# qiangbo1222/HierDiff

Measured on AMD Instinct MI355X. Metric: sampled molecules/sec (1000 diffusion steps, B=256, N=30), higher is better.
Workload: dtype f32

## Files before the change

### hierdiff_amd/csrc/common.hpp

```cpp
#pragma once
#include <hip/hip_runtime.h>
#include <stdint.h>
#include <type_traits>

typedef float f32x4 __attribute__((ext_vector_type(4)));
typedef float f32x16 __attribute__((ext_vector_type(16)));
typedef float f32x2 __attribute__((ext_vector_type(2)));
typedef unsigned u32x4 __attribute__((ext_vector_type(4)));
typedef __bf16 bf16x2_t __attribute__((ext_vector_type(2)));
typedef __bf16 bf16x4_t __attribute__((ext_vector_type(4)));
typedef __bf16 bf16x8_t __attribute__((ext_vector_type(8)));
typedef __bf16 bf16x8 __attribute__((ext_vector_type(8)));

#define HD_DEVINL __device__ __forceinline__

HD_DEVINL void glds16(const void* gsrc, void* lds_dst) {
    __builtin_amdgcn_global_load_lds((const __attribute__((address_space(1))) void*)gsrc,
                                     (__attribute__((address_space(3))) void*)lds_dst, 16, 0, 0);
}
template <int OFF>
HD_DEVINL void glds16o(const void* gsrc, void* lds_dst) {
    static_assert(OFF >= 0 && OFF < 4096, "12-bit immediate");
    __builtin_amdgcn_global_load_lds((const __attribute__((address_space(1))) void*)gsrc,
                                     (__attribute__((address_space(3))) void*)lds_dst, 16, OFF, 0);
}


HD_DEVINL float silu_f(float x) {
    const float L2E_HI = 1.44269502162933349609375f;
    const float L2E_LO = 1.925962991e-8f;
    const float LN2 = 0.693147180559945309f;
    float nx = -x;
    float t = nx * L2E_HI;
    float tlo = __builtin_fmaf(nx, L2E_HI, -t) + nx * L2E_LO;
    float e = __builtin_amdgcn_exp2f(t);
    e = e * __builtin_fmaf(tlo, LN2, 1.0f);
    return x * __builtin_amdgcn_rcpf(1.0f + e);
}

HD_DEVINL float sigmoid_f(float x) {
    const float L2E_HI = 1.44269502162933349609375f, L2E_LO = 1.925962991e-8f, LN2 = 0.693147180559945309f;
    float nx = -x;
    float t = nx * L2E_HI;
    float tlo = __builtin_fmaf(nx, L2E_HI, -t) + nx * L2E_LO;
    float e = __builtin_amdgcn_exp2f(t) * __builtin_fmaf(tlo, LN2, 1.0f);
    return __builtin_amdgcn_rcpf(1.0f + e);
}

HD_DEVINL float silu_fast(float x) {
    float e = __builtin_amdgcn_exp2f(x * -1.44269502162933349609375f);
    return x * __builtin_amdgcn_rcpf(1.0f + e);
}

HD_DEVINL float silu_scaled(float x) { return x * __builtin_amdgcn_rcpf(1.0f + __builtin_amdgcn_exp2f(x)); }
HD_DEVINL void bf16_split2(float y0, float y1, uint32_t& hi, uint32_t& lo) {
    const uint32_t hp = __builtin_bit_cast(uint32_t, __builtin_convertvector((f32x2){y0, y1}, bf16x2_t));
    const float l0 = y0 - __builtin_bit_cast(float, hp << 16);
    const float l1 = y1 - __builtin_bit_cast(float, hp & 0xffff0000u);
    hi = hp;
    lo = __builtin_bit_cast(uint32_t, __builtin_convertvector((f32x2){l0, l1}, bf16x2_t));
}

typedef _Float16 f16x8 __attribute__((ext_vector_type(8)));
typedef _Float16 f16x2_t __attribute__((ext_vector_type(2)));
HD_DEVINL void f16_split2(float y0, float y1, uint32_t& hi, uint32_t& lo) {
    const f16x2_t hp = __builtin_convertvector((f32x2){y0, y1}, f16x2_t);
    const float l0 = y0 - (float)hp[0];
    const float l1 = y1 - (float)hp[1];
    hi = __builtin_bit_cast(uint32_t, hp);
    lo = __builtin_bit_cast(uint32_t, __builtin_convertvector((f32x2){l0, l1}, f16x2_t));
}
template <bool F16>
HD_DEVINL void split2(float y0, float y1, uint32_t& hi, uint32_t& lo) {
    if constexpr (F16) f16_split2(y0, y1, hi, lo);
    else bf16_split2(y0, y1, hi, lo);
}
template <bool F16>
HD_DEVINL f32x16 mma16(bf16x8 a, bf16x8 b, f32x16 c) {
    if constexpr (F16) return __builtin_amdgcn_mfma_f32_32x32x16_f16(__builtin_bit_cast(f16x8, a), __builtin_bit_cast(f16x8, b), c, 0, 0, 0);
    else return __builtin_amdgcn_mfma_f32_32x32x16_bf16(a, b, c, 0, 0, 0);
}
#define HD_F16_FLOOR 9.5367431640625e-07f
#define HD_TWOWAY(p) ((p) == 1 || (p) == 3)

HD_DEVINL void bf16_split3(float y0, float y1, uint32_t& hi, uint32_t& mid, uint32_t& lo) {
    const uint32_t hp = __builtin_bit_cast(uint32_t, __builtin_convertvector((f32x2){y0, y1}, bf16x2_t));
    const float r0 = y0 - __builtin_bit_cast(float, hp << 16);
    const float r1 = y1 - __builtin_bit_cast(float, hp & 0xffff0000u);
    const uint32_t mp = __builtin_bit_cast(uint32_t, __builtin_convertvector((f32x2){r0, r1}, bf16x2_t));
    const float s0 = r0 - __builtin_bit_cast(float, mp << 16);
    const float s1 = r1 - __builtin_bit_cast(float, mp & 0xffff0000u);
    hi = hp;
    mid = mp;
    lo = __builtin_bit_cast(uint32_t, __builtin_convertvector((f32x2){s0, s1}, bf16x2_t));
}

template <int I, int N, typename F>
HD_DEVINL void static_for(F&& f) {
    if constexpr (I < N) {
        f(std::integral_constant<int, I>{});
        static_for<I + 1, N>(f);
    }
}


HD_DEVINL void philox_round(uint32_t& c0, uint32_t& c1, uint32_t& c2, uint32_t& c3, uint32_t k0, uint32_t k1) {
    const uint32_t M0 = 0xD2511F53u, M1 = 0xCD9E8D57u;
    uint32_t hi0 = __umulhi(M0, c0), lo0 = M0 * c0;
    uint32_t hi1 = __umulhi(M1, c2), lo1 = M1 * c2;
    uint32_t n0 = hi1 ^ c1 ^ k0, n1 = lo1, n2 = hi0 ^ c3 ^ k1, n3 = lo0;
    c0 = n0; c1 = n1; c2 = n2; c3 = n3;
}

HD_DEVINL float philox_normal(uint64_t seed, uint64_t sample, uint32_t draw, uint32_t index) {
    uint32_t c0 = index >> 1, c1 = draw, c2 = (uint32_t)sample, c3 = (uint32_t)(sample >> 32);
    uint32_t k0 = (uint32_t)seed, k1 = (uint32_t)(seed >> 32);
#pragma unroll
    for (int r = 0; r < 10; ++r) {
        philox_round(c0, c1, c2, c3, k0, k1);
        k0 += 0x9E3779B9u; k1 += 0xBB67AE85u;
    }
    float u1 = ((float)(c0 >> 8) + 0.5f) * (1.0f / 16777216.0f);
    float u2 = ((float)(c1 >> 8) + 0.5f) * (1.0f / 16777216.0f);
    float rad = sqrtf(-2.0f * logf(u1));
    float ang = 6.283185307179586f * u2;
    return (index & 1) ? rad * sinf(ang) : rad * cosf(ang);
}
```

### hierdiff_amd/csrc/hierdiff_hip.hip

```cpp
#include "../../include/hierdiff_hip.h"
#include "kernels.hpp"

#include <algorithm>
#include <cmath>
#include <cstdio>
#include <cstring>
#include <cstdlib>
#include <string>
#include <mutex>
#include <vector>


static thread_local std::string g_err;

static int fail(int code, const std::string& msg) {
    g_err = msg;
    return code;
}

#define HIP_TRY(expr)                                                                        \
    do {                                                                                     \
        hipError_t _e = (expr);                                                              \
        if (_e != hipSuccess)                                                                \
            return fail(HD_E_HIP, std::string(#expr) + ": " + hipGetErrorString(_e));        \
    } while (0)

#define HD_TRY(expr)                 \
    do {                             \
        int _r = (expr);             \
        if (_r != HD_OK) return _r;  \
    } while (0)


#define HD_FUSE_MIN_ROWS 5400
#define HD_NODE_SPLIT_MAX_ROWS 2048
#define HD_SPLIT_MAX_TILES 512
#define HD_MIX_MAX_TILES 16384

struct LayerW {
    size_t ab_img, ab_bias, wrd, w2_img, b2, wa, w3_img, b3, w4_img, b4;
    size_t ab_gimg, w3_gimg, w4_gimg;
    float ba;
    float w2s, wrmax, wdmax;
    float w3s, w4s, abs_;
    float w3l1, w4l1, b3max, b4max;
};

struct ProfRec { int fam; hipEvent_t a, b; };

struct hd_handle {
    hd_config cfg;
    int device;
    int H, fin, F, D, NS;
    int edge_mode, node_mode;
    bool scaled;
    long long n_weights;
    bool weights_set;
    float* dw;
    size_t dw_floats;
    size_t embT, emb_b, outW, out_b;
    std::vector<LayerW> gcl;
    std::vector<LayerW> coord;
    int* d_nanflag;
    long long* d_nan_events;
    int T;
    std::vector<float> tau_h, coef_h;
    float* d_tau;
    float* d_coef;
    int* d_step;
    uint32_t* d_draw;
    float* d_tcur;
    unsigned long long* d_base;
    hipStream_t own_stream;
    hipEvent_t ev_in, ev_out;
    hipEvent_t ev_last;
    bool ev_last_set;
    unsigned long long weights_gen, sched_gen;
    float* d_coef_ip;
    unsigned long long ip_sched_gen, ip_gen;
    uint32_t* d_ipdraw;
    int ipdraw_cap;
    int split_max_tiles;
    int fuse_min_rows;
    int node_split_max_rows;
    int f32_split;
    int mix_max_tiles;
    int mix_rounds;
    int n_cu;
#ifdef HD_DEBUG_KERNELS
    long long* d_trace;
    int trace_wg;
    int ablate;
#endif
    int prof;
    int prof_stride;
    long long prof_fwd;
    bool prof_now;
    std::vector<ProfRec> recs;
    std::vector<hipEvent_t> pool;
    size_t pool_used;
};

struct GraphKey {
    const float *raw_x, *raw_h;
    int has_ctx, mol_shape, noise_rows, T, s_hi;
    uint64_t seed;
    unsigned long long weights_gen, sched_gen;
    bool operator==(const GraphKey& o) const {
        return raw_x == o.raw_x && raw_h == o.raw_h && has_ctx == o.has_ctx && mol_shape == o.mol_shape &&
               noise_rows == o.noise_rows && T == o.T && s_hi == o.s_hi && seed == o.seed && weights_gen == o.weights_gen &&
               sched_gen == o.sched_gen;
    }
};

struct InpaintKey {
    int has_ctx, T, resamplings;
    uint64_t seed;
    unsigned long long weights_gen, sched_gen, ip_gen;
    bool operator==(const InpaintKey& o) const {
        return has_ctx == o.has_ctx && T == o.T && resamplings == o.resamplings && seed == o.seed && weights_gen == o.weights_gen &&
               sched_gen == o.sched_gen && ip_gen == o.ip_gen;
    }
};

struct hd_topology {
    hd_handle* h;
    int device;
    char* arena;
    int B, N, M, M_pad, E, E_pad, n_tiles, n_wg, n_parts;
    int *node_of, *slot_of, *ei, *ej, *seg_part, *tile_nseg, *pstart, *nvalid;
    int *rptr, *rrows, *sptr, *srows;
    std::vector<int>* node_of_host;
    float *w2img, *w2timg;
    uint8_t *eseg, *nm_bytes;
    float* nmask;
    float *hbuf, *AB, *AB2, *Tb, *agg, *x0, *xcur, *part, *xpart, *eps;
    float *abmax, *abmax2;
    float *rowinfo;
    float *zbuf, *ctxbuf;
    hipGraphExec_t gexec;
    GraphKey gkey;
    hipGraphExec_t gexec_ip;
    InpaintKey ikey;
    uint8_t* ip_fixed;
    float* ip_known;
    size_t arena_bytes;
    char* staging;
    size_t staging_bytes;
    hipStream_t stream0, last_stream;
    hipEvent_t ready;
    bool multi_stream;
};


static inline float agg_norm(const hd_config& c, const hd_topology* t) {
    return c.aggregation_mean ? (float)t->N : c.normalization_factor;
}

extern "C" int hd_version(void) { return HD_ABI_VERSION; }
extern "C" const char* hd_last_error(void) { return g_err.c_str(); }

extern "C" int hd_device_count(void) {
    int n = 0;
    if (hipGetDeviceCount(&n) != hipSuccess) { (void)hipGetLastError(); return 0; }
    return n;
}

static long long weight_count(const hd_config& c) {
    const long long H = c.hidden_nf, fin = c.in_node_nf + c.context_node_nf;
    long long n = H * fin + H + fin * H + fin;
    long long gcl = H * (2 * H + 2) + H + H * H + H + H * 2 * H + H + H * H + H + (c.attention ? H + 1 : 0);
    long long crd = H * (2 * H + 2) + H + H * H + H + H;
    n += (long long)c.n_layers * (c.inv_sublayers * gcl + crd);
    return n;
}

extern "C" long long hd_weight_count(const hd_handle* h) { return h ? h->n_weights : 0; }

template <typename T>
static int dev_alloc(T** p, size_t count) {
    *p = nullptr;
    if (count == 0) count = 1;
    hipError_t e = hipMalloc(reinterpret_cast<void**>(p), count * sizeof(T));
    if (e != hipSuccess) return fail(HD_E_NOMEM, std::string("hipMalloc: ") + hipGetErrorString(e));
    return HD_OK;
}

template <typename T>
static int dev_upload(T** p, const std::vector<T>& v) {
    HD_TRY(dev_alloc(p, v.size()));
    if (!v.empty()) HIP_TRY(hipMemcpy(*p, v.data(), v.size() * sizeof(T), hipMemcpyHostToDevice));
    return HD_OK;
}


static int prepare_kernels(hd_handle* h);
template <int H> static int prepare_edge_bwd_h();

extern "C" int hd_create(const hd_config* cfg, int device, hd_handle** out) {
    if (!cfg || !out) return fail(HD_E_INVALID, "hd_create: null argument");
    *out = nullptr;
    if (cfg->n_dims != 3) return fail(HD_E_INVALID, "hd_create: n_dims must be 3");
    const int H = cfg->hidden_nf;
    if (H != 32 && H != 64 && H != 128 && H != 256)
        return fail(HD_E_INVALID, "hd_create: hidden_nf must be 32, 64, 128 or 256");
    if (cfg->n_layers < 1 || cfg->inv_sublayers < 1) return fail(HD_E_INVALID, "hd_create: n_layers / inv_sublayers must be >= 1");
    const int F = cfg->in_node_nf - (cfg->condition_time ? 1 : 0);
    if (F < 1) return fail(HD_E_INVALID, "hd_create: in_node_nf must leave at least one feature column");
    if (cfg->context_node_nf < 0) return fail(HD_E_INVALID, "hd_create: context_node_nf < 0");
    if (cfg->precision != 0 && cfg->precision != 3)
        return fail(HD_E_INVALID, "hd_create: precision must be 0 (fp32) or 3 (fp16x3); 1 (bf16x3) and 2 (bf16x6) were retired in ABI 12");
    if (!cfg->aggregation_mean && !(cfg->normalization_factor != 0.0f)) return fail(HD_E_INVALID, "hd_create: normalization_factor == 0");
    if (hd_device_count() <= device || device < 0)
        return fail(HD_E_HIP, "hd_create: no such HIP device (is a GPU visible?)");
    HIP_TRY(hipSetDevice(device));
    hd_handle* h = new hd_handle();
    h->cfg = *cfg;
    h->device = device;
    h->H = H;
    h->fin = cfg->in_node_nf + cfg->context_node_nf;
    h->F = F;
    h->D = 3 + F;
    {
        const bool wide = cfg->hidden_nf >= 128;
        switch (cfg->precision) {
            case 3: h->edge_mode = 3; h->node_mode = wide ? 3 : 0; break;
            default: h->edge_mode = 0; h->node_mode = 0; break;
        }
        h->scaled = h->edge_mode == 3;
    }
    h->NS = (cfg->hidden_nf == 32) ? 1 : 2;
    h->n_weights = weight_count(*cfg);
    h->weights_set = false;
    h->dw = nullptr;
    h->dw_floats = 0;
    h->T = 0;
    h->d_tau = h->d_coef = nullptr;
    h->prof = 0;
    h->prof_stride = 1;
    h->prof_fwd = 0;
    h->prof_now = false;
    h->pool_used = 0;
    h->own_stream = nullptr;
    h->ev_in = h->ev_out = nullptr;
    h->ev_last = nullptr; h->ev_last_set = false;
    h->weights_gen = h->sched_gen = 0;
    h->d_coef_ip = nullptr; h->ip_sched_gen = 0; h->ip_gen = 0; h->d_ipdraw = nullptr; h->ipdraw_cap = 0;
    h->d_nanflag = nullptr; h->d_nan_events = nullptr; h->d_step = nullptr; h->d_draw = nullptr; h->d_tcur = nullptr;
    h->d_base = nullptr;
    h->split_max_tiles = HD_SPLIT_MAX_TILES;
    h->mix_max_tiles = HD_MIX_MAX_TILES;
    h->fuse_min_rows = HD_FUSE_MIN_ROWS;
    h->node_split_max_rows = HD_NODE_SPLIT_MAX_ROWS;
    h->f32_split = 1;
    h->mix_rounds = -1;
    {
        hipDeviceProp_t prop;
        h->n_cu = (hipGetDeviceProperties(&prop, device) == hipSuccess && prop.multiProcessorCount > 0) ? prop.multiProcessorCount : 256;
    }
#ifdef HD_DEBUG_KERNELS
    h->d_trace = nullptr; h->trace_wg = 0;
    { const char* e = getenv("HD_ABLATE"); h->ablate = e ? atoi(e) : 0; }
    { const char* e = getenv("HD_SPLIT_MAX_TILES"); if (e) h->split_max_tiles = atoi(e); }
    { const char* e = getenv("HD_MIX_MAX_TILES"); if (e) h->mix_max_tiles = atoi(e); }
    { const char* e = getenv("HD_FUSE_MIN_ROWS"); if (e) h->fuse_min_rows = atoi(e); }
    { const char* e = getenv("HD_NODE_SPLIT_MAX_ROWS"); if (e) h->node_split_max_rows = atoi(e); }
    { const char* e = getenv("HD_F32_SPLIT"); if (e) h->f32_split = atoi(e); }
    { const char* e = getenv("HD_MIX_ROUNDS"); if (e) h->mix_rounds = atoi(e); }
#endif
    auto create_rest = [&]() -> int {
        HD_TRY(dev_alloc(&h->d_nanflag, 1));
        HD_TRY(dev_alloc(&h->d_nan_events, 1));
        HD_TRY(dev_alloc(&h->d_step, 1));
        HD_TRY(dev_alloc(&h->d_draw, 1));
        HD_TRY(dev_alloc(&h->d_tcur, 1));
        HD_TRY(dev_alloc(&h->d_base, 1));
        HIP_TRY(hipMemset(h->d_nanflag, 0, sizeof(int)));
        HIP_TRY(hipMemset(h->d_nan_events, 0, sizeof(long long)));
        HIP_TRY(hipEventCreateWithFlags(&h->ev_in, hipEventDisableTiming));
        HIP_TRY(hipEventCreateWithFlags(&h->ev_out, hipEventDisableTiming));
        HIP_TRY(hipEventCreateWithFlags(&h->ev_last, hipEventDisableTiming));
        return prepare_kernels(h);
    };
    const int r = create_rest();
    if (r != HD_OK) { const std::string keep = g_err; hd_destroy(h); g_err = keep; return r; }
    *out = h;
    return HD_OK;
}

extern "C" int hd_destroy(hd_handle* h) {
    if (!h) return HD_OK;
    (void)hipSetDevice(h->device);
    (void)hipDeviceSynchronize();
    hipFree(h->dw); hipFree(h->d_nanflag); hipFree(h->d_nan_events);
    hipFree(h->d_tau); hipFree(h->d_coef); hipFree(h->d_step); hipFree(h->d_draw); hipFree(h->d_tcur); hipFree(h->d_base);
    hipFree(h->d_coef_ip); hipFree(h->d_ipdraw);
#ifdef HD_DEBUG_KERNELS
    hipFree(h->d_trace);
#endif
    for (auto e : h->pool) hipEventDestroy(e);
    if (h->ev_in) hipEventDestroy(h->ev_in);
    if (h->ev_out) hipEventDestroy(h->ev_out);
    if (h->ev_last) hipEventDestroy(h->ev_last);
    if (h->own_stream) hipStreamDestroy(h->own_stream);
    delete h;
    return HD_OK;
}


template <typename Fn>
static void pack_gemm_b(std::vector<float>& dst, size_t off, int K, int Nc, int WN, Fn W) {
    const int BN = 32 * WN, ntile = Nc / BN, nchunk = K / 32;
    for (int ct = 0; ct < ntile; ++ct)
        for (int c = 0; c < nchunk; ++c)
            for (int wc = 0; wc < WN; ++wc)
                for (int q = 0; q < 4; ++q)
                    for (int lane = 0; lane < 64; ++lane)
                        for (int j = 0; j < 4; ++j) {
                            const int k = 32 * c + 16 * (lane >> 5) + 4 * q + j;
                            const int col = ct * BN + 32 * wc + (lane & 31);
                            dst[off + ((((size_t)(ct * nchunk + c) * WN + wc) * 4 + q) * 64 + lane) * 4 + j] = W(col, k);
                        }
}

template <typename Fn>
static void pack_gemm_b16(std::vector<float>& dst, size_t off, int K, int Nc, Fn W) {
    const int nchunk = K / 32;
    for (int ct = 0; ct < Nc / 16; ++ct)
        for (int c = 0; c < nchunk; ++c)
            for (int lane = 0; lane < 64; ++lane)
                for (int p = 0; p < 8; ++p) {
                    const int m = lane & 15, gs = lane >> 4, odd = gs >> 1, hf = gs & 1;
                    dst[off + (((size_t)ct * nchunk + c) * 64 + lane) * 8 + p] = W(16 * ct + m, 32 * c + 16 * hf + 2 * p + odd);
                }
}

static void pack_edge_w2(std::vector<float>& dst, size_t off, int H, const float* W2) {
    const int NCT = H / 32;
    for (int c = 0; c < H / 32; ++c)
        for (int q = 0; q < 4; ++q)
            for (int ct = 0; ct < NCT; ++ct)
                for (int lane = 0; lane < 64; ++lane)
                    for (int j = 0; j < 4; ++j) {
                        const int k = 32 * c + 16 * (lane >> 5) + 4 * q + j;
                        const int col = 32 * ct + (lane & 31);
                        dst[off + (size_t)c * 32 * H + ((size_t)(q * NCT + ct) * 64 + lane) * 4 + j] = W2[(size_t)col * H + k];
                    }
}

template <typename Fn>
static float pack_node_b_f16(std::vector<float>& dstf, size_t off, int K, int Nc, Fn W, float* l1) {
    float wmax = 0.0f, l1max = 0.0f;
    for (int col = 0; col < Nc; ++col) {
        double sum = 0.0;
        for (int k = 0; k < K; ++k) { const float v = std::fabs(W(col, k)); sum += v; if (v > wmax && std::isfinite(v)) wmax = v; }
        l1max = std::max(l1max, (float)(sum * 1.000001));
    }
    if (l1) *l1 = l1max;
    int ex = 0;
    if (wmax > 0.0f) (void)std::frexp(wmax, &ex);
    const float sw = std::ldexp(1.0f, wmax > 0.0f ? std::max(-100, std::min(100, 15 - ex)) : 0);
    _Float16* dst = reinterpret_cast<_Float16*>(dstf.data() + off);
    const int nct = Nc / 32;
    for (int st = 0; st < K / 16; ++st)
        for (int ct = 0; ct < nct; ++ct)
            for (int lane = 0; lane < 64; ++lane)
                for (int i = 0; i < 8; ++i) {
                    const float v = W(32 * ct + (lane & 31), 16 * st + 8 * (lane >> 5) + i) * sw;
                    const size_t base = ((size_t)(st * nct + ct) * 2) * 512;
                    const _Float16 hi = (_Float16)v;
                    dst[base + (size_t)lane * 8 + i] = hi;
                    dst[base + 512 + (size_t)lane * 8 + i] = (_Float16)(v - (float)hi);
                }
    return sw;
}

template <typename Fn>
static void pack_node_b_f32(std::vector<float>& dst, size_t off, int K, int Nc, Fn W) {
    const int nct = Nc / 32;
    for (int st = 0; st < K / 32; ++st)
        for (int ct = 0; ct < nct; ++ct)
            for (int q = 0; q < 4; ++q)
                for (int lane = 0; lane < 64; ++lane)
                    for (int j = 0; j < 4; ++j)
                        dst[off + (((size_t)(st * nct + ct) * 4 + q) * 64 + lane) * 4 + j] =
                            W(32 * ct + (lane & 31), 32 * st + 16 * (lane >> 5) + 4 * q + j);
}

static float pack_edge_w2_f16(std::vector<float>& dstf, size_t off, int H, const float* W2) {
    float wmax = 0.0f;
    for (size_t i = 0; i < (size_t)H * H; ++i) { const float v = std::fabs(W2[i]); if (v > wmax && std::isfinite(v)) wmax = v; }
    int ex = 0;
    if (wmax > 0.0f) (void)std::frexp(wmax, &ex);
    const int k = std::max(-100, std::min(100, 15 - ex));
    const float sw = std::ldexp(1.0f, wmax > 0.0f ? k : 0);
    _Float16* dst = reinterpret_cast<_Float16*>(dstf.data() + off);
    const int NCT = H / 32;
    for (int c = 0; c < H / 32; ++c)
        for (int st = 0; st < 2; ++st)
            for (int ct = 0; ct < NCT; ++ct)
                for (int lane = 0; lane < 64; ++lane)
                    for (int i = 0; i < 8; ++i) {
                        const int kk = 32 * c + 16 * (lane >> 5) + 8 * st + i;
                        const int col = 32 * ct + (lane & 31);
                        const float v = W2[(size_t)col * H + kk] * sw;
                        const _Float16 hi = (_Float16)v;
                        const _Float16 lo = (_Float16)(v - (float)hi);
                        const size_t blk = (size_t)c * 32 * H * 2;
// ... 274 lines not shown
    std::vector<float>& nmask = L.nmask;
    slot_of.assign(BN, -1); node_of.clear(); nvalid.assign(B, 0); nmask.clear();
    for (size_t f = 0; f < BN; ++f) {
        if (active[f]) { slot_of[f] = (int)node_of.size(); node_of.push_back((int)f); nmask.push_back(node_mask[f] ? 1.0f : 0.0f); }
        if (node_mask[f]) nvalid[f / N]++;
    }
    const int M = (int)node_of.size();
    const int M_pad = std::max(128, (M + 127) / 128 * 128);
    nmask.resize(M_pad, 0.0f);
    std::vector<int> mei, mej;
    std::vector<long long> mstart(B + 1, 0);
    for (int b = 0; b < B; ++b) {
        for (int i = 0; i < N; ++i) {
            const size_t fi = (size_t)b * N + i;
            if (!active[fi]) continue;
            for (int j = 0; j < N; ++j) {
                const size_t fj = (size_t)b * N + j;
                const bool on = edge_mask ? edge_mask[fi * N + j] != 0 : (node_mask[fi] && node_mask[fj] && i != j);
                if (on) { mei.push_back(slot_of[fi]); mej.push_back(slot_of[fj]); }
            }
        }
        mstart[b + 1] = (long long)mei.size();
    }
    const long long E = (long long)mei.size();
    if (E > (1LL << 30)) return fail(HD_E_INVALID, "hd_topology_create: too many edges");
    std::vector<int>& pstart = L.pstart;
    std::vector<int> first_piece(M, 0);
    pstart.assign(M + 1, 0);
    for (int b = 0; b < B; ++b) {
        const long long e0 = mstart[b], e1 = mstart[b + 1];
        for (long long e = e0; e < e1;) {
            const int node = mei[e];
            long long f = e;
            while (f < e1 && mei[f] == node) ++f;
            first_piece[node] = (int)((e - e0) / 32);
            pstart[node + 1] = (int)((f - 1 - e0) / 32) - first_piece[node] + 1;
            e = f;
        }
    }
    for (int i = 0; i < M; ++i) pstart[i + 1] += pstart[i];
    std::vector<int>&ei = L.ei, &ej = L.ej, &seg_part = L.seg_part, &tile_nseg = L.tile_nseg;
    std::vector<uint8_t>& eseg = L.eseg;
    ei.clear(); ej.clear(); seg_part.clear(); tile_nseg.clear(); eseg.clear();
    auto new_tile = [&]() {
        const int t = (int)tile_nseg.size();
        ei.resize(ei.size() + 32, 0); ej.resize(ej.size() + 32, 0); eseg.resize(eseg.size() + 32, 255);
        seg_part.resize(seg_part.size() + 32, 0); tile_nseg.push_back(0);
        return t;
    };
    auto place = [&](int t, int off, int b, int piece, int cnt) {
        const long long e0 = mstart[b] + 32LL * piece;
        int prev = -1;
        for (int r = 0; r < cnt; ++r) {
            const int node = mei[e0 + r];
            if (node != prev) {
                seg_part[(size_t)t * 32 + tile_nseg[t]] = pstart[node] + (piece - first_piece[node]);
                tile_nseg[t]++;
                prev = node;
            }
            ei[(size_t)t * 32 + off + r] = node; ej[(size_t)t * 32 + off + r] = mej[e0 + r];
            eseg[(size_t)t * 32 + off + r] = (uint8_t)(tile_nseg[t] - 1);
        }
    };
    int tail_tile = -1, tail_fill = 0;
    for (int b = 0; b < B; ++b) {
        const int Eb = (int)(mstart[b + 1] - mstart[b]);
        const int nfull = Eb / 32, tail = Eb % 32;
        for (int k = 0; k < nfull; ++k) place(new_tile(), 0, b, k, 32);
        if (tail) {
            if (tail_tile < 0 || tail_fill + tail > 32) { tail_tile = new_tile(); tail_fill = 0; }
            place(tail_tile, tail_fill, b, nfull, tail);
            tail_fill = (tail_fill + tail + 3) & ~3;
        }
    }
    L.n_tiles = (int)tile_nseg.size();
    L.n_wg = (L.n_tiles + 3) / 4;
    while ((int)tile_nseg.size() < std::max(1, L.n_wg * 4)) new_tile();
    L.M = M; L.M_pad = M_pad; L.E = E; L.n_parts = pstart[M];
    L.rptr.assign(M + 1, 0); L.sptr.assign(M + 1, 0);
    const size_t rows = ei.size();
    for (size_t r = 0; r < rows; ++r)
        if (eseg[r] != 255) { L.rptr[ei[r] + 1]++; L.sptr[ej[r] + 1]++; }
    for (int i = 0; i < M; ++i) { L.rptr[i + 1] += L.rptr[i]; L.sptr[i + 1] += L.sptr[i]; }
    L.rrows.assign((size_t)E, 0); L.srows.assign((size_t)E, 0);
    {
        std::vector<int> rp(L.rptr.begin(), L.rptr.end() - 1), sp(L.sptr.begin(), L.sptr.end() - 1);
        for (size_t r = 0; r < rows; ++r)
            if (eseg[r] != 255) { L.rrows[rp[ei[r]]++] = (int)r; L.srows[sp[ej[r]]++] = (int)r; }
    }
    return HD_OK;
}

extern "C" int hd_topology_layout(const uint8_t* node_mask, const uint8_t* edge_mask, int B, int N, long long* counts5,
                                  int* ei, int* ej, uint8_t* eseg, int* seg_part, int* tile_nseg, int* pstart) {
    if (!node_mask || !counts5) return fail(HD_E_INVALID, "hd_topology_layout: null argument");
    TileLayout L;
    HD_TRY(build_layout(node_mask, edge_mask, B, N, L));
    counts5[0] = L.M; counts5[1] = L.E; counts5[2] = (long long)L.tile_nseg.size(); counts5[3] = L.n_parts;
    counts5[4] = (long long)L.ei.size();
    if (ei) std::copy(L.ei.begin(), L.ei.end(), ei);
    if (ej) std::copy(L.ej.begin(), L.ej.end(), ej);
    if (eseg) std::copy(L.eseg.begin(), L.eseg.end(), eseg);
    if (seg_part) std::copy(L.seg_part.begin(), L.seg_part.end(), seg_part);
    if (tile_nseg) std::copy(L.tile_nseg.begin(), L.tile_nseg.end(), tile_nseg);
    if (pstart) std::copy(L.pstart.begin(), L.pstart.end(), pstart);
    return HD_OK;
}

extern "C" int hd_topology_create_s(hd_handle* h, const uint8_t* node_mask, const uint8_t* edge_mask, int B, int N,
                                    void* stream, hd_topology** out) {
    if (!h || !node_mask || !out) return fail(HD_E_INVALID, "hd_topology_create: null argument");
    hipStream_t s0 = (hipStream_t)stream;
    *out = nullptr;
    TileLayout L;
    HD_TRY(build_layout(node_mask, edge_mask, B, N, L));
    HIP_TRY(hipSetDevice(h->device));
    const size_t BN = (size_t)B * N;
    const int M = L.M, M_pad = L.M_pad, n_tiles = L.n_tiles, n_wg = L.n_wg, n_parts = L.n_parts;
    const long long E = L.E;
    const int E_pad = (int)L.ei.size();
    std::vector<int>&slot_of = L.slot_of, &node_of = L.node_of, &nvalid = L.nvalid, &ei = L.ei, &ej = L.ej;
    std::vector<int>&seg_part = L.seg_part, &tile_nseg = L.tile_nseg, &pstart = L.pstart;
    std::vector<uint8_t>& eseg = L.eseg;
    std::vector<float>& nmask = L.nmask;
    std::vector<uint8_t> nm_bytes(BN);
    for (size_t f = 0; f < BN; ++f) nm_bytes[f] = node_mask[f] ? 1 : 0;

    hd_topology* t = new hd_topology();
    std::memset(t, 0, sizeof(*t));
    t->h = h; t->device = h->device; t->B = B; t->N = N; t->M = M; t->M_pad = M_pad; t->E = (int)E; t->E_pad = E_pad;
    t->n_tiles = n_tiles; t->n_wg = n_wg; t->n_parts = n_parts;
    const int H = h->H;
    std::vector<char> blob;
    auto stage = [&](const void* src, size_t bytes) {
        const size_t off = (blob.size() + 255) & ~size_t(255);
        blob.resize(off + std::max<size_t>(bytes, 4), 0);
        if (bytes) std::memcpy(blob.data() + off, src, bytes);
        return off;
    };
    auto stage_v = [&](const auto& v) { return stage(v.data(), v.size() * sizeof(v[0])); };
    const size_t o_node_of = stage_v(node_of), o_slot_of = stage_v(slot_of), o_ei = stage_v(ei), o_ej = stage_v(ej);
    const size_t o_seg_part = stage_v(seg_part), o_tile_nseg = stage_v(tile_nseg), o_pstart = stage_v(pstart), o_nvalid = stage_v(nvalid);
    const size_t o_eseg = stage_v(eseg), o_nm = stage_v(nm_bytes), o_nmask = stage_v(nmask);
    const size_t o_rptr = stage_v(L.rptr), o_rrows = stage_v(L.rrows), o_sptr = stage_v(L.sptr), o_srows = stage_v(L.srows);
    const size_t table_bytes = (blob.size() + 255) & ~size_t(255);
    size_t ws_floats = 0;
    auto carve = [&](size_t count) { const size_t o = ws_floats; ws_floats += (std::max<size_t>(count, 1) + 63) & ~size_t(63); return o; };
    const size_t f_h = carve((size_t)M_pad * H), f_AB = carve((size_t)M_pad * 2 * H), f_AB2 = carve((size_t)M_pad * 2 * H);
    const size_t f_Tb = carve((size_t)M_pad * H), f_agg = carve((size_t)M_pad * H);
    const size_t f_x0 = carve((size_t)M_pad * 4), f_xcur = carve((size_t)M_pad * 4);
    const size_t f_part = carve((size_t)std::max(1, n_parts) * H), f_xpart = carve((size_t)std::max(1, n_parts) * 4);
    const size_t f_abmax = carve((size_t)M_pad * 2), f_abmax2 = carve((size_t)M_pad * 2), f_rowinfo = carve((size_t)M_pad * 2);
    const size_t f_eps = carve(BN * h->D), f_z = carve(BN * h->D), f_ctx = carve(BN * (size_t)std::max(1, h->cfg.context_node_nf));
    const size_t f_w2 = carve((size_t)H * H * 3 / 2), f_w2t = carve((size_t)H * H * 3 / 2);
    auto build = [&]() -> int {
        ArenaSlot sl;
        HD_TRY(arena_acquire(h->device, table_bytes + ws_floats * sizeof(float), table_bytes, sl));
        t->arena = sl.dev; t->arena_bytes = sl.dev_bytes; t->staging = sl.pinned; t->staging_bytes = sl.pinned_bytes;
        t->stream0 = t->last_stream = s0;
        char* base = t->arena;
        std::memcpy(t->staging, blob.data(), blob.size());
        HIP_TRY(hipMemcpyAsync(base, t->staging, blob.size(), hipMemcpyHostToDevice, s0));
        HIP_TRY(hipMemsetAsync(base + table_bytes, 0, ws_floats * sizeof(float), s0));
        HIP_TRY(hipEventCreateWithFlags(&t->ready, hipEventDisableTiming));
        HIP_TRY(hipEventRecord(t->ready, s0));
        auto I = [&](size_t off) { return reinterpret_cast<int*>(base + off); };
        t->node_of = I(o_node_of); t->slot_of = I(o_slot_of); t->ei = I(o_ei); t->ej = I(o_ej); t->seg_part = I(o_seg_part);
        t->tile_nseg = I(o_tile_nseg); t->pstart = I(o_pstart); t->nvalid = I(o_nvalid);
        t->eseg = reinterpret_cast<uint8_t*>(base + o_eseg); t->nm_bytes = reinterpret_cast<uint8_t*>(base + o_nm);
        t->nmask = reinterpret_cast<float*>(base + o_nmask);
        t->rptr = I(o_rptr); t->rrows = I(o_rrows); t->sptr = I(o_sptr); t->srows = I(o_srows);
        float* ws = reinterpret_cast<float*>(base + table_bytes);
        t->hbuf = ws + f_h; t->AB = ws + f_AB; t->AB2 = ws + f_AB2; t->Tb = ws + f_Tb; t->agg = ws + f_agg; t->x0 = ws + f_x0;
        t->xcur = ws + f_xcur; t->part = ws + f_part; t->xpart = ws + f_xpart; t->eps = ws + f_eps; t->zbuf = ws + f_z;
        t->abmax = ws + f_abmax; t->abmax2 = ws + f_abmax2; t->rowinfo = ws + f_rowinfo;
        t->ctxbuf = ws + f_ctx; t->w2img = ws + f_w2; t->w2timg = ws + f_w2t;
        t->node_of_host = new std::vector<int>(node_of);
        return HD_OK;
    };
    const int r = build();
    if (r != HD_OK) { const std::string keep = g_err; hd_topology_destroy(t); g_err = keep; return r; }
    *out = t;
    return HD_OK;
}

extern "C" int hd_topology_create(hd_handle* h, const uint8_t* node_mask, const uint8_t* edge_mask, int B, int N,
                                  hd_topology** out) {
    HD_TRY(hd_topology_create_s(h, node_mask, edge_mask, B, N, nullptr, out));
    HIP_TRY(hipStreamSynchronize(nullptr));
    hipEvent_t ev = (*out)->ready;
    (*out)->ready = nullptr;
    if (ev) (void)hipEventDestroy(ev);
    return HD_OK;
}

__global__ void k_widen_index(const int* src, long long* dst, int n) {
    const int i = blockIdx.x * blockDim.x + threadIdx.x;
    if (i < n) dst[i] = src[i];
}

extern "C" int hd_topology_nodes_device(hd_topology* t, long long* index, void* stream) {
    if (!t || !index) return fail(HD_E_INVALID, "hd_topology_nodes_device: null argument");
    HIP_TRY(hipSetDevice(t->device));
    topo_use(t, (hipStream_t)stream);
    if (t->M > 0) hipLaunchKernelGGL(k_widen_index, dim3((t->M + 255) / 256), dim3(256), 0, (hipStream_t)stream, t->node_of, index, t->M);
    HIP_TRY(hipGetLastError());
    return HD_OK;
}

extern "C" int hd_topology_info(const hd_topology* t, long long* info6) {
    if (!t || !info6) return fail(HD_E_INVALID, "hd_topology_info: null argument");
    info6[0] = t->B; info6[1] = t->N; info6[2] = t->M; info6[3] = t->E; info6[4] = t->n_tiles; info6[5] = t->n_parts;
    return HD_OK;
}


extern "C" int hd_profile_enable(hd_handle* h, int on) {
    if (!h) return fail(HD_E_INVALID, "hd_profile_enable: null handle");
    h->prof = on & 7;
    h->prof_stride = std::max(1, on >> 8);
    h->prof_fwd = 0;
    h->prof_now = false;
    h->recs.clear();
    h->pool_used = 0;
    return HD_OK;
}

static hipEvent_t prof_event(hd_handle* h) {
    if (h->pool_used == h->pool.size()) {
        hipEvent_t e;
        hipEventCreate(&e);
        h->pool.push_back(e);
    }
    return h->pool[h->pool_used++];
}

struct ProfScope {
    hd_handle* h; hipStream_t s; int fam; hipEvent_t a;
    ProfScope(hd_handle* h_, hipStream_t s_, int fam_) : h(h_), s(s_), fam(fam_), a(nullptr) {
        if (h->prof_now && (h->prof & (1 << fam))) { a = prof_event(h); hipEventRecord(a, s); }
    }
    ~ProfScope() {
        if (a) { hipEvent_t b = prof_event(h); hipEventRecord(b, s); h->recs.push_back({fam, a, b}); }
    }
};

extern "C" int hd_profile_read(hd_handle* h, double* ms3, long long* launches3) {
    if (!h || !ms3 || !launches3) return fail(HD_E_INVALID, "hd_profile_read: null argument");
    for (int k = 0; k < 3; ++k) { ms3[k] = 0.0; launches3[k] = 0; }
    for (auto& r : h->recs) {
        HIP_TRY(hipEventSynchronize(r.b));
        float ms = 0.f;
        HIP_TRY(hipEventElapsedTime(&ms, r.a, r.b));
        ms3[r.fam] += ms;
        launches3[r.fam] += 1;
    }
    h->recs.clear();
    h->pool_used = 0;
    return HD_OK;
}


template <int WM, int WN, int CN>
static void launch_gemm(int epi, bool cat, const GemmArgs& g, hipStream_t s) {
    const int nrt = (g.M + 32 * WM - 1) / (32 * WM), nct = g.Nc / (32 * WN * CN);
    dim3 grid(8 * ((nrt + 7) / 8) * nct);
    dim3 block(WM * WN * 64);
    if (cat && epi == EPI_RANK1_SILU) hipLaunchKernelGGL((k_gemm<WM, WN, CN, EPI_RANK1_SILU, true>), grid, block, 0, s, g);
    else if (epi == EPI_BIAS_MASK) hipLaunchKernelGGL((k_gemm<WM, WN, CN, EPI_BIAS_MASK, false>), grid, block, 0, s, g);
    else if (cat && epi == EPI_BIAS) hipLaunchKernelGGL((k_gemm<WM, WN, CN, EPI_BIAS, true>), grid, block, 0, s, g);
    else if (cat) hipLaunchKernelGGL((k_gemm<WM, WN, CN, EPI_BIAS_SILU, true>), grid, block, 0, s, g);
    else if (epi == EPI_BIAS_SILU) hipLaunchKernelGGL((k_gemm<WM, WN, CN, EPI_BIAS_SILU, false>), grid, block, 0, s, g);
    else if (epi == EPI_BIAS) hipLaunchKernelGGL((k_gemm<WM, WN, CN, EPI_BIAS, false>), grid, block, 0, s, g);
    else if (epi == EPI_EGCL_PRE) hipLaunchKernelGGL((k_gemm<WM, WN, CN, EPI_EGCL_PRE, false>), grid, block, 0, s, g);
    else hipLaunchKernelGGL((k_gemm<WM, WN, CN, EPI_RESID_MASK, false>), grid, block, 0, s, g);
}

template <int RT>
static void launch_r16(int epi, bool agg, const R16Args& g, hipStream_t s) {
    const int wpt = g.Nc >= 128 ? 8 : (g.Nc >> 4);
    const dim3 grid(((g.M + 16 * RT - 1) / (16 * RT)) * (g.Nc / (16 * wpt)) * g.n_img), block(512);
    const int lds = 16 * RT * (g.K + 4) * 4;
    if (agg) hipLaunchKernelGGL((k_gemm_r16<EPI_BIAS_SILU, true, RT>), grid, block, lds, s, g);
    else if (epi == EPI_BIAS) hipLaunchKernelGGL((k_gemm_r16<EPI_BIAS, false, RT>), grid, block, lds, s, g);
    else if (epi == EPI_BIAS_SILU) hipLaunchKernelGGL((k_gemm_r16<EPI_BIAS_SILU, false, RT>), grid, block, lds, s, g);
    else hipLaunchKernelGGL((k_gemm_r16<EPI_RESID_MASK, false, RT>), grid, block, lds, s, g);
}

static void gemm_r16(hd_handle* h, int epi, bool agg, const R16Args& g, hipStream_t s) {
    ProfScope ps(h, s, 1);
    launch_r16<1>(epi, agg, g, s);
}

template <int H>
static int node_lds_bytes(bool upd, int np = 2) {
    const int r1 = std::max(32 * (H + 8) * 2 * np, 32 * (H + 4) * 4);
    return 32 * ((upd ? 2 * H : H) + 8) * 2 * np + r1;
}

template <int H>
static int node_f32_lds_bytes(bool upd) { return 32 * ((upd ? 2 * H : H) + 4) * 4 + 32 * (H + 4) * 4; }

template <int H, int NW>
static void launch_node_hw(bool upd, int nab, int mode, const NodeArgs& a, hipStream_t s) {
    const int nrt = (a.M + 31) / 32;
    const dim3 grid(8 * ((nrt + 7) / 8)), block(64 * NW);
    if (mode == 0) {
        const int ldsf = node_f32_lds_bytes<H>(upd);
        if (!upd) hipLaunchKernelGGL((k_node_f32<H, NW, false, 1>), grid, block, ldsf, s, a);
        else if (nab == 1) hipLaunchKernelGGL((k_node_f32<H, NW, true, 1>), grid, block, ldsf, s, a);
        else hipLaunchKernelGGL((k_node_f32<H, NW, true, 2>), grid, block, ldsf, s, a);
        return;
    }
    if constexpr (H >= 128) {
        const int lds = node_lds_bytes<H>(upd);
        if (!upd) hipLaunchKernelGGL((k_node<H, NW, false, 1, 2, true>), grid, block, lds, s, a);
        else if (nab == 1) hipLaunchKernelGGL((k_node<H, NW, true, 1, 2, true>), grid, block, lds, s, a);
        else hipLaunchKernelGGL((k_node<H, NW, true, 2, 2, true>), grid, block, lds, s, a);
    }
}

template <int H, int NW>
static int prepare_node_hw() {
    HIP_TRY(hipFuncSetAttribute((const void*)k_node_f32<H, NW, false, 1>, hipFuncAttributeMaxDynamicSharedMemorySize, node_f32_lds_bytes<H>(false)));
    HIP_TRY(hipFuncSetAttribute((const void*)k_node_f32<H, NW, true, 1>, hipFuncAttributeMaxDynamicSharedMemorySize, node_f32_lds_bytes<H>(true)));
    HIP_TRY(hipFuncSetAttribute((const void*)k_node_f32<H, NW, true, 2>, hipFuncAttributeMaxDynamicSharedMemorySize, node_f32_lds_bytes<H>(true)));
    if constexpr (H >= 128) {
        HIP_TRY(hipFuncSetAttribute((const void*)k_node<H, NW, false, 1, 2, true>, hipFuncAttributeMaxDynamicSharedMemorySize, node_lds_bytes<H>(false)));
        HIP_TRY(hipFuncSetAttribute((const void*)k_node<H, NW, true, 1, 2, true>, hipFuncAttributeMaxDynamicSharedMemorySize, node_lds_bytes<H>(true)));
        HIP_TRY(hipFuncSetAttribute((const void*)k_node<H, NW, true, 2, 2, true>, hipFuncAttributeMaxDynamicSharedMemorySize, node_lds_bytes<H>(true)));
    }
    return HD_OK;
}

template <int H>
static void launch_node_h(bool upd, int nab, int mode, const NodeArgs& a, hipStream_t s) {
    launch_node_hw<H, (H / 32 < 8 ? H / 32 : 8)>(upd, nab, mode, a, s);
}

template <int H>
static int prepare_node_h() { return prepare_node_hw<H, (H / 32 < 8 ? H / 32 : 8)>(); }

static void node_update(hd_handle* h, bool upd, int nab, const NodeArgs& a, hipStream_t s) {
    ProfScope ps(h, s, 1);
    const int mode = h->node_mode;
    switch (h->H) {
        case 32: launch_node_h<32>(upd, nab, mode, a, s); break;
        case 64: launch_node_h<64>(upd, nab, mode, a, s); break;
        case 128: launch_node_h<128>(upd, nab, mode, a, s); break;
        default: launch_node_h<256>(upd, nab, mode, a, s); break;
    }
}

template <int H, int PH, int CTW>
static void launch_node_split_hc(const NodeSplitArgs& a, hipStream_t s) {
    const int nrt = (a.M + 31) / 32;
    const int per = (PH == 3 ? 2 * H / 32 * a.n_img : H / 32) / CTW;
    const int lds = node_split_lds_bytes<H, PH, CTW>();
    hipLaunchKernelGGL((k_node_split<H, PH, CTW>), dim3(8 * ((nrt + 7) / 8) * per), dim3(256), lds, s, a);
}
template <int H, int PH>
static void launch_node_split_h(const NodeSplitArgs& a, hipStream_t s) { launch_node_split_hc<H, PH, 1>(a, s); }
template <int PH>
static void launch_node_split(hd_handle* h, const NodeSplitArgs& a, hipStream_t s) {
    ProfScope ps(h, s, 1);
    if (h->H == 128) launch_node_split_h<128, PH>(a, s); else launch_node_split_h<256, PH>(a, s);
}
template <int H, int PH, int CTW>
static int prepare_node_split_one() {
    const int lds = node_split_lds_bytes<H, PH, CTW>();
    HIP_TRY(hipFuncSetAttribute((const void*)k_node_split<H, PH, CTW>, hipFuncAttributeMaxDynamicSharedMemorySize, lds));
    return HD_OK;
// ... 60 lines not shown
        }
        hipLaunchKernelGGL((k_edge<256, false, PREC, ABL>), grid, block, lds, s, b);
    };
    switch (h->ablate) {
        case 1: run(std::integral_constant<int, 1>{}); return true;
        case 2: run(std::integral_constant<int, 2>{}); return true;
        case 4: run(std::integral_constant<int, 4>{}); return true;
        case 5: run(std::integral_constant<int, 5>{}); return true;
        case 8: run(std::integral_constant<int, 8>{}); return true;
        case 12: run(std::integral_constant<int, 12>{}); return true;
        case 13: run(std::integral_constant<int, 13>{}); return true;
        case 15: run(std::integral_constant<int, 15>{}); return true;
        case 16: run(std::integral_constant<int, 16>{}); return true;
        case 18: run(std::integral_constant<int, 18>{}); return true;
        case 20: run(std::integral_constant<int, 20>{}); return true;
        case 24: run(std::integral_constant<int, 24>{}); return true;
        case 30: run(std::integral_constant<int, 30>{}); return true;
        case 32: run(std::integral_constant<int, 32>{}); return true;
        case 64: run(std::integral_constant<int, 64>{}); return true;
        case 128: run(std::integral_constant<int, 128>{}); return true;
        case 1024: run(std::integral_constant<int, 1024>{}); return true;
        case 1025: run(std::integral_constant<int, 1025>{}); return true;
        default: return false;
    }
}
#else
extern "C" int hd_debug_edge_trace(hd_handle*, long long*, int) { return 0; }
#endif

static bool edge_runs_split(const hd_handle* h, int n_tiles, int mode) {
    return n_tiles > 0 && n_tiles <= (mode == 0 ? h->split_max_tiles + h->split_max_tiles / 3 : h->split_max_tiles);
}
static bool edge_runs_mixed(const hd_handle* h, int n_tiles, int mode) {
    const int per_round = 4 * h->n_cu;
    const int left = n_tiles - (n_tiles / per_round) * per_round;
    const bool pays = left > 0 && left * 10 <= (mode == 0 ? 29 : 10) * h->n_cu;
    return n_tiles > per_round && n_tiles < h->mix_max_tiles && (pays || h->mix_rounds >= 0);
}

template <int H>
static int launch_edge_h(hd_handle* h, bool coord, const EdgeArgs& a, hipStream_t s, int mode_override = -1) {
    const int lds = edge_lds_bytes<H>();
    const int prec = mode_override >= 0 ? mode_override : h->edge_mode;
    const dim3 grid(a.n_wg), block(256);
    if constexpr (H >= 128) {
        if (a.dscal) {
            if (a.pre2) {
                if (coord) hipLaunchKernelGGL((k_edge<H, true, 3, HD_EDGE_SAVE | HD_EDGE_UNSCALED>), grid, block, lds, s, a);
                else hipLaunchKernelGGL((k_edge<H, false, 3, HD_EDGE_SAVE | HD_EDGE_UNSCALED>), grid, block, lds, s, a);
            } else {
                if (coord) hipLaunchKernelGGL((k_edge<H, true, 3, HD_EDGE_UNSCALED>), grid, block, lds, s, a);
                else hipLaunchKernelGGL((k_edge<H, false, 3, HD_EDGE_UNSCALED>), grid, block, lds, s, a);
            }
            return HD_OK;
        }
    }
    if (a.pre2) {
        if (coord) hipLaunchKernelGGL((k_edge<H, true, 0, HD_EDGE_SAVE>), grid, block, lds, s, a);
        else hipLaunchKernelGGL((k_edge<H, false, 0, HD_EDGE_SAVE>), grid, block, lds, s, a);
        return HD_OK;
    }
#ifdef HD_DEBUG_KERNELS
    if constexpr (H == 256) {
        if (h->ablate && !coord && (prec == 3 ? launch_edge_ablated<3>(h, a, s) : launch_edge_ablated<0>(h, a, s))) return HD_OK;
    }
#endif
    if constexpr (H >= 128) {
        const int mode = prec;
        if (edge_runs_split(h, a.n_tiles, mode)) {
            const dim3 sgrid(a.n_tiles);
            if (mode == 0) {
                if (coord) hipLaunchKernelGGL((k_edge_split<H, true, 0>), sgrid, block, 0, s, a);
                else hipLaunchKernelGGL((k_edge_split<H, false, 0>), sgrid, block, 0, s, a);
            } else {
                if (coord) hipLaunchKernelGGL((k_edge_split<H, true, 3>), sgrid, block, 0, s, a);
                else hipLaunchKernelGGL((k_edge_split<H, false, 3>), sgrid, block, 0, s, a);
            }
            return HD_OK;
        }
    }
    if constexpr (H >= 128) {
        const int mode = prec;
        const int per_round = 4 * h->n_cu;
        int R = a.n_tiles / per_round;
        if (edge_runs_mixed(h, a.n_tiles, mode)) {
            if (h->mix_rounds >= 0) R = std::min(R, h->mix_rounds);
            EdgeArgs m = a;
            m.n_wg = R * h->n_cu;
            const dim3 mgrid(m.n_wg + (a.n_tiles - 4 * m.n_wg));
            const int ldsm = std::max(edge_lds_bytes<H>(), edge_split_lds_bytes<H, 0>());
            if (mode == 0) {
                if (coord) hipLaunchKernelGGL((k_edge_mixed<H, true, 0>), mgrid, block, ldsm, s, m);
                else hipLaunchKernelGGL((k_edge_mixed<H, false, 0>), mgrid, block, ldsm, s, m);
            } else {
                if (coord) hipLaunchKernelGGL((k_edge_mixed<H, true, 3>), mgrid, block, ldsm, s, m);
                else hipLaunchKernelGGL((k_edge_mixed<H, false, 3>), mgrid, block, ldsm, s, m);
            }
            return HD_OK;
        }
    }
    if (prec == 3) {
        if (coord) hipLaunchKernelGGL((k_edge<H, true, 3>), grid, block, lds, s, a);
        else hipLaunchKernelGGL((k_edge<H, false, 3>), grid, block, lds, s, a);
    } else {
        if (coord) hipLaunchKernelGGL((k_edge<H, true, 0>), grid, block, lds, s, a);
        else hipLaunchKernelGGL((k_edge<H, false, 0>), grid, block, lds, s, a);
    }
    return HD_OK;
}

template <int H>
static int prepare_edge_h() {
    const int lds = edge_lds_bytes<H>();
    HIP_TRY(hipFuncSetAttribute((const void*)k_edge<H, true, 0>, hipFuncAttributeMaxDynamicSharedMemorySize, lds));
    HIP_TRY(hipFuncSetAttribute((const void*)k_edge<H, false, 0>, hipFuncAttributeMaxDynamicSharedMemorySize, lds));
    HIP_TRY(hipFuncSetAttribute((const void*)k_edge<H, true, 3>, hipFuncAttributeMaxDynamicSharedMemorySize, lds));
    HIP_TRY(hipFuncSetAttribute((const void*)k_edge<H, false, 3>, hipFuncAttributeMaxDynamicSharedMemorySize, lds));
    HIP_TRY(hipFuncSetAttribute((const void*)k_edge<H, true, 0, HD_EDGE_SAVE>, hipFuncAttributeMaxDynamicSharedMemorySize, lds));
    HIP_TRY(hipFuncSetAttribute((const void*)k_edge<H, false, 0, HD_EDGE_SAVE>, hipFuncAttributeMaxDynamicSharedMemorySize, lds));
    if constexpr (H >= 128) {
        HIP_TRY(hipFuncSetAttribute((const void*)k_edge<H, true, 3, HD_EDGE_SAVE | HD_EDGE_UNSCALED>, hipFuncAttributeMaxDynamicSharedMemorySize, lds));
        HIP_TRY(hipFuncSetAttribute((const void*)k_edge<H, false, 3, HD_EDGE_SAVE | HD_EDGE_UNSCALED>, hipFuncAttributeMaxDynamicSharedMemorySize, lds));
        HIP_TRY(hipFuncSetAttribute((const void*)k_edge<H, true, 3, HD_EDGE_UNSCALED>, hipFuncAttributeMaxDynamicSharedMemorySize, lds));
        HIP_TRY(hipFuncSetAttribute((const void*)k_edge<H, false, 3, HD_EDGE_UNSCALED>, hipFuncAttributeMaxDynamicSharedMemorySize, lds));
        const int m0 = std::max(edge_lds_bytes<H>(), edge_split_lds_bytes<H, 0>());
        HIP_TRY(hipFuncSetAttribute((const void*)k_edge_mixed<H, true, 0>, hipFuncAttributeMaxDynamicSharedMemorySize, m0));
        HIP_TRY(hipFuncSetAttribute((const void*)k_edge_mixed<H, false, 0>, hipFuncAttributeMaxDynamicSharedMemorySize, m0));
        HIP_TRY(hipFuncSetAttribute((const void*)k_edge_mixed<H, true, 3>, hipFuncAttributeMaxDynamicSharedMemorySize, m0));
        HIP_TRY(hipFuncSetAttribute((const void*)k_edge_mixed<H, false, 3>, hipFuncAttributeMaxDynamicSharedMemorySize, m0));
    }
    return HD_OK;
}

static int prepare_kernels(hd_handle* h) {
    switch (h->H) {
        case 32: HD_TRY(prepare_node_h<32>()); HD_TRY(prepare_edge_bwd_h<32>()); return prepare_edge_h<32>();
        case 64: HD_TRY(prepare_node_h<64>()); HD_TRY(prepare_edge_bwd_h<64>()); return prepare_edge_h<64>();
        case 128: HD_TRY(prepare_node_h<128>()); HD_TRY(prepare_node_split_h<128>()); HD_TRY(prepare_edge_bwd_h<128>()); return prepare_edge_h<128>();
        default: HD_TRY(prepare_node_h<256>()); HD_TRY(prepare_node_split_h<256>()); HD_TRY(prepare_edge_bwd_h<256>()); return prepare_edge_h<256>();
    }
}

static int edge(hd_handle* h, bool coord, const EdgeArgs& a, hipStream_t s, int mode_override = -1) {
    if (a.n_wg == 0) return HD_OK;
    ProfScope ps(h, s, 0);
    switch (h->H) {
        case 32: return launch_edge_h<32>(h, coord, a, s, mode_override);
        case 64: return launch_edge_h<64>(h, coord, a, s, mode_override);
        case 128: return launch_edge_h<128>(h, coord, a, s, mode_override);
        default: return launch_edge_h<256>(h, coord, a, s, mode_override);
    }
}

static int forward_impl(hd_handle* h, hd_topology* t, const float* xh, const float* tt, int t_numel,
                        const float* context, int mol_shape, float* out, hipStream_t s) {
    const hd_config& c = h->cfg;
    const int H = h->H, M = t->M;
    const float* W = h->dw;
    h->prof_now = h->prof != 0 && (h->prof_fwd++ % h->prof_stride) == 0;
    if (M == 0) HIP_TRY(hipMemsetAsync(h->d_nanflag, 0, sizeof(int), s));
    if (M > 0) {
        {
            ProfScope ps(h, s, 2);
            InitArgs a;
            a.xh = xh; a.t = tt; a.ctx = context; a.node_of = t->node_of; a.nmask = t->nmask;
            a.embT = W + h->embT; a.emb_b = W + h->emb_b; a.h = t->hbuf; a.x0 = t->x0; a.xcur = t->xcur;
            a.nanflag = h->d_nanflag;
            a.zero_max = (h->node_mode == 3 && M < h->node_split_max_rows && h->edge_mode == 3) ? t->abmax : nullptr;
            a.M = M; a.N = t->N; a.D = h->D; a.F = h->F; a.C = c.context_node_nf; a.H = H;
            a.t_stride = (t_numel == 1) ? 0 : 1; a.cond_time = c.condition_time;
            const long long total = (long long)M * (H / 4);
            hipLaunchKernelGGL(k_node_init, dim3((unsigned)((total + 255) / 256)), dim3(256), 0, s, a);
        }
        const float range = c.coords_range / (float)c.n_layers;
        const int S = c.inv_sublayers;
        const float* ab_cur = t->AB;
        auto node_args = [&]() {
            NodeArgs a;
            std::memset(&a, 0, sizeof(a));
            a.h_in = t->hbuf; a.h_out = t->hbuf; a.part = t->part; a.pstart = t->pstart; a.nmask = t->nmask;
            a.norm = agg_norm(c, t); a.M = M;
            return a;
        };
        auto set_ab = [&](NodeArgs& a, int q, const LayerW& nw, float* dst) {
            a.ABimg[q] = W + nw.ab_img; a.ABbias[q] = W + nw.ab_bias; a.ABout[q] = dst;
            a.abinv[q] = h->node_mode == 3 ? 1.0f / nw.abs_ : 1.0f;
            a.ABmax[q] = (h->edge_mode == 3 && h->node_mode != 0) ? (dst == t->AB ? t->abmax : t->abmax2) : nullptr;
        };
        const bool fused = h->node_mode != 0 || M >= h->fuse_min_rows;
        auto r16_args = [&]() {
            R16Args g;
            std::memset(&g, 0, sizeof(g));
            g.A = t->hbuf; g.lda = H; g.K1 = H; g.K = H; g.M = M; g.n_img = 1; g.nmask = t->nmask; g.norm = agg_norm(c, t);
            return g;
        };
        auto ab_r16 = [&](int nab, const LayerW* const* nxt, float* const* dst) {
            R16Args g = r16_args();
            g.Nc = 2 * H; g.ldc = 2 * H; g.n_img = nab;
            for (int q = 0; q < nab; ++q) { g.Bimg[q] = W + nxt[q]->ab_gimg; g.bias[q] = W + nxt[q]->ab_bias; g.C[q] = dst[q]; }
            gemm_r16(h, EPI_BIAS, false, g, s);
        };
        const bool nsplit = h->node_mode == 3 && M < h->node_split_max_rows;
        const bool fsplit = h->node_mode == 0 && M < h->fuse_min_rows && H >= 128 && h->f32_split;
        auto split_args = [&]() {
            NodeSplitArgs a;
            std::memset(&a, 0, sizeof(a));
            a.h_in = t->hbuf; a.h_out = t->hbuf; a.part = t->part; a.pstart = t->pstart; a.nmask = t->nmask; a.norm = agg_norm(c, t);
            a.T = t->Tb; a.rowinfo = t->rowinfo; a.M = M; a.n_img = 1;
            return a;
        };
        auto split_ab = [&](NodeSplitArgs& a, int q, const LayerW& nw, float* dst) {
            a.Wimg[q] = W + nw.ab_img; a.bias[q] = W + nw.ab_bias; a.winv[q] = 1.0f / nw.abs_; a.ABout[q] = dst;
            a.ABmax[q] = h->edge_mode == 3 ? (dst == t->AB ? t->abmax : t->abmax2) : nullptr;
        };
        {
            const LayerW* first[2] = {&h->gcl[0], nullptr};
            float* dst[2] = {t->AB, nullptr};
            if (nsplit) {
                NodeSplitArgs a = split_args();
                split_ab(a, 0, h->gcl[0], t->AB);
                a.upd = 0;
                launch_node_split<3>(h, a, s);
            } else if (fsplit) {
                NodeSplitArgs a = split_args();
                a.Wimg[0] = W + h->gcl[0].ab_img; a.bias[0] = W + h->gcl[0].ab_bias; a.ABout[0] = t->AB; a.upd = 0;
                launch_node_split_f32<3>(h, a, s);
            } else if (fused) {
                NodeArgs a = node_args();
                set_ab(a, 0, h->gcl[0], t->AB);
                node_update(h, false, 1, a, s);
            } else {
                ab_r16(1, first, dst);
            }
        }
        for (int i = 0; i < c.n_layers; ++i) {
            for (int j = 0; j <= c.inv_sublayers; ++j) {
                const bool coord = (j == c.inv_sublayers);
                const LayerW& w = coord ? h->coord[i] : h->gcl[(size_t)i * c.inv_sublayers + j];
                EdgeArgs e;
                std::memset(&e, 0, sizeof(e));
                e.AB = ab_cur; e.wrd = W + w.wrd; e.W2img = W + w.w2_img; e.b2 = W + w.b2; e.wa = W + w.wa;
                e.w2s_inv = 1.0f / w.w2s; e.wrmax = w.wrmax; e.wdmax = w.wdmax;
                const bool fused_max = h->edge_mode == 3 && h->node_mode != 0;
                e.abmax = (fused_max && ab_cur == t->AB2) ? t->abmax2 : t->abmax;
                if (h->edge_mode == 3 && !fused_max) {
                    ProfScope ps(h, s, 2);
                    AbMaxArgs am{ab_cur, t->abmax, M, H};
                    hipLaunchKernelGGL(k_ab_rowmax, dim3((M + 3) / 4), dim3(256), 0, s, am);
                }
                e.ei = t->ei; e.ej = t->ej; e.eseg = t->eseg; e.seg_part = t->seg_part; e.tile_nseg = t->tile_nseg;
                e.xcur = t->xcur; e.x0 = t->x0; e.part = coord ? t->xpart : t->part; e.ba = w.ba;
                e.norm_constant = c.norm_constant; e.coords_range = range; e.attention = c.attention;
                e.use_tanh = c.tanh; e.n_tiles = t->n_tiles; e.n_wg = t->n_wg;
                HD_TRY(edge(h, coord, e, s));
                if (!coord) {
                    const LayerW* nxt[2] = {nullptr, nullptr};
                    float* dst[2] = {t->AB, t->AB2};
                    int nab = 1;
                    if (j + 1 < S) {
                        nxt[0] = &h->gcl[(size_t)i * S + j + 1];
                    } else {
                        nxt[0] = &h->coord[i];
                        if (i + 1 < c.n_layers) { nxt[1] = &h->gcl[(size_t)(i + 1) * S]; nab = 2; }
                    }
                    if (nsplit) {
                        NodeSplitArgs a = split_args();
                        a.w3l1 = w.w3l1; a.w4l1 = w.w4l1; a.b3max = w.b3max; a.b4max = w.b4max;
                        NodeSplitArgs p1 = a, p2 = a, p3 = a;
                        p1.Wimg[0] = W + w.w3_img; p1.bias[0] = W + w.b3; p1.winv[0] = 1.0f / w.w3s;
                        launch_node_split<1>(h, p1, s);
                        p2.Wimg[0] = W + w.w4_img; p2.bias[0] = W + w.b4; p2.winv[0] = 1.0f / w.w4s;
                        p3.n_img = nab; p3.upd = 1;
                        for (int q = 0; q < nab; ++q) { split_ab(p3, q, *nxt[q], dst[q]); p2.zero_max[q] = p3.ABmax[q]; }
                        launch_node_split<2>(h, p2, s);
                        launch_node_split<3>(h, p3, s);
                    } else if (fsplit) {
                        NodeSplitArgs p1 = split_args(), p2 = split_args(), p3 = split_args();
                        p1.Wimg[0] = W + w.w3_img; p1.bias[0] = W + w.b3;
                        launch_node_split_f32<1>(h, p1, s);
                        p2.Wimg[0] = W + w.w4_img; p2.bias[0] = W + w.b4;
                        launch_node_split_f32<2>(h, p2, s);
                        p3.n_img = nab; p3.upd = 1;
                        for (int q = 0; q < nab; ++q) { p3.Wimg[q] = W + nxt[q]->ab_img; p3.bias[q] = W + nxt[q]->ab_bias; p3.ABout[q] = dst[q]; }
                        launch_node_split_f32<3>(h, p3, s);
                    } else if (fused) {
                        NodeArgs a = node_args();
                        a.W3img = W + w.w3_img; a.b3 = W + w.b3; a.W4img = W + w.w4_img; a.b4 = W + w.b4;
                        if (h->node_mode == 3) {
                            a.w3inv = 1.0f / w.w3s; a.w4inv = 1.0f / w.w4s; a.w3l1 = w.w3l1; a.w4l1 = w.w4l1; a.b3max = w.b3max; a.b4max = w.b4max;
                        }
                        for (int q = 0; q < nab; ++q) set_ab(a, q, *nxt[q], dst[q]);
                        node_update(h, true, nab, a, s);
                    } else {
                        R16Args g = r16_args();
                        g.part = t->part; g.pstart = t->pstart; g.K1 = H; g.K = 2 * H; g.Nc = H;
                        g.Bimg[0] = W + w.w3_gimg; g.bias[0] = W + w.b3; g.C[0] = t->Tb; g.ldc = H;
                        gemm_r16(h, EPI_BIAS_SILU, true, g, s);
                        g = r16_args();
                        g.A = t->Tb; g.Bimg[0] = W + w.w4_gimg; g.bias[0] = W + w.b4; g.C[0] = t->hbuf; g.ldc = H; g.Nc = H;
                        gemm_r16(h, EPI_RESID_MASK, false, g, s);
                        ab_r16(nab, nxt, dst);
                    }
                    ab_cur = t->AB;
                } else {
                    ProfScope ps(h, s, 2);
                    XupdArgs x;
                    x.part = t->xpart; x.pstart = t->pstart; x.nmask = t->nmask; x.xcur = t->xcur;
                    x.norm = agg_norm(c, t); x.M = M;
                    hipLaunchKernelGGL(k_xupd, dim3((M + 255) / 256), dim3(256), 0, s, x);
                    ab_cur = t->AB2;
                }
            }
        }
        {
            ProfScope ps(h, s, 2);
            Post1Args p;
            p.h = t->hbuf; p.outW = W + h->outW; p.out_b = W + h->out_b; p.x0 = t->x0; p.xcur = t->xcur;
            p.node_of = t->node_of; p.nmask = t->nmask; p.out = out; p.nanflag = h->d_nanflag;
            p.M = M; p.N = t->N; p.D = h->D; p.F = h->F; p.H = H; p.mol_shape = mol_shape;
            hipLaunchKernelGGL(k_post1, dim3((M + 3) / 4), dim3(256), 0, s, p);
        }
    }
    {
        ProfScope ps(h, s, 2);
        Post2Args p;
        p.slot_of = t->slot_of; p.nmask = t->nmask; p.nvalid = t->nvalid; p.out = out; p.nanflag = h->d_nanflag;
        p.nan_events = h->d_nan_events; p.B = t->B; p.N = t->N; p.D = h->D;
        hipLaunchKernelGGL(k_post2, dim3((t->B + 3) / 4), dim3(256), 0, s, p);
    }
    HIP_TRY(hipGetLastError());
    return HD_OK;
}

static int check_ready(hd_handle* h, hd_topology* t, const char* who) {
    if (!h || !t) return fail(HD_E_INVALID, std::string(who) + ": null handle/topology");
    if (t->h != h) return fail(HD_E_INVALID, std::string(who) + ": topology belongs to another handle");
    if (!h->weights_set) return fail(HD_E_STATE, std::string(who) + ": weights not set (hd_set_weights)");
    return HD_OK;
}

extern "C" int hd_egnn_forward(hd_handle* h, hd_topology* topo, const float* xh, const float* t, int t_numel,
                               const float* context, int mol_shape, float* out, void* stream) {
    HD_TRY(check_ready(h, topo, "hd_egnn_forward"));
    if (!xh || !out) return fail(HD_E_INVALID, "hd_egnn_forward: null tensor");
    if (h->cfg.condition_time && (!t || (t_numel != 1 && t_numel != topo->B)))
        return fail(HD_E_INVALID, "hd_egnn_forward: t must have 1 or B elements");
    if (h->cfg.context_node_nf > 0 && !context) return fail(HD_E_INVALID, "hd_egnn_forward: context required");
    if (mol_shape > topo->N) mol_shape = topo->N;
    HIP_TRY(hipSetDevice(h->device));
    topo_use(topo, (hipStream_t)stream);
    return forward_impl(h, topo, xh, t, t_numel, context, mol_shape, out, (hipStream_t)stream);
}

extern "C" int hd_nan_events(hd_handle* h, void* stream, long long* count) {
    if (!h || !count) return fail(HD_E_INVALID, "hd_nan_events: null argument");
    HIP_TRY(hipStreamSynchronize((hipStream_t)stream));
    HIP_TRY(hipMemcpy(count, h->d_nan_events, sizeof(long long), hipMemcpyDeviceToHost));
    return HD_OK;
}


extern "C" int hd_topology_nodes(const hd_topology* t, int* node_of) {
    if (!t || !node_of) return fail(HD_E_INVALID, "hd_topology_nodes: null argument");
    std::copy(t->node_of_host->begin(), t->node_of_host->end(), node_of);
    return HD_OK;
}

template <int H>
static int edge_bwd_lds_bytes() { return (2 * 32 * H + 4 * 288) * 4; }

template <int H>
static int prepare_edge_bwd_h() {
    const int lds = edge_bwd_lds_bytes<H>();
    HIP_TRY(hipFuncSetAttribute((const void*)k_edge_bwd<H, false, 0>, hipFuncAttributeMaxDynamicSharedMemorySize, lds));
    HIP_TRY(hipFuncSetAttribute((const void*)k_edge_bwd<H, false, 1>, hipFuncAttributeMaxDynamicSharedMemorySize, lds));
    HIP_TRY(hipFuncSetAttribute((const void*)k_edge_bwd<H, true, 0>, hipFuncAttributeMaxDynamicSharedMemorySize, lds));
    HIP_TRY(hipFuncSetAttribute((const void*)k_edge_bwd<H, true, 1>, hipFuncAttributeMaxDynamicSharedMemorySize, lds));
    if constexpr (H >= 128) {
        HIP_TRY(hipFuncSetAttribute((const void*)k_edge_bwd<H, false, 1, 3>, hipFuncAttributeMaxDynamicSharedMemorySize, lds));
        HIP_TRY(hipFuncSetAttribute((const void*)k_edge_bwd<H, true, 1, 3>, hipFuncAttributeMaxDynamicSharedMemorySize, lds));
    }
    return HD_OK;
}

template <int H>
static void launch_edge_bwd_h(bool coord, int stage, int prec, const EdgeBwdArgs& a, int n_wg, hipStream_t s) {
    const dim3 grid(n_wg), block(256);
    if (stage == 0 && a.pre2) {
        const int ldss = 4 * 288 * 4;
        if (coord) hipLaunchKernelGGL((k_edge_bwd<H, true, 0, 0, true>), grid, block, ldss, s, a);
        else hipLaunchKernelGGL((k_edge_bwd<H, false, 0, 0, true>), grid, block, ldss, s, a);
        return;
    }
    if constexpr (H >= 128) {
        if (prec == 3 && stage == 1) {
            const int lds = (2 * 16 * H + 4 * 288) * 4;
            if (coord) hipLaunchKernelGGL((k_edge_bwd<H, true, 1, 3>), grid, block, lds, s, a);
            else hipLaunchKernelGGL((k_edge_bwd<H, false, 1, 3>), grid, block, lds, s, a);
            return;
        }
    }
    const int lds = edge_bwd_lds_bytes<H>();
    if (!coord && stage == 0) hipLaunchKernelGGL((k_edge_bwd<H, false, 0>), grid, block, lds, s, a);
    else if (!coord) hipLaunchKernelGGL((k_edge_bwd<H, false, 1>), grid, block, lds, s, a);
    else if (stage == 0) hipLaunchKernelGGL((k_edge_bwd<H, true, 0>), grid, block, lds, s, a);
    else hipLaunchKernelGGL((k_edge_bwd<H, true, 1>), grid, block, lds, s, a);
}

static void launch_edge_bwd(hd_handle* h, bool coord, int stage, int prec, const EdgeBwdArgs& a, int n_wg, hipStream_t s) {
    switch (h->H) {
        case 32: launch_edge_bwd_h<32>(coord, stage, 0, a, n_wg, s); break;
        case 64: launch_edge_bwd_h<64>(coord, stage, 0, a, n_wg, s); break;
        case 128: launch_edge_bwd_h<128>(coord, stage, prec, a, n_wg, s); break;
        default: launch_edge_bwd_h<256>(coord, stage, prec, a, n_wg, s); break;
    }
}

static int check_train(hd_handle* h, hd_topology* t, const char* who) {
    if (!h || !t) return fail(HD_E_INVALID, std::string(who) + ": null handle/topology");
    if (t->h != h) return fail(HD_E_INVALID, std::string(who) + ": topology belongs to another handle");
    if (h->cfg.precision != 0) return fail(HD_E_STATE, std::string(who) + ": training primitives need precision 0 (exact fp32)");
    return HD_OK;
}

extern "C" long long hd_edge_layer_f16ws_floats(hd_handle* h, hd_topology* t, int* n_wg) {
    if (!h || !t || t->h != h) return 0;
    if (n_wg) *n_wg = t->n_wg;
    return 4 + 2 * (long long)t->n_wg + (long long)t->n_wg * 4 * 32;
}

extern "C" long long hd_edge_layer_save_rows(hd_handle* h, hd_topology* t, int precision) {
    if (!h || !t || t->h != h || t->n_wg == 0 || t->M == 0) return 0;
    if (precision != 0 && precision != 3) return 0;
    const int mode = h->H >= 128 ? precision : 0;
    if (h->H >= 128 && edge_runs_split(h, t->n_tiles, mode)) return 0;
    return (long long)t->n_wg * 4 * 32 + 32;
}

extern "C" int hd_edge_layer_forward_s(hd_handle* h, hd_topology* t, int coord, int precision, const float* AB, const float* x,
                                       const float* x0, const float* wrd, const float* W2, const float* b2,
                                       const float* wa, const float* ba, float* out, float* pre2, void* stream) {
    HD_TRY(check_train(h, t, "hd_edge_layer_forward"));
    if (precision != 0 && precision != 3)
        return fail(HD_E_INVALID, "hd_edge_layer_forward_s: precision must be 0 (fp32) or 3 (fp16x3); 2 (bf16x6) was retired in ABI 12");
    const bool f16 = precision == 3 && h->H >= 128;
    topo_use(t, (hipStream_t)stream);
    if (!AB || !x || !x0 || !wrd || !W2 || !b2 || !wa || !out) return fail(HD_E_INVALID, "hd_edge_layer_forward: null tensor");
    HIP_TRY(hipSetDevice(h->device));
    hipStream_t s = (hipStream_t)stream;
    const hd_config& c = h->cfg;
    const int H = h->H, M = t->M;
    const int ow = coord ? 4 : H;
    if (t->n_wg == 0 || M == 0) {
        HIP_TRY(hipMemsetAsync(out, 0, (size_t)std::max(1, M) * ow * sizeof(float), s));
        return HD_OK;
    }
    EdgeArgs e;
    std::memset(&e, 0, sizeof(e));
    if (f16) {
        float* scal = pre2 ? pre2 + (size_t)t->n_wg * 128 * H : t->w2img + (size_t)H * H;
        hipLaunchKernelGGL(k_f16_prep, dim3(1), dim3(1024), 0, s, W2, wrd, scal, H);
        hipLaunchKernelGGL((k_pack_w2_f16<false>), dim3((H * H / 8 + 255) / 256), dim3(256), 0, s, W2, (const float*)scal,
                           reinterpret_cast<f16x8*>(t->w2img), H);
        AbMaxArgs am{AB, t->abmax, M, H};
        hipLaunchKernelGGL(k_ab_rowmax, dim3((M + 3) / 4), dim3(256), 0, s, am);
        e.dscal = scal; e.abmax = t->abmax;
    } else hipLaunchKernelGGL((k_pack_w2<false>), dim3((H * H + 255) / 256), dim3(256), 0, s, W2, t->w2img, H);
    e.AB = AB; e.wrd = wrd; e.W2img = t->w2img; e.b2 = b2; e.wa = wa;
    e.w2s_inv = 1.0f; e.wrmax = e.wdmax = 0.0f;
    e.ei = t->ei; e.ej = t->ej; e.eseg = t->eseg; e.seg_part = t->seg_part; e.tile_nseg = t->tile_nseg;
    e.xcur = x; e.x0 = x0; e.part = coord ? t->xpart : t->part; e.ba = 0.0f; e.ba_ptr = ba;
    e.norm_constant = c.norm_constant; e.coords_range = c.coords_range / (float)c.n_layers; e.attention = c.attention;
    e.use_tanh = c.tanh; e.n_tiles = t->n_tiles; e.n_wg = t->n_wg;
    e.pre2 = pre2;
    HD_TRY(edge(h, coord != 0, e, s, f16 ? 3 : 0));
    AggArgs ag;
    ag.part = coord ? t->xpart : t->part; ag.pstart = t->pstart; ag.agg = out; ag.norm = agg_norm(c, t);
    ag.M = M; ag.H = ow;
    const long long total = (long long)M * (ow / 4);
    hipLaunchKernelGGL(k_agg, dim3((unsigned)((total + 255) / 256)), dim3(256), 0, s, ag);
// ... 572 lines not shown
}

extern "C" int hd_dw2_f16(int device, int rows, int H, const float* G2, const float* P, const float* gmax, const float* pmax, int n,
                          float* dW2, int ldc, float* ws, long long ws_floats, void* stream) {
    const char* who = "hd_dw2_f16";
    if (!G2 || !P || !dW2 || !ws || !gmax || !pmax || n < 1) return fail(HD_E_INVALID, std::string(who) + ": null tensor / no maxima");
    if (H != 128 && H != 256) return fail(HD_E_INVALID, std::string(who) + ": H must be 128 or 256 (narrower layers use hd_gemm_f32)");
    if (rows <= 0 || rows % 32 != 0 || ldc < H) return fail(HD_E_INVALID, std::string(who) + ": rows must be a positive multiple of 32 (whole edge tiles), ldc >= H");
    if (hd_device_count() <= device || device < 0) return fail(HD_E_HIP, std::string(who) + ": no such HIP device (is a GPU visible?)");
    HIP_TRY(hipSetDevice(device));
    hipStream_t s = (hipStream_t)stream;
    int slabs = (int)std::min<long long>(256, ws_floats / ((long long)H * H));
    slabs = std::max(1, std::min(slabs, rows / 128));
    if ((long long)slabs * H * H > ws_floats) return fail(HD_E_INVALID, std::string(who) + ": workspace smaller than one H x H slab");
    const int kslab = ((rows / 32 + slabs - 1) / slabs) * 32;
    slabs = (rows + kslab - 1) / kslab;
    Dw2F16Args a;
    a.G = G2; a.P = P; a.ws = ws; a.gmax = gmax; a.pmax = pmax; a.rows = rows; a.kslab = kslab; a.nmax = n;
    {
        static std::mutex mu;
        static unsigned long long prepared_mask = 0;
        std::lock_guard<std::mutex> lk(mu);
        const unsigned long long bit = 1ull << (device & 63);
        if (!(prepared_mask & bit)) {
            HIP_TRY(hipFuncSetAttribute((const void*)k_dw2_f16<256>, hipFuncAttributeMaxDynamicSharedMemorySize, dw2_f16_lds_bytes<256>()));
            HIP_TRY(hipFuncSetAttribute((const void*)k_dw2_f16<128>, hipFuncAttributeMaxDynamicSharedMemorySize, dw2_f16_lds_bytes<128>()));
            prepared_mask |= bit;
        }
    }
    if (H == 256) hipLaunchKernelGGL((k_dw2_f16<256>), dim3(slabs), dim3(512), dw2_f16_lds_bytes<256>(), s, a);
    else hipLaunchKernelGGL((k_dw2_f16<128>), dim3(slabs), dim3(512), dw2_f16_lds_bytes<128>(), s, a);
    hipLaunchKernelGGL(k_dw2_reduce, dim3((H * H + 255) / 256), dim3(256), 0, s, ws, dW2, H * H, H, ldc, slabs);
    HIP_TRY(hipGetLastError());
    return HD_OK;
}

static int vlb_check(const char* who, int device, int B, int N, int D, int int_nf, int cont_nf) {
    if (B < 1 || N < 1 || D < 4 || int_nf < 0 || cont_nf < 0 || 3 + int_nf + cont_nf > D)
        return fail(HD_E_INVALID, std::string(who) + ": bad shape (B, N >= 1, D >= 4, 3 + int_nf + cont_nf <= D)");
    if (hd_device_count() <= device || device < 0) return fail(HD_E_HIP, std::string(who) + ": no such HIP device (is a GPU visible?)");
    HIP_TRY(hipSetDevice(device));
    return HD_OK;
}

extern "C" int hd_vlb_loss_forward(int device, int B, int N, int D, int int_nf, int cont_nf, int l2_train, float T, float nv2, float nb2,
                                   float log_nv0, const float* net, const float* zt, const float* xh, const float* eps, const float* nm,
                                   const float* gam, const float* t_int, float* loss, float* err, void* stream) {
    HD_TRY(vlb_check("hd_vlb_loss_forward", device, B, N, D, int_nf, cont_nf));
    if (!net || !zt || !xh || !eps || !nm || !gam || !t_int || !loss || !err) return fail(HD_E_INVALID, "hd_vlb_loss_forward: null tensor");
    VlbArgs a;
    std::memset(&a, 0, sizeof(a));
    a.net = net; a.zt = zt; a.xh = xh; a.eps = eps; a.nm = nm; a.gam = gam; a.t_int = t_int; a.loss = loss; a.err = err;
    a.B = B; a.N = N; a.D = D; a.int_nf = int_nf; a.cont_nf = cont_nf; a.l2_train = l2_train; a.T = T; a.nv2 = nv2; a.nb2 = nb2; a.log_nv0 = log_nv0;
    hipLaunchKernelGGL((k_vlb<false>), dim3(B), dim3(256), 0, (hipStream_t)stream, a);
    HIP_TRY(hipGetLastError());
    return HD_OK;
}

extern "C" int hd_vlb_loss_backward(int device, int B, int N, int D, int int_nf, int cont_nf, int l2_train, float T, float nv2, float nb2,
                                    float log_nv0, const float* net, const float* zt, const float* xh, const float* eps, const float* nm,
                                    const float* gam, const float* t_int, const float* gout, float* dnet, float* dzt, float* dgam,
                                    void* stream) {
    HD_TRY(vlb_check("hd_vlb_loss_backward", device, B, N, D, int_nf, cont_nf));
    if (!net || !zt || !xh || !eps || !nm || !gam || !t_int || !gout || !dnet || !dzt || !dgam)
        return fail(HD_E_INVALID, "hd_vlb_loss_backward: null tensor");
    VlbArgs a;
    std::memset(&a, 0, sizeof(a));
    a.net = net; a.zt = zt; a.xh = xh; a.eps = eps; a.nm = nm; a.gam = gam; a.t_int = t_int; a.gout = gout; a.dnet = dnet; a.dzt = dzt; a.dgam = dgam;
    a.B = B; a.N = N; a.D = D; a.int_nf = int_nf; a.cont_nf = cont_nf; a.l2_train = l2_train; a.T = T; a.nv2 = nv2; a.nb2 = nb2; a.log_nv0 = log_nv0;
    hipLaunchKernelGGL((k_vlb<true>), dim3(B), dim3(256), 0, (hipStream_t)stream, a);
    HIP_TRY(hipGetLastError());
    return HD_OK;
}

extern "C" int hd_vlb_zt(int device, int B, int ND, const float* xh, const float* eps, const float* gt, float* zt, const float* dzt,
                         float* dgt, void* stream) {
    if (B < 1 || ND < 1 || !xh || !eps || !gt || (!dzt && !zt) || (dzt && !dgt)) return fail(HD_E_INVALID, "hd_vlb_zt: bad argument");
    if (hd_device_count() <= device || device < 0) return fail(HD_E_HIP, "hd_vlb_zt: no such HIP device (is a GPU visible?)");
    HIP_TRY(hipSetDevice(device));
    VlbZtArgs a{xh, eps, gt, zt, dzt, dgt, B, ND};
    if (dzt) hipLaunchKernelGGL((k_vlb_zt<true>), dim3(B), dim3(256), 0, (hipStream_t)stream, a);
    else hipLaunchKernelGGL((k_vlb_zt<false>), dim3(B), dim3(256), 0, (hipStream_t)stream, a);
    HIP_TRY(hipGetLastError());
    return HD_OK;
}

extern "C" int hd_edge_prep(int device, int H, int dir, float* W1, const float* b1, float* Wst, float* bst, float* wrd, void* stream) {
    if (H < 1 || !W1 || !Wst || !wrd || (dir == 0 && (!b1 || !bst))) return fail(HD_E_INVALID, "hd_edge_prep: bad argument");
    if (hd_device_count() <= device || device < 0) return fail(HD_E_HIP, "hd_edge_prep: no such HIP device (is a GPU visible?)");
    HIP_TRY(hipSetDevice(device));
    EdgePrepArgs a{W1, b1, Wst, bst, wrd, H};
    const dim3 grid((H * (2 * H + 2) + 255) / 256);
    if (dir == 0) hipLaunchKernelGGL((k_edge_prep<0>), grid, dim3(256), 0, (hipStream_t)stream, a);
    else hipLaunchKernelGGL((k_edge_prep<1>), grid, dim3(256), 0, (hipStream_t)stream, a);
    HIP_TRY(hipGetLastError());
    return HD_OK;
}

extern "C" int hd_colsum_f32(int device, int rows, int n, const float* const* src, const int* width, float* const* dst,
                             float* ws, void* stream) {
    if (n < 1 || n > 4 || !src || !width || !dst || !ws) return fail(HD_E_INVALID, "hd_colsum_f32: 1..4 arrays, a workspace");
    if (rows < 0) return fail(HD_E_INVALID, "hd_colsum_f32: rows < 0");
    if (hd_device_count() <= device || device < 0) return fail(HD_E_HIP, "hd_colsum_f32: no such HIP device (is a GPU visible?)");
    HIP_TRY(hipSetDevice(device));
    ColSumArgs a;
    std::memset(&a, 0, sizeof(a));
    a.rows = rows; a.n = n; a.ws = ws;
    for (int i = 0; i < n; ++i) {
        if (!src[i] || !dst[i] || width[i] < 1) return fail(HD_E_INVALID, "hd_colsum_f32: null array / width < 1");
        a.src[i] = src[i]; a.dst[i] = dst[i]; a.width[i] = width[i]; a.off[i + 1] = a.off[i] + width[i];
    }
    const int total = a.off[n];
    hipStream_t s = (hipStream_t)stream;
    hipLaunchKernelGGL(k_colsum_stage1, dim3((total + 63) / 64, CS_CHUNKS), dim3(256), 0, s, a);
    hipLaunchKernelGGL(k_colsum_stage2, dim3((total + 255) / 256), dim3(256), 0, s, a);
    HIP_TRY(hipGetLastError());
    return HD_OK;
}

static std::mutex g_digest_mu;
static unsigned long long* g_digest_host[64] = {nullptr};

extern "C" int hd_params_digest(int device, const void* const* ptrs_dev, const long long* prefix_dev, int n, long long total,
                                unsigned long long* state_dev, unsigned long long* digest_host, void* stream) {
    if (!ptrs_dev || !prefix_dev || !state_dev || !digest_host) return fail(HD_E_INVALID, "hd_params_digest: null argument");
    if (n < 1 || total < 0) return fail(HD_E_INVALID, "hd_params_digest: n < 1 or total < 0");
    if (hd_device_count() <= device || device < 0 || device >= 64) return fail(HD_E_HIP, "hd_params_digest: no such HIP device (is a GPU visible?)");
    HIP_TRY(hipSetDevice(device));
    hipStream_t s = (hipStream_t)stream;
    if (total == 0) { *digest_host = 0; return HD_OK; }
    std::lock_guard<std::mutex> lk(g_digest_mu);
    if (!g_digest_host[device]) HIP_TRY(hipHostMalloc(reinterpret_cast<void**>(&g_digest_host[device]), 64, hipHostMallocDefault));
    DigestArgs a;
    a.ptrs = reinterpret_cast<const uint32_t* const*>(ptrs_dev); a.prefix = prefix_dev; a.n = n; a.total = total;
    a.state = state_dev; a.host_out = g_digest_host[device];
    const long long groups = (total + DIGEST_CHUNK - 1) / DIGEST_CHUNK;
    hipLaunchKernelGGL(k_params_digest, dim3((unsigned)groups), dim3(256), 0, s, a);
    HIP_TRY(hipGetLastError());
    HIP_TRY(hipStreamSynchronize(s));
    *digest_host = *reinterpret_cast<volatile unsigned long long*>(g_digest_host[device]);
    return HD_OK;
}


static NoiseSrc make_noise(const float* raw_x, const float* raw_h, int rows, uint64_t seed, uint64_t base,
                           uint32_t draw, int share) {
    NoiseSrc n;
    n.raw_x = raw_x; n.raw_h = raw_h; n.rows = rows; n.seed = seed; n.sample_base = base; n.draw = draw; n.share = share;
    return n;
}

static int step_impl(hd_handle* h, hd_topology* t, const float* zt, const float* eps, const float* coef, int coef_rows,
                     const NoiseSrc& ns, int mol, float* zs, int out_stride, const int* step_ptr,
                     const uint32_t* draw_ptr, uint32_t draw0, hipStream_t s, const unsigned long long* base_ptr = nullptr) {
    ProfScope ps(h, s, 2);
    StepArgs a;
    a.zt = zt; a.eps = eps; a.coef = coef; a.nm = t->nm_bytes; a.zs = zs; a.noise = ns; a.draw_ptr = draw_ptr;
    a.step_ptr = step_ptr; a.base_ptr = base_ptr; a.draw0 = draw0; a.coef_rows = coef_rows; a.B = t->B; a.N = t->N; a.D = h->D; a.F = h->F;
    a.mol = mol; a.out_stride = out_stride;
    hipLaunchKernelGGL(k_post_step, dim3(t->B), dim3(256), (size_t)a.mol * a.D * sizeof(float), s, a);
    HIP_TRY(hipGetLastError());
    return HD_OK;
}

extern "C" int hd_posterior_step(hd_handle* h, hd_topology* topo, const float* zt, const float* eps, const float* coef,
                                 int coef_rows, const float* raw_x, const float* raw_h, int noise_rows, int mol_shape,
                                 float* zs, void* stream) {
    if (!h || !topo) return fail(HD_E_INVALID, "hd_posterior_step: null handle/topology");
    if (!zt || !eps || !coef || !raw_x || !raw_h || !zs) return fail(HD_E_INVALID, "hd_posterior_step: null tensor");
    if (coef_rows != 1 && coef_rows != topo->B) return fail(HD_E_INVALID, "hd_posterior_step: coef_rows must be 1 or B");
    if (noise_rows != 1 && noise_rows != topo->B) return fail(HD_E_INVALID, "hd_posterior_step: noise_rows must be 1 or B");
    const int mol = (mol_shape < 0 || mol_shape > topo->N) ? topo->N : mol_shape;
    if (zs == zt && mol != topo->N) return fail(HD_E_INVALID, "hd_posterior_step: in-place needs mol_shape == N");
    HIP_TRY(hipSetDevice(h->device));
    topo_use(topo, (hipStream_t)stream);
    return step_impl(h, topo, zt, eps, coef, coef_rows, make_noise(raw_x, raw_h, noise_rows, 0, 0, 0, 0), mol, zs, mol,
                     nullptr, nullptr, 0, (hipStream_t)stream);
}

extern "C" int hd_final_decode(hd_handle* h, hd_topology* topo, const float* z0, const float* eps, const float* coef3,
                               const float* raw_x, const float* raw_h, int noise_rows, uint64_t seed,
                               uint64_t sample_id_base, uint32_t draw, int share_rows, float* x, float* hfeat,
                               void* stream) {
    if (!h || !topo) return fail(HD_E_INVALID, "hd_final_decode: null handle/topology");
    if (!z0 || !eps || !coef3 || !x || !hfeat) return fail(HD_E_INVALID, "hd_final_decode: null tensor");
    if ((raw_x == nullptr) != (raw_h == nullptr)) return fail(HD_E_INVALID, "hd_final_decode: raw_x and raw_h go together");
    if (raw_x && noise_rows != 1 && noise_rows != topo->B) return fail(HD_E_INVALID, "hd_final_decode: noise_rows must be 1 or B");
    HIP_TRY(hipSetDevice(h->device));
    hipStream_t s = (hipStream_t)stream;
    topo_use(topo, s);
    ProfScope ps(h, s, 2);
    DecodeArgs a;
    a.z0 = z0; a.eps = eps; a.nm = topo->nm_bytes; a.x = x; a.hfeat = hfeat;
    a.noise = make_noise(raw_x, raw_h, noise_rows, seed, sample_id_base, draw, share_rows);
    a.sigma_0 = coef3[0]; a.alpha_0 = coef3[1]; a.sigma_x = coef3[2];
    a.B = topo->B; a.N = topo->N; a.D = h->D; a.F = h->F;
    hipLaunchKernelGGL(k_final_decode, dim3((topo->B + 3) / 4), dim3(256), 0, s, a);
    HIP_TRY(hipGetLastError());
    return HD_OK;
}

extern "C" int hd_noise(hd_handle* h, hd_topology* topo, const float* raw_x, const float* raw_h, int noise_rows,
                        uint64_t seed, uint64_t sample_id_base, uint32_t draw, int share_rows, float* z, void* stream) {
    if (!h || !topo || !z) return fail(HD_E_INVALID, "hd_noise: null argument");
    if ((raw_x == nullptr) != (raw_h == nullptr)) return fail(HD_E_INVALID, "hd_noise: raw_x and raw_h go together");
    if (raw_x && noise_rows != 1 && noise_rows != topo->B) return fail(HD_E_INVALID, "hd_noise: noise_rows must be 1 or B");
    HIP_TRY(hipSetDevice(h->device));
    hipStream_t s = (hipStream_t)stream;
    topo_use(topo, s);
    ProfScope ps(h, s, 2);
    NoiseArgs a;
    a.nm = topo->nm_bytes; a.z = z; a.noise = make_noise(raw_x, raw_h, noise_rows, seed, sample_id_base, draw, share_rows);
    a.B = topo->B; a.N = topo->N; a.D = h->D; a.F = h->F;
    hipLaunchKernelGGL(k_noise, dim3((topo->B + 3) / 4), dim3(256), 0, s, a);
    HIP_TRY(hipGetLastError());
    return HD_OK;
}

extern "C" int hd_set_schedule(hd_handle* h, int T, const float* tau, const float* coef4) {
    if (!h || !tau || !coef4 || T < 1) return fail(HD_E_INVALID, "hd_set_schedule: bad argument");
    HIP_TRY(hipSetDevice(h->device));
    HIP_TRY(hipDeviceSynchronize());
    hipFree(h->d_tau); hipFree(h->d_coef);
    h->d_tau = h->d_coef = nullptr;
    h->tau_h.assign(tau, tau + T + 1);
    h->coef_h.assign(coef4, coef4 + (size_t)4 * T);
    HD_TRY(dev_upload(&h->d_tau, h->tau_h));
    HD_TRY(dev_upload(&h->d_coef, h->coef_h));
    h->T = T;
    h->sched_gen++;
    return HD_OK;
}

extern "C" int hd_sample_loop(hd_handle* h, hd_topology* topo, float* z, const float* context, int mol_shape,
                              int s_hi, int s_lo, const float* raw_x, const float* raw_h, int noise_rows,
                              uint64_t seed, uint64_t sample_id_base, int use_graph, void* stream) {
    HD_TRY(check_ready(h, topo, "hd_sample_loop"));
    if (h->T < 1) return fail(HD_E_STATE, "hd_sample_loop: schedule not set (hd_set_schedule)");
    if (!z) return fail(HD_E_INVALID, "hd_sample_loop: null z");
    if (s_hi > h->T || s_lo < 0 || s_lo > s_hi) return fail(HD_E_INVALID, "hd_sample_loop: need 0 <= s_lo <= s_hi <= T");
    if ((raw_x == nullptr) != (raw_h == nullptr)) return fail(HD_E_INVALID, "hd_sample_loop: raw_x and raw_h go together");
    if (noise_rows != 1 && noise_rows != topo->B) return fail(HD_E_INVALID, "hd_sample_loop: noise_rows must be 1 or B");
    if (h->cfg.context_node_nf > 0 && !context) return fail(HD_E_INVALID, "hd_sample_loop: context required");
    if (!h->cfg.condition_time) return fail(HD_E_INVALID, "hd_sample_loop: needs a time-conditioned model");
    const int mol = (mol_shape < 0 || mol_shape > topo->N) ? topo->N : mol_shape;
    HIP_TRY(hipSetDevice(h->device));
    hipStream_t s = (hipStream_t)stream;
    const int nsteps = s_hi - s_lo;
    topo_use(topo, s);
    if (nsteps == 0) return HD_OK;
    const int T = h->T;
    const uint32_t draw0 = (uint32_t)(T - (s_hi - 1));
    const int share = (noise_rows == 1) ? 1 : 0;
    if (!use_graph) {
        for (int k = 0; k < nsteps; ++k) {
            const int sidx = s_hi - 1 - k;
            HD_TRY(forward_impl(h, topo, z, h->d_tau + sidx + 1, 1, context, mol_shape < 0 ? -1 : mol, topo->eps, s));
            NoiseSrc ns = make_noise(raw_x ? raw_x + (size_t)k * noise_rows * mol * 3 : nullptr,
                                     raw_h ? raw_h + (size_t)k * noise_rows * mol * h->F : nullptr, noise_rows, seed,
                                     sample_id_base, draw0 + (uint32_t)k, share);
            HD_TRY(step_impl(h, topo, z, topo->eps, h->d_coef + (size_t)sidx * 4, 1, ns, mol, z, topo->N, nullptr, nullptr, 0, s));
        }
        return HD_OK;
    }
    const size_t zbytes = (size_t)topo->B * topo->N * h->D * sizeof(float);
    const size_t cbytes = (size_t)topo->B * topo->N * h->cfg.context_node_nf * sizeof(float);
    hipStream_t rs = s;
    if (s == nullptr) {
        if (!h->own_stream) HIP_TRY(hipStreamCreateWithFlags(&h->own_stream, hipStreamNonBlocking));
        rs = h->own_stream;
        HIP_TRY(hipEventRecord(h->ev_in, s));
        HIP_TRY(hipStreamWaitEvent(rs, h->ev_in, 0));
    }
    GraphKey key;
    key.raw_x = raw_x; key.raw_h = raw_h; key.has_ctx = context ? 1 : 0; key.mol_shape = mol_shape < 0 ? -1 : mol;
    key.noise_rows = noise_rows; key.T = T; key.s_hi = raw_x ? s_hi : 0; key.seed = seed; key.weights_gen = h->weights_gen; key.sched_gen = h->sched_gen;
    if (h->ev_last_set) HIP_TRY(hipStreamWaitEvent(rs, h->ev_last, 0));
    if (topo->gexec && !(topo->gkey == key)) {
        if (h->ev_last_set) HIP_TRY(hipEventSynchronize(h->ev_last));
        HIP_TRY(hipStreamSynchronize(rs));
        hipGraphExecDestroy(topo->gexec);
        topo->gexec = nullptr;
    }
    if (!topo->gexec) {
        const int was_prof = h->prof;
        h->prof = 0;
        hipGraph_t graph = nullptr;
        HIP_TRY(hipStreamBeginCapture(rs, hipStreamCaptureModeThreadLocal));
        int rc = forward_impl(h, topo, topo->zbuf, h->d_tcur, 1, context ? topo->ctxbuf : nullptr, mol_shape < 0 ? -1 : mol,
                              topo->eps, rs);
        if (rc == HD_OK) {
            NoiseSrc ns = make_noise(raw_x, raw_h, noise_rows, seed, 0, draw0, share);
            rc = step_impl(h, topo, topo->zbuf, topo->eps, h->d_coef, 1, ns, mol, topo->zbuf, topo->N, h->d_step, h->d_draw,
                           draw0, rs, h->d_base);
        }
        if (rc == HD_OK) hipLaunchKernelGGL(k_advance, dim3(1), dim3(1), 0, rs, h->d_step, h->d_draw, h->d_tcur, h->d_tau);
        const hipError_t ce = hipStreamEndCapture(rs, &graph);
        h->prof = was_prof;
        if (rc != HD_OK) { if (graph) hipGraphDestroy(graph); return rc; }
        if (ce != hipSuccess) return fail(HD_E_HIP, std::string("hipStreamEndCapture: ") + hipGetErrorString(ce));
        const hipError_t ie = hipGraphInstantiate(&topo->gexec, graph, nullptr, nullptr, 0);
        hipGraphDestroy(graph);
        if (ie != hipSuccess) { topo->gexec = nullptr; return fail(HD_E_HIP, std::string("hipGraphInstantiate: ") + hipGetErrorString(ie)); }
        topo->gkey = key;
    }
    HIP_TRY(hipMemcpyAsync(topo->zbuf, z, zbytes, hipMemcpyDeviceToDevice, rs));
    if (context) HIP_TRY(hipMemcpyAsync(topo->ctxbuf, context, cbytes, hipMemcpyDeviceToDevice, rs));
    hipLaunchKernelGGL(k_loop_state, dim3(1), dim3(1), 0, rs, h->d_step, h->d_draw, h->d_tcur, h->d_base, h->d_tau,
                       s_hi - 1, draw0, (unsigned long long)sample_id_base);
    for (int k = 0; k < nsteps; ++k) {
        const hipError_t le = hipGraphLaunch(topo->gexec, rs);
        if (le != hipSuccess) return fail(HD_E_HIP, std::string("hipGraphLaunch: ") + hipGetErrorString(le));
    }
    HIP_TRY(hipMemcpyAsync(z, topo->zbuf, zbytes, hipMemcpyDeviceToDevice, rs));
    HIP_TRY(hipEventRecord(h->ev_last, rs));
    h->ev_last_set = true;
    if (rs != s) {
        HIP_TRY(hipEventRecord(h->ev_out, rs));
        HIP_TRY(hipStreamWaitEvent(s, h->ev_out, 0));
    }
    return HD_OK;
}


extern "C" int hd_set_inpaint_schedule(hd_handle* h, int T, const float* coef4) {
    if (!h || !coef4 || T < 1) return fail(HD_E_INVALID, "hd_set_inpaint_schedule: bad argument");
    if (h->T < 1) return fail(HD_E_STATE, "hd_set_inpaint_schedule: schedule not set (hd_set_schedule)");
    if (T != h->T) return fail(HD_E_INVALID, "hd_set_inpaint_schedule: T differs from the schedule's (hd_set_schedule)");
    HIP_TRY(hipSetDevice(h->device));
    HIP_TRY(hipDeviceSynchronize());
    hipFree(h->d_coef_ip);
    h->d_coef_ip = nullptr;
    h->ip_sched_gen = 0;
    const std::vector<float> rows(coef4, coef4 + (size_t)4 * T);
    HD_TRY(dev_upload(&h->d_coef_ip, rows));
    h->ip_sched_gen = h->sched_gen;
    h->ip_gen++;
    return HD_OK;
}

static int inpaint_launch(hd_handle* h, hd_topology* t, bool jump, float* z, const uint8_t* fixed, const float* known, uint64_t seed,
                          uint64_t base, uint32_t draw, int step, const uint32_t* draw_ptr, const int* step_ptr,
                          const unsigned long long* base_ptr, hipStream_t s) {
    ProfScope ps(h, s, 2);
    InpaintArgs a;
    a.z = z; a.nm = t->nm_bytes; a.fixed = fixed; a.known = known; a.coef = h->d_coef_ip; a.seed = seed; a.sample_base = base;
    a.draw = draw; a.step = step; a.draw_ptr = draw_ptr; a.step_ptr = step_ptr; a.base_ptr = base_ptr;
    a.B = t->B; a.N = t->N; a.D = h->D;
    const size_t lds = (size_t)t->N * h->D * sizeof(float);
    if (jump) hipLaunchKernelGGL(k_inpaint_jump, dim3(t->B), dim3(256), lds, s, a);
    else hipLaunchKernelGGL(k_inpaint_replace, dim3(t->B), dim3(256), lds, s, a);
    HIP_TRY(hipGetLastError());
    return HD_OK;
}

extern "C" int hd_sample_loop_inpaint(hd_handle* h, hd_topology* topo, float* z, const float* context, int mol_shape,
                                      int s_hi, int s_lo, const float* raw_x, const float* raw_h, int noise_rows,
                                      uint64_t seed, uint64_t sample_id_base, int use_graph, const uint8_t* fixed_mask,
                                      const float* xh_known, int resamplings, void* stream) {
    HD_TRY(check_ready(h, topo, "hd_sample_loop_inpaint"));
    if (h->T < 1) return fail(HD_E_STATE, "hd_sample_loop_inpaint: schedule not set (hd_set_schedule)");
    if (!h->d_coef_ip || h->ip_sched_gen != h->sched_gen)
        return fail(HD_E_STATE, "hd_sample_loop_inpaint: inpainting schedule not set for the current schedule (hd_set_inpaint_schedule)");
    if (!z || !fixed_mask || !xh_known) return fail(HD_E_INVALID, "hd_sample_loop_inpaint: null z / fixed_mask / xh_known");
    if (s_hi > h->T || s_lo < 0 || s_lo > s_hi) return fail(HD_E_INVALID, "hd_sample_loop_inpaint: need 0 <= s_lo <= s_hi <= T");
    if (raw_x || raw_h) return fail(HD_E_INVALID, "hd_sample_loop_inpaint: injected noise is not supported (counter-based generator only)");
    if (noise_rows != topo->B) return fail(HD_E_INVALID, "hd_sample_loop_inpaint: noise_rows must be B");
    if (mol_shape >= 0 && mol_shape < topo->N) return fail(HD_E_INVALID, "hd_sample_loop_inpaint: fixed tail rows (mol_shape < N) are not supported");
    if (resamplings < 1) return fail(HD_E_INVALID, "hd_sample_loop_inpaint: resamplings must be >= 1");
    if (h->cfg.context_node_nf > 0 && !context) return fail(HD_E_INVALID, "hd_sample_loop_inpaint: context required");
    if (!h->cfg.condition_time) return fail(HD_E_INVALID, "hd_sample_loop_inpaint: needs a time-conditioned model");
    const int T = h->T, R = resamplings, nd = 3 * R;
    const uint32_t stride = (uint32_t)T + 2u;
    if ((unsigned long long)stride * (unsigned long long)nd > 0xffffffffULL)
        return fail(HD_E_INVALID, "hd_sample_loop_inpaint: (T + 2) * 3 * resamplings exceeds the 32-bit draw index");
    if ((size_t)topo->N * h->D * sizeof(float) > 64 * 1024) return fail(HD_E_INVALID, "hd_sample_loop_inpaint: N * D floats exceed one workgroup's LDS");
    HIP_TRY(hipSetDevice(h->device));
    hipStream_t s = (hipStream_t)stream;
    const int nsteps = s_hi - s_lo;
    topo_use(topo, s);
    if (nsteps == 0) return HD_OK;
    const int N = topo->N;
    const uint32_t draw0 = (uint32_t)(T - (s_hi - 1));
    if (!use_graph) {
        for (int k = 0; k < nsteps; ++k) {
            const int sidx = s_hi - 1 - k;
            const uint32_t d = draw0 + (uint32_t)k;
            for (int j = 0; j < R; ++j) {
                HD_TRY(forward_impl(h, topo, z, h->d_tau + sidx + 1, 1, context, -1, topo->eps, s));
                NoiseSrc ns = make_noise(nullptr, nullptr, noise_rows, seed, sample_id_base, stride * (uint32_t)(3 * j) + d, 0);
                HD_TRY(step_impl(h, topo, z, topo->eps, h->d_coef + (size_t)sidx * 4, 1, ns, N, z, N, nullptr, nullptr, 0, s));
                HD_TRY(inpaint_launch(h, topo, false, z, fixed_mask, xh_known, seed, sample_id_base, stride * (uint32_t)(3 * j + 1) + d,
                                      sidx, nullptr, nullptr, nullptr, s));
                if (j < R - 1)
                    HD_TRY(inpaint_launch(h, topo, true, z, nullptr, nullptr, seed, sample_id_base, stride * (uint32_t)(3 * j + 2) + d,
                                          sidx, nullptr, nullptr, nullptr, s));
            }
        }
        return HD_OK;
    }
    const size_t BN = (size_t)topo->B * N;
    const size_t zbytes = BN * h->D * sizeof(float);
    const size_t cbytes = BN * h->cfg.context_node_nf * sizeof(float);
    hipStream_t rs = s;
    if (s == nullptr) {
        if (!h->own_stream) HIP_TRY(hipStreamCreateWithFlags(&h->own_stream, hipStreamNonBlocking));
        rs = h->own_stream;
        HIP_TRY(hipEventRecord(h->ev_in, s));
        HIP_TRY(hipStreamWaitEvent(rs, h->ev_in, 0));
    }
    if (h->ev_last_set) HIP_TRY(hipStreamWaitEvent(rs, h->ev_last, 0));
    if (nd > h->ipdraw_cap) {
        if (h->ev_last_set) HIP_TRY(hipEventSynchronize(h->ev_last));
        HIP_TRY(hipStreamSynchronize(rs));
        hipFree(h->d_ipdraw);
        h->d_ipdraw = nullptr; h->ipdraw_cap = 0;
        HD_TRY(dev_alloc(&h->d_ipdraw, (size_t)nd));
        h->ipdraw_cap = nd;
        h->ip_gen++;
    }
    if (!topo->ip_fixed) HIP_TRY(hipMalloc(reinterpret_cast<void**>(&topo->ip_fixed), BN));
    if (!topo->ip_known) HIP_TRY(hipMalloc(reinterpret_cast<void**>(&topo->ip_known), zbytes));
    InpaintKey key;
    key.has_ctx = context ? 1 : 0; key.T = T; key.resamplings = R; key.seed = seed; key.weights_gen = h->weights_gen;
    key.sched_gen = h->sched_gen; key.ip_gen = h->ip_gen;
    if (topo->gexec_ip && !(topo->ikey == key)) {
        if (h->ev_last_set) HIP_TRY(hipEventSynchronize(h->ev_last));
        HIP_TRY(hipStreamSynchronize(rs));
        hipGraphExecDestroy(topo->gexec_ip);
        topo->gexec_ip = nullptr;
    }
    if (!topo->gexec_ip) {
        const int was_prof = h->prof;
        h->prof = 0;
        hipGraph_t graph = nullptr;
        HIP_TRY(hipStreamBeginCapture(rs, hipStreamCaptureModeThreadLocal));
        int rc = HD_OK;
        for (int j = 0; j < R && rc == HD_OK; ++j) {
            rc = forward_impl(h, topo, topo->zbuf, h->d_tcur, 1, context ? topo->ctxbuf : nullptr, -1, topo->eps, rs);
            if (rc == HD_OK) {
                NoiseSrc ns = make_noise(nullptr, nullptr, noise_rows, seed, 0, 0, 0);
                rc = step_impl(h, topo, topo->zbuf, topo->eps, h->d_coef, 1, ns, N, topo->zbuf, N, h->d_step, h->d_ipdraw + 3 * j,
                               0, rs, h->d_base);
            }
            if (rc == HD_OK)
                rc = inpaint_launch(h, topo, false, topo->zbuf, topo->ip_fixed, topo->ip_known, seed, 0, 0, 0, h->d_ipdraw + 3 * j + 1,
                                    h->d_step, h->d_base, rs);
            if (rc == HD_OK && j < R - 1)
                rc = inpaint_launch(h, topo, true, topo->zbuf, nullptr, nullptr, seed, 0, 0, 0, h->d_ipdraw + 3 * j + 2, h->d_step,
                                    h->d_base, rs);
        }
        if (rc == HD_OK) {
            hipLaunchKernelGGL(k_advance, dim3(1), dim3(1), 0, rs, h->d_step, h->d_draw, h->d_tcur, h->d_tau);
            hipLaunchKernelGGL(k_inpaint_advance, dim3((nd + 255) / 256), dim3(256), 0, rs, h->d_ipdraw, nd);
        }
        const hipError_t ce = hipStreamEndCapture(rs, &graph);
        h->prof = was_prof;
        if (rc != HD_OK) { if (graph) hipGraphDestroy(graph); return rc; }
        if (ce != hipSuccess) return fail(HD_E_HIP, std::string("hipStreamEndCapture: ") + hipGetErrorString(ce));
        const hipError_t ie = hipGraphInstantiate(&topo->gexec_ip, graph, nullptr, nullptr, 0);
        hipGraphDestroy(graph);
        if (ie != hipSuccess) { topo->gexec_ip = nullptr; return fail(HD_E_HIP, std::string("hipGraphInstantiate: ") + hipGetErrorString(ie)); }
        topo->ikey = key;
    }
    HIP_TRY(hipMemcpyAsync(topo->zbuf, z, zbytes, hipMemcpyDeviceToDevice, rs));
    if (context) HIP_TRY(hipMemcpyAsync(topo->ctxbuf, context, cbytes, hipMemcpyDeviceToDevice, rs));
    HIP_TRY(hipMemcpyAsync(topo->ip_fixed, fixed_mask, BN, hipMemcpyDeviceToDevice, rs));
    HIP_TRY(hipMemcpyAsync(topo->ip_known, xh_known, zbytes, hipMemcpyDeviceToDevice, rs));
    hipLaunchKernelGGL(k_loop_state, dim3(1), dim3(1), 0, rs, h->d_step, h->d_draw, h->d_tcur, h->d_base, h->d_tau,
                       s_hi - 1, draw0, (unsigned long long)sample_id_base);
    hipLaunchKernelGGL(k_inpaint_state, dim3((nd + 255) / 256), dim3(256), 0, rs, h->d_ipdraw, nd, stride, draw0);
    for (int k = 0; k < nsteps; ++k) {
        const hipError_t le = hipGraphLaunch(topo->gexec_ip, rs);
        if (le != hipSuccess) return fail(HD_E_HIP, std::string("hipGraphLaunch: ") + hipGetErrorString(le));
    }
    HIP_TRY(hipMemcpyAsync(z, topo->zbuf, zbytes, hipMemcpyDeviceToDevice, rs));
    HIP_TRY(hipEventRecord(h->ev_last, rs));
    h->ev_last_set = true;
    if (rs != s) {
        HIP_TRY(hipEventRecord(h->ev_out, rs));
        HIP_TRY(hipStreamWaitEvent(s, h->ev_out, 0));
    }
    return HD_OK;
}

extern "C" int hd_inpaint_decode_fix(hd_handle* h, hd_topology* topo, const uint8_t* fixed_mask, const float* x_known,
                                     const float* h_known, float* x, float* hfeat, void* stream) {
    if (!h || !topo) return fail(HD_E_INVALID, "hd_inpaint_decode_fix: null handle/topology");
    if (topo->h != h) return fail(HD_E_INVALID, "hd_inpaint_decode_fix: topology belongs to another handle");
    if (!fixed_mask || !x_known || !h_known || !x || !hfeat) return fail(HD_E_INVALID, "hd_inpaint_decode_fix: null tensor");
    HIP_TRY(hipSetDevice(h->device));
    hipStream_t s = (hipStream_t)stream;
    topo_use(topo, s);
    ProfScope ps(h, s, 2);
    InpaintFixArgs a;
    a.nm = topo->nm_bytes; a.fixed = fixed_mask; a.x_known = x_known; a.h_known = h_known; a.x = x; a.hfeat = hfeat;
    a.B = topo->B; a.N = topo->N; a.F = h->F;
    hipLaunchKernelGGL(k_inpaint_decode_fix, dim3((topo->B + 3) / 4), dim3(256), 0, s, a);
    HIP_TRY(hipGetLastError());
    return HD_OK;
}

extern "C" int hd_mfma_probe(int device, int kind, const float* in1024, float* scratch, int iters, double* ns_per_mfma_per_simd,
                             void* stream) {
    if (!in1024 || !scratch || !ns_per_mfma_per_simd) return fail(HD_E_INVALID, "hd_mfma_probe: null argument");
    if (kind < 0 || kind > 1 || iters < 1) return fail(HD_E_INVALID, "hd_mfma_probe: kind must be 0 (fp32) or 1 (fp16), iters >= 1");
    if (hd_device_count() <= device || device < 0) return fail(HD_E_HIP, "hd_mfma_probe: no such HIP device (is a GPU visible?)");
    HIP_TRY(hipSetDevice(device));
    hipStream_t s = (hipStream_t)stream;
    hipDeviceProp_t prop;
    HIP_TRY(hipGetDeviceProperties(&prop, device));
    const int n_cu = prop.multiProcessorCount > 0 ? prop.multiProcessorCount : 256;
    const dim3 grid(2 * n_cu), block(256);
    auto launch = [&](int n) {
        if (kind == 0) hipLaunchKernelGGL((k_mfma_probe<0>), grid, block, 0, s, in1024, scratch, n);
        else hipLaunchKernelGGL((k_mfma_probe<1>), grid, block, 0, s, in1024, scratch, n);
    };
    hipEvent_t e0, e1;
    HIP_TRY(hipEventCreate(&e0));
    {
        const hipError_t ce = hipEventCreate(&e1);
        if (ce != hipSuccess) { (void)hipEventDestroy(e0); return fail(HD_E_HIP, std::string("hd_mfma_probe: ") + hipGetErrorString(ce)); }
    }
    launch(iters);
    (void)hipEventRecord(e0, s);
    launch(iters);
    (void)hipEventRecord(e1, s);
    const hipError_t se = hipEventSynchronize(e1);
    float ms = 0.f;
    if (se == hipSuccess) (void)hipEventElapsedTime(&ms, e0, e1);
    (void)hipEventDestroy(e0); (void)hipEventDestroy(e1);
    if (se != hipSuccess) return fail(HD_E_HIP, std::string("hd_mfma_probe: ") + hipGetErrorString(se));
    HIP_TRY(hipGetLastError());
    *ns_per_mfma_per_simd = (double)ms * 1e6 / ((double)iters * 8 * 2);
    return HD_OK;
}


struct EgclRaw {
    size_t W1, b1, W2, b2, We1, be1, We2, be2, Wn1, bn1, Wn2, bn2, Wc1, bc1, wc2, wa, ba;
};

static EgclRaw egcl_raw_offsets(const hd_egcl_config& c) {
    const size_t H = c.hidden_nf, De = c.edges_in_d, ctx = c.context_nf;
    EgclRaw R;
    std::memset(&R, 0, sizeof(R));
    size_t o = 0;
    auto take = [&](size_t n) { size_t r = o; o += n; return r; };
    R.W1 = take(H * (2 * H + 1 + De + ctx)); R.b1 = take(H); R.W2 = take(H * H); R.b2 = take(H);
    if (c.edge_update) { R.We1 = take(H * (H + 1 + De)); R.be1 = take(H); R.We2 = take(H * H); R.be2 = take(H); }
    R.Wn1 = take(2 * H * H); R.bn1 = take(H); R.Wn2 = take(H * H); R.bn2 = take(H);
    if (c.coord_update) { R.Wc1 = take(H * H); R.bc1 = take(H); R.wc2 = take(H); }
    if (c.attention) { R.wa = take(H); R.ba = take(1); }
    return R;
}

constexpr int EGCL_MAX_SPLIT = 32;

extern "C" int hd_egcl_backward(hd_egcl* g, hd_egcl_graph* t, const float* h, const float* x, const float* edge_attr,
                                const float* node_mask, const float* edge_mask, const float* saved, const float* dh_out,
                                const float* dx_out, const float* dedge_attr_out, float* dh, float* dx, float* dedge_attr,
                                float* dweights, void* stream) {
    if (!g || !t) return fail(HD_E_INVALID, "hd_egcl_backward: null handle/graph");
    if (t->g != g) return fail(HD_E_INVALID, "hd_egcl_backward: graph belongs to another handle");
    if (!g->weights_set) return fail(HD_E_STATE, "hd_egcl_backward: weights not set (hd_egcl_set_weights)");
    if (!h || !x || !saved || !dh || !dx || !dweights) return fail(HD_E_INVALID, "hd_egcl_backward: null tensor");
    const hd_egcl_config& c = g->cfg;
    if (g->De > 0 && !edge_attr) return fail(HD_E_INVALID, "hd_egcl_backward: edge_attr required");
    HIP_TRY(hipSetDevice(g->device));
    hipStream_t s = (hipStream_t)stream;
    const int H = g->H, De = g->De, ctx = g->ctx, M = t->M, E = t->E, W = H + ctx;
    const int ld1 = 2 * H + 1 + De + ctx, lde = H + 1 + De;
    const float* Wt = g->dw + g->raw;
    const EgclRaw R = egcl_raw_offsets(c);
    const EgclSaved SL = egcl_saved_layout(g, M, E);
    auto S = [&](size_t off) { return saved + off; };
    const size_t Ep = t->Ep, Mp = t->Mp, EH = Ep * H, MH = Mp * H;
    const size_t wsf = (size_t)EGCL_MAX_SPLIT * (2 * (size_t)H * H + 2 * H);
    const size_t need = 7 * EH + 8 * Ep + 9 * MH + 4 * MH + 4 * Mp + wsf;
    if (t->bw_floats < need) {
        hipFree(t->bw); t->bw = nullptr; t->bw_floats = 0;
        HD_TRY(dev_alloc(&t->bw, need));
        t->bw_floats = need;
    }
    float* p = t->bw;
    auto take = [&](size_t n) { float* r = p; p += n; return r; };
    float* B[7];
    for (int i = 0; i < 7; ++i) B[i] = take(EH);
    float *escal = take(4 * Ep), *sc4 = take(4 * Ep);
    float *X = take(2 * MH), *pn = take(MH), *Tn = take(MH), *dout = take(MH), *dpn = take(MH), *dX = take(2 * MH), *dAB = take(2 * MH);
    float *T2 = take(MH), *Tc = take(MH), *dxs = take(4 * Mp), *ws = take(wsf);
    auto blocks = [](long long total) { return dim3((unsigned)((total + 255) / 256)); };
    const dim3 wave_grid((unsigned)((E + 3) / 4)), wave_block(256);
    auto mm = [&](int rows, int N, int K, const float* A, long long sam, long long sak, const float* Bm, long long sbk, long long sbn,
                  float* C, int ldc, const float* bias, int epi, const float* aux, float* C2) {
        return hd_gemm_f32(g->device, rows, N, K, A, sam, sak, Bm, sbk, sbn, C, ldc, bias, epi, aux, nullptr, C2, 1, nullptr, nullptr, s);
// ... 214 lines not shown
```

### hierdiff_amd/csrc/k_edge.hpp

```cpp
#pragma once
#include "common.hpp"


#ifndef HD_X6_SILU
#define HD_X6_SILU silu_fast
#endif
#ifndef HD_F32_SILU
#define HD_F32_SILU silu_fast
#endif

struct EdgeArgs {
    const float* AB;
    const float* wrd;
    const float* W2img;
    const float* b2;
    const float* wa;
    const int* ei;
    const int* ej;
    const uint8_t* eseg;
    const int* seg_part;
    const int* tile_nseg;
    const float* xcur;
    const float* x0;
    float* part;
    float ba;
    const float* ba_ptr;
    float norm_constant;
    float coords_range;
    int attention, use_tanh;
    int n_tiles, n_wg;
    long long* trace;
    float w2s_inv;
    float wrmax, wdmax;
    const float* abmax;
    const float* dscal;
    float* pre2;
};

constexpr int HD_EDGE_SAVE = 256;
constexpr int HD_EDGE_UNSCALED = 512;
constexpr float HD_NEG_LOG2E = -1.4426950408889634f;


struct AbMaxArgs { const float* AB; float* out; int M, H; };
__global__ void __launch_bounds__(256) k_ab_rowmax(AbMaxArgs a) {
    const int row = blockIdx.x * 4 + (threadIdx.x >> 6), lane = threadIdx.x & 63;
    if (row >= a.M) return;
    const float* r = a.AB + (size_t)row * 2 * a.H;
    float ma = 0.f, mb = 0.f;
    for (int k = 4 * lane; k < a.H; k += 256) {
        const f32x4 va = *reinterpret_cast<const f32x4*>(r + k), vb = *reinterpret_cast<const f32x4*>(r + a.H + k);
#pragma unroll
        for (int j = 0; j < 4; ++j) { ma = fmaxf(ma, fabsf(va[j])); mb = fmaxf(mb, fabsf(vb[j])); }
    }
#pragma unroll
    for (int o = 32; o > 0; o >>= 1) { ma = fmaxf(ma, __shfl_xor(ma, o)); mb = fmaxf(mb, __shfl_xor(mb, o)); }
    if (lane == 0) { a.out[2 * (size_t)row] = ma; a.out[2 * (size_t)row + 1] = mb; }
}


template <typename V, unsigned O0, unsigned O1, unsigned O2, unsigned O3>
HD_DEVINL void lds_read4(V (&f)[4], unsigned addr) {
    asm volatile("ds_read_b128 %0, %4 offset:%5\n\t"
                 "ds_read_b128 %1, %4 offset:%6\n\t"
                 "ds_read_b128 %2, %4 offset:%7\n\t"
                 "ds_read_b128 %3, %4 offset:%8"
                 : "=&v"(f[0]), "=&v"(f[1]), "=&v"(f[2]), "=&v"(f[3])
                 : "v"(addr), "i"(O0), "i"(O1), "i"(O2), "i"(O3));
}
template <int N, typename V>
HD_DEVINL void lds_wait4(V (&f)[4]) {
    asm volatile("s_waitcnt lgkmcnt(%4)" : "+v"(f[0]), "+v"(f[1]), "+v"(f[2]), "+v"(f[3]) : "i"(N));
}

template <typename V, unsigned O0, unsigned O1>
HD_DEVINL void lds_read2f(V (&f)[2], unsigned addr) {
    asm volatile("ds_read_b128 %0, %2 offset:%3\n\tds_read_b128 %1, %2 offset:%4" : "=&v"(f[0]), "=&v"(f[1]) : "v"(addr), "i"(O0), "i"(O1));
}
template <int N, typename V>
HD_DEVINL void lds_wait2f(V (&f)[2]) { asm volatile("s_waitcnt lgkmcnt(%2)" : "+v"(f[0]), "+v"(f[1]) : "i"(N)); }

HD_DEVINL float xhalf_sum(float x) {
    float lo = x, hi = x;
    asm("s_nop 1\n\tv_permlane32_swap_b32 %0, %1\n\ts_nop 1" : "+v"(lo), "+v"(hi));
    return lo + hi;
}
HD_DEVINL void xhalf_sum4(float (&x)[4]) {
    float lo[4], hi[4];
#pragma unroll
    for (int k = 0; k < 4; ++k) { lo[k] = x[k]; hi[k] = x[k]; }
    asm("s_nop 1\n\t"
        "v_permlane32_swap_b32 %0, %4\n\tv_permlane32_swap_b32 %1, %5\n\t"
        "v_permlane32_swap_b32 %2, %6\n\tv_permlane32_swap_b32 %3, %7\n\t"
        "s_nop 1"
        : "+v"(lo[0]), "+v"(lo[1]), "+v"(lo[2]), "+v"(lo[3]), "+v"(hi[0]), "+v"(hi[1]), "+v"(hi[2]), "+v"(hi[3]));
#pragma unroll
    for (int k = 0; k < 4; ++k) x[k] = lo[k] + hi[k];
}

HD_DEVINL void vm_load2(f32x4& va, f32x4& vb, const float* pa, const float* pb) {
    asm volatile("global_load_dwordx4 %0, %2, off\n\t"
                 "global_load_dwordx4 %1, %3, off"
                 : "=&v"(va), "=&v"(vb) : "v"(pa), "v"(pb));
}
template <int OFF>
HD_DEVINL void vm_load2o(f32x4& va, f32x4& vb, const float* pa, const float* pb) {
    static_assert(OFF >= 0 && OFF < 4096, "immediate offset out of range");
    asm volatile("global_load_dwordx4 %0, %2, off offset:%4\n\t"
                 "global_load_dwordx4 %1, %3, off offset:%4"
                 : "=&v"(va), "=&v"(vb) : "v"(pa), "v"(pb), "i"(OFF));
}
HD_DEVINL void vm_glds2(const float* ga, const float* gb, unsigned lds_a, unsigned lds_b) {
    unsigned keep;
    asm volatile("s_mov_b32 %0, m0\n\t"
                 "s_mov_b32 m0, %3\n\ts_nop 0\n\tglobal_load_lds_dwordx4 %1, off\n\t"
                 "s_mov_b32 m0, %4\n\ts_nop 0\n\tglobal_load_lds_dwordx4 %2, off\n\t"
                 "s_mov_b32 m0, %0"
                 : "=&s"(keep) : "v"(ga), "v"(gb), "s"(lds_a), "s"(lds_b));
}
template <int N, unsigned OA, unsigned OB>
HD_DEVINL void lds_read2_after_vm(f32x4& qa, f32x4& qb, unsigned addr) {
    asm volatile("s_waitcnt vmcnt(%3)\n\t"
                 "ds_read_b128 %0, %2 offset:%4\n\t"
                 "ds_read_b128 %1, %2 offset:%5"
                 : "=&v"(qa), "=&v"(qb) : "v"(addr), "i"(N), "i"(OA), "i"(OB));
}
HD_DEVINL void lds_ready2(f32x4& qa, f32x4& qb) { asm volatile("s_waitcnt lgkmcnt(0)" : "+v"(qa), "+v"(qb)); }

template <int N>
HD_DEVINL void vm_wait2(f32x4& va, f32x4& vb) {
    asm volatile("s_waitcnt vmcnt(%2)" : "+v"(va), "+v"(vb) : "i"(N));
}

template <int NCT>
constexpr unsigned frag_off_bf(int u, int hl) { return (unsigned)((((hl * 2 + u / NCT) * NCT + u % NCT) * 64) * 16); }
constexpr unsigned frag_off_f32(int u) { return (unsigned)(u * 64 * 16); }
template <int NCT>
constexpr unsigned frag_off_x6(int p, int ct) { return (unsigned)((p * NCT + ct) * 64 * 16); }

template <int H, bool COORD, int PREC, int ABL>
HD_DEVINL void edge_tile_body(const EdgeArgs& a, float* smem, float* wrd_s, const int bid, const int nwt) {
    constexpr int NCT = H / 32;
    constexpr int KC = PREC == 2 ? 16 : 32;
    constexpr int NCH = H / KC;
    constexpr int CHF = PREC == 2 ? 24 * H : 32 * H;
    static_assert(CHF % 1024 == 0, "a chunk image is streamed in 1 KiB pieces, four waves");
    constexpr int GL_PER_WAVE = (ABL & 128) ? CHF / (4 * 256) / 4 : CHF / (4 * 256);
    float* wbuf = smem;
    float* scratch = smem + 2 * CHF + 2 * H;

    const int tid = threadIdx.x, lane = tid & 63;
    const int wave = __builtin_amdgcn_readfirstlane(tid >> 6);
    const int hh = lane >> 5, n = lane & 31;
    float* my_scr = scratch + wave * 136;
    uint32_t* seg_s = reinterpret_cast<uint32_t*>(my_scr + 128);

    int wt;
    {
        const int xcd = bid & 7, slot = bid >> 3;
        const int q = nwt >> 3, r = nwt & 7;
        const int start = xcd < r ? xcd * (q + 1) : r * (q + 1) + (xcd - r) * q;
        const int len = q + (xcd < r ? 1 : 0);
        if (slot >= len) return;
        wt = start + slot;
    }
    long long ts0 = 0, ts1 = 0, ts2 = 0, ts3 = 0, ts4 = 0, ts5 = 0;
    if constexpr (ABL & 16) ts0 = __builtin_readcyclecounter();

    for (int k = tid; k < 2 * H; k += 256) wrd_s[k] = a.wrd[k];
    for (int k = tid; k < H; k += 256) { wrd_s[2 * H + k] = a.b2[k]; wrd_s[3 * H + k] = a.wa[k]; }
    auto issue_chunk = [&](int c, int buf) {
        const float* src = a.W2img + (size_t)c * CHF + wave * (GL_PER_WAVE * 256) + lane * 4;
        float* dst = wbuf + buf * CHF + wave * (GL_PER_WAVE * 256);
        static_for<0, GL_PER_WAVE>([&](auto U) {
            constexpr int u = decltype(U)::value;
            glds16o<(u & 3) * 1024>(src + (u >> 2) * 1024, dst + (u >> 2) * 1024);
        });
    };
    issue_chunk(0, 0);

    const int tile = wt * 4 + wave;
    const bool tile_ok = tile < a.n_tiles;
    int ni = 0, nj = 0;
    uint32_t segb = 255;
    if (tile_ok) {
        const int e = tile * 32 + n;
        ni = a.ei[e]; nj = a.ej[e]; segb = a.eseg[e];
    }

    int gc = 0;
    f32x4 xi = *reinterpret_cast<const f32x4*>(a.xcur + (size_t)ni * 4);
    f32x4 xj = *reinterpret_cast<const f32x4*>(a.xcur + (size_t)nj * 4);
    f32x4 yi = *reinterpret_cast<const f32x4*>(a.x0 + (size_t)ni * 4);
    f32x4 yj = *reinterpret_cast<const f32x4*>(a.x0 + (size_t)nj * 4);
    const float dx = xi[0] - xj[0], dy = xi[1] - xj[1], dz = xi[2] - xj[2];
    const float radial = dx * dx + dy * dy + dz * dz;
    if constexpr (COORD) {
        if (hh == 0) {
            const float inv = ((segb != 255) ? 1.0f : 0.0f) / (sqrtf(radial + 1e-8f) + a.norm_constant);
            float* tr = my_scr + 32;
            tr[n * 3 + 0] = dx * inv; tr[n * 3 + 1] = dy * inv; tr[n * 3 + 2] = dz * inv;
        }
    }
    const float ex = yi[0] - yj[0], ey = yi[1] - yj[1], ez = yi[2] - yj[2];
    const float d0 = ex * ex + ey * ey + ez * ez;
    const uint32_t segb_t = segb;
    float f16_inv = 1.0f;
    if constexpr (PREC == 3) {
        const float nodes = a.abmax[2 * (size_t)ni] + a.abmax[2 * (size_t)nj + 1] + HD_F16_FLOOR;
        const float wrmax = (ABL & HD_EDGE_UNSCALED) ? a.dscal[2] : a.wrmax, wdmax = (ABL & HD_EDGE_UNSCALED) ? a.dscal[3] : a.wdmax;
        const float bound = __builtin_fmaf(radial, wrmax, __builtin_fmaf(d0, wdmax, nodes));
        const uint32_t eb = (__builtin_bit_cast(uint32_t, bound) >> 23) & 0xffu;
        f16_inv = __builtin_bit_cast(float, (eb - 13u) << 23);
        if (hh == 0) my_scr[n] = f16_inv * ((ABL & HD_EDGE_UNSCALED) ? a.dscal[1] : a.w2s_inv);
    }
    const int pid_l = tile_ok ? a.seg_part[tile * 32 + n] : 0;
    const int nseg = tile_ok ? a.tile_nseg[tile] : 0;
    if (hh == 0) reinterpret_cast<uint8_t*>(seg_s)[n] = (uint8_t)segb_t;

    const float* Arow = a.AB + (size_t)ni * (2 * H) + (KC / 2) * hh;
    const float* Brow = a.AB + (size_t)nj * (2 * H) + H + (KC / 2) * hh;
    f32x4 pa[4], pb[4];
    auto rows_issue = [&](int u, int c) {
        if constexpr (ABL & 8) { pa[u] = f32x4{radial, d0, radial, d0}; pb[u] = pa[u]; }
        else vm_load2(pa[u], pb[u], Arow + KC * c + 4 * u, Brow + KC * c + 4 * u);
    };
    auto make_P = [&](int c, float (&P)[16]) {
#pragma unroll
        for (int u = 0; u < 4; ++u) {
            f32x4 wr4 = *reinterpret_cast<const f32x4*>(wrd_s + 32 * c + 16 * hh + 4 * u);
            f32x4 wd4 = *reinterpret_cast<const f32x4*>(wrd_s + H + 32 * c + 16 * hh + 4 * u);
#pragma unroll
            for (int j = 0; j < 4; ++j) {
                float pre = pa[u][j] + pb[u][j];
                pre = __builtin_fmaf(radial, wr4[j], pre);
                pre = __builtin_fmaf(d0, wd4[j], pre);
                P[4 * u + j] = HD_F32_SILU(pre);
            }
        }
    };
    auto make_quad = [&](f32x4 av, f32x4 bv, f32x4 wr4, f32x4 wd4, uint32_t (&hi)[2], uint32_t (&lo)[2]) {
        float pre[4], e[4];
#pragma unroll
        for (int j = 0; j < 4; ++j) pre[j] = av[j] + bv[j];
#pragma unroll
        for (int j = 0; j < 4; ++j) pre[j] = __builtin_fmaf(radial, wr4[j], pre[j]);
#pragma unroll
        for (int j = 0; j < 4; ++j) pre[j] = __builtin_fmaf(d0, wd4[j], pre[j]);
        if constexpr (ABL & 2) {
            bf16_split2(av[0], av[1], hi[0], lo[0]);
            bf16_split2(av[2], av[3], hi[1], lo[1]);
            return;
        }
#pragma unroll
        for (int j = 0; j < 4; ++j) e[j] = __builtin_amdgcn_exp2f((ABL & HD_EDGE_UNSCALED) ? pre[j] * HD_NEG_LOG2E : pre[j]);
#pragma unroll
        for (int j = 0; j < 4; ++j) e[j] = PREC == 3 ? __builtin_fmaf(e[j], f16_inv, f16_inv) : 1.0f + e[j];
#pragma unroll
        for (int j = 0; j < 4; ++j) e[j] = __builtin_amdgcn_rcpf(e[j]);
#pragma unroll
        for (int j = 0; j < 4; ++j) pre[j] *= e[j];
        split2<PREC == 3>(pre[0], pre[1], hi[0], lo[0]);
        split2<PREC == 3>(pre[2], pre[3], hi[1], lo[1]);
    };
    auto make_P_bf = [&](int c, u32x4 (&ph)[2], u32x4 (&pl)[2]) {
#pragma unroll
        for (int u = 0; u < 4; ++u) {
            const f32x4 wr4 = *reinterpret_cast<const f32x4*>(wrd_s + 32 * c + 16 * hh + 4 * u);
            const f32x4 wd4 = *reinterpret_cast<const f32x4*>(wrd_s + H + 32 * c + 16 * hh + 4 * u);
            uint32_t hi[2], lo[2];
            make_quad(pa[u], pb[u], wr4, wd4, hi, lo);
            ph[u >> 1][2 * (u & 1)] = hi[0]; ph[u >> 1][2 * (u & 1) + 1] = hi[1];
            pl[u >> 1][2 * (u & 1)] = lo[0]; pl[u >> 1][2 * (u & 1) + 1] = lo[1];
        }
    };

    auto make_quad_x6 = [&](f32x4 av, f32x4 bv, f32x4 wr4, f32x4 wd4, uint32_t (&hi)[2], uint32_t (&mi)[2], uint32_t (&lo)[2]) {
        float y[4];
#pragma unroll
        for (int j = 0; j < 4; ++j) {
            float pre = av[j] + bv[j];
            pre = __builtin_fmaf(radial, wr4[j], pre);
            pre = __builtin_fmaf(d0, wd4[j], pre);
            y[j] = (ABL & 2) ? pre : HD_X6_SILU(pre);
        }
        if constexpr (ABL & 2) {
            hi[0] = mi[0] = lo[0] = __builtin_bit_cast(uint32_t, y[0] + y[1]); hi[1] = mi[1] = lo[1] = __builtin_bit_cast(uint32_t, y[2] + y[3]);
            return;
        }
        bf16_split3(y[0], y[1], hi[0], mi[0], lo[0]);
        bf16_split3(y[2], y[3], hi[1], mi[1], lo[1]);
    };
    float Pc[16];
    u32x4 phc[2], plc[2];
    constexpr int NQ = KC / 8;
    u32x4 xh, xm, xl;
#pragma unroll
    for (int u = 0; u < NQ; ++u) rows_issue(u, 0);
    if constexpr (NQ == 4) asm volatile("s_waitcnt vmcnt(0)" : "+v"(pa[0]), "+v"(pa[1]), "+v"(pa[2]), "+v"(pa[3]),
                                                              "+v"(pb[0]), "+v"(pb[1]), "+v"(pb[2]), "+v"(pb[3]));
    else asm volatile("s_waitcnt vmcnt(0)" : "+v"(pa[0]), "+v"(pa[1]), "+v"(pb[0]), "+v"(pb[1]));
    __syncthreads();
    if constexpr (PREC == 0) make_P(0, Pc);
    else if constexpr (HD_TWOWAY(PREC)) make_P_bf(0, phc, plc);
    else {
#pragma unroll
        for (int u = 0; u < 2; ++u) {
            const f32x4 wr4 = *reinterpret_cast<const f32x4*>(wrd_s + 8 * hh + 4 * u);
            const f32x4 wd4 = *reinterpret_cast<const f32x4*>(wrd_s + H + 8 * hh + 4 * u);
            uint32_t hi[2], mi[2], lo[2];
            make_quad_x6(pa[u], pb[u], wr4, wd4, hi, mi, lo);
            xh[2 * u] = hi[0]; xh[2 * u + 1] = hi[1]; xm[2 * u] = mi[0]; xm[2 * u + 1] = mi[1]; xl[2 * u] = lo[0]; xl[2 * u + 1] = lo[1];
        }
    }
#pragma unroll
    for (int u = 0; u < NQ; ++u) rows_issue(u, NCH > 1 ? 1 : 0);

    #ifdef HD_NO_PEEL
    constexpr bool PEEL = false;
#else
    constexpr bool PEEL = PREC == 3 && !(ABL & 2) && !(ABL & 1024);
#endif
    f32x16 acc[NCT];
    if constexpr (!PEEL) {
#pragma unroll
        for (int ct = 0; ct < NCT; ++ct) {
            const float b2v = PREC == 3 ? 0.0f : wrd_s[2 * H + 32 * ct + n];
#pragma unroll
            for (int r = 0; r < 16; ++r) acc[ct][r] = b2v;
        }
    }
    if constexpr (ABL & 16) ts1 = __builtin_readcyclecounter();
    auto chunk = [&](auto First, const int c) {
        constexpr bool FIRST = decltype(First)::value;
        const int buf = (ABL & 4) ? 0 : (gc & 1);
        if constexpr (!(ABL & 4) && !(ABL & 64)) {
            if constexpr (PREC == 2) { if (c > 0) asm volatile("s_waitcnt vmcnt(4)\n\ts_barrier" ::: "memory"); }
            else if (c > 0) asm volatile("s_waitcnt vmcnt(8)\n\ts_barrier" ::: "memory");
        }
        u32x4 phn[2], pln[2];
        const int cn1 = c + 1 < NCH ? c + 1 : NCH - 1, cn2 = c + 2 < NCH ? c + 2 : NCH - 1;
        const float* Arow_n2 = Arow + KC * cn2;
        const float* Brow_n2 = Brow + KC * cn2;
        const float* wb = wbuf + buf * CHF;
        const unsigned wb_lds = (unsigned)(size_t)(__attribute__((address_space(3))) const void*)wb + lane * 16;
// ... 236 lines not shown
#pragma unroll
            for (int r = 0; r < 16; ++r) e[r] = __builtin_amdgcn_exp2f((ABL & HD_EDGE_UNSCALED) ? acc[ct][r] * HD_NEG_LOG2E : acc[ct][r]);
            __builtin_amdgcn_sched_barrier(0);
#pragma unroll
            for (int r = 0; r < 16; ++r) e[r] = 1.0f + e[r];
            __builtin_amdgcn_sched_barrier(0);
#pragma unroll
            for (int r = 0; r < 16; ++r) e[r] = __builtin_amdgcn_rcpf(e[r]);
            __builtin_amdgcn_sched_barrier(0);
#pragma unroll
            for (int r = 0; r < 16; ++r) acc[ct][r] *= e[r];
            __builtin_amdgcn_sched_barrier(0);
#pragma unroll
            for (int r = 0; r < 16; ++r) dot[r] = __builtin_fmaf(acc[ct][r], wav, dot[r]);
            __builtin_amdgcn_sched_barrier(0);
        }
    }
    if constexpr (ABL & 16) ts3 = __builtin_readcyclecounter();
    float rowdot;
    {
        float v8[8], v4[4], v2[2];
        const bool b4 = n & 16, b3 = n & 8, b2_ = n & 4, b1 = n & 2;
#pragma unroll
        for (int k = 0; k < 8; ++k) {
            const float send = b4 ? dot[k] : dot[k + 8];
            const float keep = b4 ? dot[k + 8] : dot[k];
            v8[k] = keep + __shfl_xor(send, 16);
        }
#pragma unroll
        for (int k = 0; k < 4; ++k) {
            const float send = b3 ? v8[k] : v8[k + 4];
            const float keep = b3 ? v8[k + 4] : v8[k];
            v4[k] = keep + __shfl_xor(send, 8);
        }
#pragma unroll
        for (int k = 0; k < 2; ++k) {
            const float send = b2_ ? v4[k] : v4[k + 2];
            const float keep = b2_ ? v4[k + 2] : v4[k];
            v2[k] = keep + __shfl_xor(send, 4);
        }
        {
            const float send = b1 ? v2[0] : v2[1];
            const float keep = b1 ? v2[1] : v2[0];
            rowdot = keep + __shfl_xor(send, 2);
        }
        rowdot += __shfl_xor(rowdot, 1);
    }
    if constexpr (ABL & 16) ts4 = __builtin_readcyclecounter();
    const int my_slot = (n >> 1) & 15;

    if (!COORD) {
        uint32_t sw[4];
#pragma unroll
        for (int q = 0; q < 4; ++q) sw[q] = seg_s[2 * q + hh];
        float att_mine = 1.0f;
        if (a.attention) {
            const float ba = a.ba_ptr ? *a.ba_ptr : a.ba;
            if constexpr (!HD_TWOWAY(PREC)) att_mine = sigmoid_f(rowdot + ba);
            else att_mine = __builtin_amdgcn_rcpf(1.0f + __builtin_amdgcn_exp2f((ABL & HD_EDGE_UNSCALED) ? (rowdot + ba) * HD_NEG_LOG2E : rowdot + ba));
        }
        float w[16];
        int sg[16];
#pragma unroll
        for (int r = 0; r < 16; ++r) {
            sg[r] = (sw[r >> 2] >> (8 * (r & 3))) & 255;
            const float att = __shfl(att_mine, (lane & 32) | (2 * r));
            w[r] = (sg[r] != 255) ? att : 0.0f;
        }
        if constexpr (ABL & 16) ts5 = __builtin_readcyclecounter();
        const bool tile_has_nan = __builtin_amdgcn_ballot_w64(rowdot != rowdot) != 0;
        for (int s = 0; s < nseg; ++s) {
            float ws[16];
#pragma unroll
            for (int r = 0; r < 16; ++r) ws[r] = (sg[r] == s) ? w[r] : 0.0f;
            float* dst = a.part + (size_t)__builtin_amdgcn_readlane(pid_l, s) * H + n;
            float sums[NCT];
            if (__builtin_expect(tile_has_nan, 0)) {
#pragma unroll
                for (int ct = 0; ct < NCT; ++ct) {
                    float sum = 0.f;
#pragma unroll
                    for (int r = 0; r < 16; ++r) sum = (sg[r] == s) ? __builtin_fmaf(ws[r], acc[ct][r], sum) : sum;
                    sums[ct] = sum;
                }
            } else {
#pragma unroll
                for (int ct = 0; ct < NCT; ++ct) {
                    float sum = 0.f;
#pragma unroll
                    for (int r = 0; r < 16; ++r) sum = __builtin_fmaf(ws[r], acc[ct][r], sum);
                    sums[ct] = sum;
                }
            }
            if constexpr (NCT % 4 == 0) {
#pragma unroll
                for (int c4 = 0; c4 < NCT; c4 += 4) {
                    float q4[4] = {sums[c4], sums[c4 + 1], sums[c4 + 2], sums[c4 + 3]};
                    xhalf_sum4(q4);
#pragma unroll
                    for (int k = 0; k < 4; ++k) sums[c4 + k] = q4[k];
                }
            } else {
#pragma unroll
                for (int ct = 0; ct < NCT; ++ct) sums[ct] = xhalf_sum(sums[ct]);
            }
            if (hh == 0) {
#pragma unroll
                for (int ct = 0; ct < NCT; ++ct) dst[32 * ct] = sums[ct];
            }
        }
    } else {
        if ((n & 1) == 0) my_scr[(my_slot & 3) + 8 * (my_slot >> 2) + 4 * hh] = rowdot;
        __builtin_amdgcn_wave_barrier();
        __builtin_amdgcn_fence(__ATOMIC_ACQ_REL, "wavefront");
        if (hh == 0) {
            float phi = my_scr[n];
            float sc = a.use_tanh ? tanhf(phi) * a.coords_range : phi;
            float* tr = my_scr + 32;
            tr[n * 3 + 0] *= sc;
            tr[n * 3 + 1] *= sc;
            tr[n * 3 + 2] *= sc;
        }
        __builtin_amdgcn_wave_barrier();
        __builtin_amdgcn_fence(__ATOMIC_ACQ_REL, "wavefront");
        if (lane < nseg) {
            const uint8_t* sb = reinterpret_cast<const uint8_t*>(seg_s);
            const float* tr = my_scr + 32;
            float sx = 0.f, sy = 0.f, sz = 0.f;
            for (int rr = 0; rr < 32; ++rr) {
                if (sb[rr] == lane) { sx += tr[rr * 3]; sy += tr[rr * 3 + 1]; sz += tr[rr * 3 + 2]; }
            }
            f32x4 o = {sx, sy, sz, 0.f};
            *reinterpret_cast<f32x4*>(a.part + (size_t)pid_l * 4) = o;
        }
        __builtin_amdgcn_wave_barrier();
        __builtin_amdgcn_fence(__ATOMIC_ACQ_REL, "wavefront");
    }
    if constexpr (ABL & 16) {
        if (lane == 0) {
            long long* t = a.trace + ((size_t)blockIdx.x * 4 + wave) * 8;
            const long long hw = __builtin_amdgcn_s_getreg((16 - 1) << 11 | 4) & 0xffff;
            const long long xcc = __builtin_amdgcn_s_getreg((4 - 1) << 11 | 20) & 0xf;
            t[0] = (ts0 & 0xffffffffffffll) | (hw << 48); t[1] = (ts1 & 0xffffffffffffll) | (xcc << 48);
            const long long m48 = 0xffffffffffffll;
            t[2] = ts2 & m48; t[3] = __builtin_readcyclecounter() & m48; t[4] = ts3 & m48; t[5] = ts4 & m48; t[6] = ts5 & m48; t[7] = nseg;
        }
    }
}

template <int H, bool COORD, int PREC, int ABL = 0>
__global__ __launch_bounds__(256, 2) void k_edge(EdgeArgs a) {
    extern __shared__ __attribute__((aligned(16))) float smem[];
    __shared__ __attribute__((aligned(16))) float wrd_s[4 * H];
    edge_tile_body<H, COORD, PREC, ABL>(a, smem, wrd_s, blockIdx.x, a.n_wg);
}
```

### hierdiff_amd/csrc/k_edge_split.hpp

```cpp
#pragma once
#include "k_edge.hpp"

template <int H, int PREC>
constexpr int edge_split_lds_bytes() {
    return (H / (PREC == 2 ? 16 : 32)) * (PREC == 2 ? 3 : 4) * 64 * 16 + (16 * 64 + 64 + 8 + 32 + 96 + 4 + 32) * 4;
}

template <int H, bool COORD, int PREC, bool DEEP>
HD_DEVINL void edge_split_body(const EdgeArgs& a, char* lds, float* wrd_s, const int tile) {
    constexpr int KC = PREC == 2 ? 16 : 32;
    constexpr int NCT = H / 32, NCW = NCT / 4, NCH = H / KC, CHF = PREC == 2 ? 24 * H : 32 * H, NQ = KC / 8;
    static_assert(NCT % 4 == 0, "column tiles are dealt to four wavefronts");
    constexpr int SL = PREC == 2 ? 3 : 4;
    u32x4* opnd_s = reinterpret_cast<u32x4*>(lds);
    float* dot_x = reinterpret_cast<float*>(lds + NCH * SL * 64 * 16);
    float* att_s = dot_x + 16 * 64;
    uint32_t* seg_s = reinterpret_cast<uint32_t*>(att_s + 64);
    float* cs_phi = reinterpret_cast<float*>(seg_s + 8);
    float* cs_tr = cs_phi + 32;
    int* nan_p = reinterpret_cast<int*>(cs_tr + 96);
    float* rs_s = reinterpret_cast<float*>(nan_p + 4);

    const int tid = threadIdx.x, lane = tid & 63;
    const int wave = __builtin_amdgcn_readfirstlane(tid >> 6);
    const int hh = lane >> 5, n = lane & 31;

    for (int k = tid; k < 2 * H; k += 256) wrd_s[k] = a.wrd[k];
    for (int k = tid; k < H; k += 256) { wrd_s[2 * H + k] = a.b2[k]; wrd_s[3 * H + k] = a.wa[k]; }

    const int e = tile * 32 + n;
    const int ni = a.ei[e], nj = a.ej[e];
    const uint32_t segb = a.eseg[e];
    const f32x4 xi = *reinterpret_cast<const f32x4*>(a.xcur + (size_t)ni * 4);
    const f32x4 xj = *reinterpret_cast<const f32x4*>(a.xcur + (size_t)nj * 4);
    const f32x4 yi = *reinterpret_cast<const f32x4*>(a.x0 + (size_t)ni * 4);
    const f32x4 yj = *reinterpret_cast<const f32x4*>(a.x0 + (size_t)nj * 4);
    const float dx = xi[0] - xj[0], dy = xi[1] - xj[1], dz = xi[2] - xj[2];
    const float radial = dx * dx + dy * dy + dz * dz;
    const float ex = yi[0] - yj[0], ey = yi[1] - yj[1], ez = yi[2] - yj[2];
    const float d0 = ex * ex + ey * ey + ez * ez;
    const int pid_l = a.seg_part[tile * 32 + n];
    const int nseg = a.tile_nseg[tile];
    float f16_inv = 1.0f;
    if constexpr (PREC == 3) {
        const float nodes = a.abmax[2 * (size_t)ni] + a.abmax[2 * (size_t)nj + 1] + HD_F16_FLOOR;
        const float bound = __builtin_fmaf(radial, a.wrmax, __builtin_fmaf(d0, a.wdmax, nodes));
        const uint32_t eb = (__builtin_bit_cast(uint32_t, bound) >> 23) & 0xffu;
        f16_inv = __builtin_bit_cast(float, (eb - 13u) << 23);
        if (wave == 3 && hh == 0) rs_s[n] = f16_inv * a.w2s_inv;
    }
    if (wave == 3 && hh == 0) {
        reinterpret_cast<uint8_t*>(seg_s)[n] = (uint8_t)segb;
        if constexpr (COORD) {
            const float inv = ((segb != 255) ? 1.0f : 0.0f) / (sqrtf(radial + 1e-8f) + a.norm_constant);
            cs_tr[n * 3 + 0] = dx * inv; cs_tr[n * 3 + 1] = dy * inv; cs_tr[n * 3 + 2] = dz * inv;
        }
    }

    const float* Arow = a.AB + (size_t)ni * (2 * H) + (KC / 2) * hh;
    const float* Brow = a.AB + (size_t)nj * (2 * H) + H + (KC / 2) * hh;
    struct Raw { f32x4 a[NQ], b[NQ]; };
    auto load_raw = [&](int c, Raw& w) {
#pragma unroll
        for (int u = 0; u < NQ; ++u) {
            w.a[u] = *reinterpret_cast<const f32x4*>(Arow + KC * c + 4 * u);
            w.b[u] = *reinterpret_cast<const f32x4*>(Brow + KC * c + 4 * u);
        }
    };
    struct Opnd { float P[PREC == 0 ? 16 : 1]; u32x4 ph[2], pl[2], xh, xm, xl; };
    auto finish_P = [&](int c, const Raw& w, Opnd& o) {
#pragma unroll
        for (int u = 0; u < NQ; ++u) {
            const f32x4 wr4 = *reinterpret_cast<const f32x4*>(wrd_s + KC * c + (KC / 2) * hh + 4 * u);
            const f32x4 wd4 = *reinterpret_cast<const f32x4*>(wrd_s + H + KC * c + (KC / 2) * hh + 4 * u);
            if constexpr (PREC == 0) {
#pragma unroll
                for (int j = 0; j < 4; ++j) {
                    float pre = w.a[u][j] + w.b[u][j];
                    pre = __builtin_fmaf(radial, wr4[j], pre);
                    pre = __builtin_fmaf(d0, wd4[j], pre);
                    o.P[4 * u + j] = HD_F32_SILU(pre);
                }
            } else if constexpr (HD_TWOWAY(PREC)) {
                float pre[4], ev[4];
#pragma unroll
                for (int j = 0; j < 4; ++j) pre[j] = w.a[u][j] + w.b[u][j];
#pragma unroll
                for (int j = 0; j < 4; ++j) pre[j] = __builtin_fmaf(radial, wr4[j], pre[j]);
#pragma unroll
                for (int j = 0; j < 4; ++j) pre[j] = __builtin_fmaf(d0, wd4[j], pre[j]);
#pragma unroll
                for (int j = 0; j < 4; ++j) ev[j] = __builtin_amdgcn_exp2f(pre[j]);
#pragma unroll
                for (int j = 0; j < 4; ++j) ev[j] = PREC == 3 ? __builtin_fmaf(ev[j], f16_inv, f16_inv) : 1.0f + ev[j];
#pragma unroll
                for (int j = 0; j < 4; ++j) ev[j] = __builtin_amdgcn_rcpf(ev[j]);
#pragma unroll
                for (int j = 0; j < 4; ++j) pre[j] *= ev[j];
                uint32_t hi[2], lo[2];
                split2<PREC == 3>(pre[0], pre[1], hi[0], lo[0]);
                split2<PREC == 3>(pre[2], pre[3], hi[1], lo[1]);
                o.ph[u >> 1][2 * (u & 1)] = hi[0]; o.ph[u >> 1][2 * (u & 1) + 1] = hi[1];
                o.pl[u >> 1][2 * (u & 1)] = lo[0]; o.pl[u >> 1][2 * (u & 1) + 1] = lo[1];
            } else {
                float y[4];
#pragma unroll
                for (int j = 0; j < 4; ++j) {
                    float pre = w.a[u][j] + w.b[u][j];
                    pre = __builtin_fmaf(radial, wr4[j], pre);
                    pre = __builtin_fmaf(d0, wd4[j], pre);
                    y[j] = HD_X6_SILU(pre);
                }
                uint32_t hi[2], mi[2], lo[2];
                bf16_split3(y[0], y[1], hi[0], mi[0], lo[0]);
                bf16_split3(y[2], y[3], hi[1], mi[1], lo[1]);
                o.xh[2 * u] = hi[0]; o.xh[2 * u + 1] = hi[1]; o.xm[2 * u] = mi[0]; o.xm[2 * u + 1] = mi[1];
                o.xl[2 * u] = lo[0]; o.xl[2 * u + 1] = lo[1];
            }
        }
    };
    const int ct0 = wave * NCW;
    constexpr int NF = (PREC == 2 ? 3 : 4) * NCW;
    const char* wimg = reinterpret_cast<const char*>(a.W2img) + lane * 16;
    auto load_frags = [&](int c, u32x4 (&f)[NF]) {
        const char* base = wimg + (size_t)c * CHF * 4;
#pragma unroll
        for (int i = 0; i < NF; ++i) {
            const int x = i / NCW, k = i % NCW;
            unsigned off;
            if constexpr (PREC == 0) off = frag_off_f32(x * NCT + ct0 + k);
            else if constexpr (HD_TWOWAY(PREC)) off = (unsigned)(((((x >> 1) * 2 + (x & 1)) * NCT + ct0 + k) * 64) * 16);
            else off = (unsigned)((x * NCT + ct0 + k) * 64 * 16);
            f[i] = *reinterpret_cast<const u32x4*>(base + off);
        }
    };
    constexpr int RING0 = PREC == 0 ? 3 : (HD_TWOWAY(PREC) ? 4 : 6);
    constexpr int RING = DEEP ? (PREC == 0 ? 6 : (HD_TWOWAY(PREC) ? 6 : 8)) : RING0;
    u32x4 fr[RING][NF];
    static_for<0, (RING - 1 < NCH ? RING - 1 : NCH)>([&](auto Cc) { load_frags(decltype(Cc)::value, fr[decltype(Cc)::value]); });
    constexpr int CPW = NCH / 4;
    {
        Raw raw[CPW];
#pragma unroll
        for (int i = 0; i < CPW; ++i) load_raw(4 * i + wave, raw[i]);
        __syncthreads();
#pragma unroll
        for (int i = 0; i < CPW; ++i) {
            const int c = 4 * i + wave;
            Opnd o;
            finish_P(c, raw[i], o);
            u32x4* dst = opnd_s + (size_t)c * SL * 64 + lane;
            if constexpr (PREC == 0) {
#pragma unroll
                for (int q = 0; q < 4; ++q) dst[q * 64] = __builtin_bit_cast(u32x4, f32x4{o.P[4 * q], o.P[4 * q + 1], o.P[4 * q + 2], o.P[4 * q + 3]});
            } else if constexpr (HD_TWOWAY(PREC)) {
                dst[0] = o.ph[0]; dst[64] = o.ph[1]; dst[128] = o.pl[0]; dst[192] = o.pl[1];
            } else {
                dst[0] = o.xh; dst[64] = o.xm; dst[128] = o.xl;
            }
        }
    }
    __syncthreads();
    auto read_op = [&](int c, u32x4 (&v)[SL]) {
#pragma unroll
        for (int q = 0; q < SL; ++q) v[q] = opnd_s[((size_t)c * SL + q) * 64 + lane];
    };
    u32x4 opv[2][SL];
    read_op(0, opv[0]);
    f32x16 acc[NCW];
#pragma unroll
    for (int k = 0; k < NCW; ++k) {
        const float b2v = PREC == 3 ? 0.0f : wrd_s[2 * H + 32 * (ct0 + k) + n];
#pragma unroll
        for (int r = 0; r < 16; ++r) acc[k][r] = b2v;
    }
    static_for<0, NCH>([&](auto Cc) {
        constexpr int c = decltype(Cc)::value;
        if constexpr (c + RING - 1 < NCH) load_frags(c + RING - 1, fr[(c + RING - 1) % RING]);
        if constexpr (c + 1 < NCH) read_op(c + 1, opv[(c + 1) & 1]);
        u32x4(&f)[NF] = fr[c % RING];
        u32x4(&ov)[SL] = opv[c & 1];
        if constexpr (PREC == 0) {
#pragma unroll
            for (int q = 0; q < 4; ++q)
#pragma unroll
                for (int j = 0; j < 4; ++j)
#pragma unroll
// ... 35 lines not shown
        for (int k = 0; k < NCW; ++k) {
            const float b2v = wrd_s[2 * H + 32 * (ct0 + k) + n];
#pragma unroll
            for (int r = 0; r < 16; ++r) acc[k][r] = __builtin_fmaf(acc[k][r], rsc[r >> 2][r & 3], b2v);
        }
    }
#pragma unroll
    for (int k = 0; k < NCW; ++k)
#pragma unroll
        for (int r = 0; r < 16; ++r) {
            if constexpr (PREC == 0) acc[k][r] = HD_F32_SILU(acc[k][r]);
            else if constexpr (PREC == 2) acc[k][r] = HD_X6_SILU(acc[k][r]);
            else acc[k][r] = acc[k][r] * __builtin_amdgcn_rcpf(1.0f + __builtin_amdgcn_exp2f(acc[k][r]));
        }
    float dot[16];
#pragma unroll
    for (int r = 0; r < 16; ++r) dot[r] = 0.f;
    for (int w = 0; w < 4; ++w) {
        if (wave == w) {
            if (w > 0) {
#pragma unroll
                for (int r = 0; r < 16; ++r) dot[r] = dot_x[r * 64 + lane];
            }
#pragma unroll
            for (int k = 0; k < NCW; ++k) {
                const float wav = wrd_s[3 * H + 32 * (ct0 + k) + n];
#pragma unroll
                for (int r = 0; r < 16; ++r) dot[r] = __builtin_fmaf(acc[k][r], wav, dot[r]);
            }
            if (w < 3) {
#pragma unroll
                for (int r = 0; r < 16; ++r) dot_x[r * 64 + lane] = dot[r];
            }
        }
        __syncthreads();
    }
    if (wave == 3) {
        float rowdot;
        {
            float v8[8], v4[4], v2[2];
            const bool b4 = n & 16, b3 = n & 8, b2_ = n & 4, b1 = n & 2;
#pragma unroll
            for (int k = 0; k < 8; ++k) {
                const float send = b4 ? dot[k] : dot[k + 8];
                const float keep = b4 ? dot[k + 8] : dot[k];
                v8[k] = keep + __shfl_xor(send, 16);
            }
#pragma unroll
            for (int k = 0; k < 4; ++k) {
                const float send = b3 ? v8[k] : v8[k + 4];
                const float keep = b3 ? v8[k + 4] : v8[k];
                v4[k] = keep + __shfl_xor(send, 8);
            }
#pragma unroll
            for (int k = 0; k < 2; ++k) {
                const float send = b2_ ? v4[k] : v4[k + 2];
                const float keep = b2_ ? v4[k + 2] : v4[k];
                v2[k] = keep + __shfl_xor(send, 4);
            }
            {
                const float send = b1 ? v2[0] : v2[1];
                const float keep = b1 ? v2[1] : v2[0];
                rowdot = keep + __shfl_xor(send, 2);
            }
            rowdot += __shfl_xor(rowdot, 1);
        }
        const int my_slot = (n >> 1) & 15;
        if constexpr (!COORD) {
            float att_mine = 1.0f;
            if (a.attention) {
                const float ba = a.ba_ptr ? *a.ba_ptr : a.ba;
                if constexpr (!HD_TWOWAY(PREC)) att_mine = sigmoid_f(rowdot + ba);
                else att_mine = __builtin_amdgcn_rcpf(1.0f + __builtin_amdgcn_exp2f(rowdot + ba));
            }
            att_s[lane] = att_mine;
            const bool tile_has_nan = __builtin_amdgcn_ballot_w64(rowdot != rowdot) != 0;
            if (lane == 0) *nan_p = tile_has_nan ? 1 : 0;
        } else {
            if ((n & 1) == 0) cs_phi[(my_slot & 3) + 8 * (my_slot >> 2) + 4 * hh] = rowdot;
            __builtin_amdgcn_wave_barrier();
            __builtin_amdgcn_fence(__ATOMIC_ACQ_REL, "wavefront");
            if (hh == 0) {
                const float phi = cs_phi[n];
                const float sc = a.use_tanh ? tanhf(phi) * a.coords_range : phi;
                cs_tr[n * 3 + 0] *= sc;
                cs_tr[n * 3 + 1] *= sc;
                cs_tr[n * 3 + 2] *= sc;
            }
            __builtin_amdgcn_wave_barrier();
            __builtin_amdgcn_fence(__ATOMIC_ACQ_REL, "wavefront");
            if (lane < nseg) {
                const uint8_t* sb = reinterpret_cast<const uint8_t*>(seg_s);
                float sx = 0.f, sy = 0.f, sz = 0.f;
                for (int rr = 0; rr < 32; ++rr) {
                    if (sb[rr] == lane) { sx += cs_tr[rr * 3]; sy += cs_tr[rr * 3 + 1]; sz += cs_tr[rr * 3 + 2]; }
                }
                const f32x4 o = {sx, sy, sz, 0.f};
                *reinterpret_cast<f32x4*>(a.part + (size_t)pid_l * 4) = o;
            }
        }
    }
    if constexpr (COORD) return;
    __syncthreads();
    {
        uint32_t sw[4];
#pragma unroll
        for (int q = 0; q < 4; ++q) sw[q] = seg_s[2 * q + hh];
        float w[16];
        int sg[16];
#pragma unroll
        for (int r = 0; r < 16; ++r) {
            sg[r] = (sw[r >> 2] >> (8 * (r & 3))) & 255;
            const float att = att_s[(lane & 32) | (2 * r)];
            w[r] = (sg[r] != 255) ? att : 0.0f;
        }
        const bool tile_has_nan = *nan_p != 0;
        for (int s = 0; s < nseg; ++s) {
            float ws[16];
#pragma unroll
            for (int r = 0; r < 16; ++r) ws[r] = (sg[r] == s) ? w[r] : 0.0f;
            float* dst = a.part + (size_t)__builtin_amdgcn_readlane(pid_l, s) * H + 32 * ct0 + n;
            float sums[NCW];
            if (__builtin_expect(tile_has_nan, 0)) {
#pragma unroll
                for (int k = 0; k < NCW; ++k) {
                    float sum = 0.f;
#pragma unroll
                    for (int r = 0; r < 16; ++r) sum = (sg[r] == s) ? __builtin_fmaf(ws[r], acc[k][r], sum) : sum;
                    sums[k] = sum;
                }
            } else {
#pragma unroll
                for (int k = 0; k < NCW; ++k) {
                    float sum = 0.f;
#pragma unroll
                    for (int r = 0; r < 16; ++r) sum = __builtin_fmaf(ws[r], acc[k][r], sum);
                    sums[k] = sum;
                }
            }
#pragma unroll
            for (int k = 0; k < NCW; ++k) sums[k] = xhalf_sum(sums[k]);
            if (hh == 0) {
#pragma unroll
                for (int k = 0; k < NCW; ++k) dst[32 * k] = sums[k];
            }
        }
    }
}

template <int H, bool COORD, int PREC>
__global__ __launch_bounds__(256) void k_edge_split(EdgeArgs a) {
    __shared__ __attribute__((aligned(16))) float wrd_s[4 * H];
    __shared__ __attribute__((aligned(16))) char lds[edge_split_lds_bytes<H, PREC>()];
    edge_split_body<H, COORD, PREC, true>(a, lds, wrd_s, blockIdx.x);
}

template <int H, bool COORD, int PREC>
__global__ __launch_bounds__(256, 2) void k_edge_mixed(EdgeArgs a) {
    extern __shared__ __attribute__((aligned(16))) float smem[];
    __shared__ __attribute__((aligned(16))) float wrd_s[4 * H];
    const int bid = blockIdx.x;
    if (bid < a.n_wg) edge_tile_body<H, COORD, PREC, 0>(a, smem, wrd_s, bid, a.n_wg);
    else edge_split_body<H, COORD, PREC, false>(a, reinterpret_cast<char*>(smem), wrd_s, 4 * a.n_wg + (bid - a.n_wg));
}
```

### hierdiff_amd/csrc/k_sampling.hpp

```cpp
#pragma once
#include "common.hpp"


struct XupdArgs {
    const float* part;
    const int* pstart;
    const float* nmask;
    float* xcur;
    float norm;
    int M;
};

__global__ void k_xupd(XupdArgs a) {
    int i = blockIdx.x * blockDim.x + threadIdx.x;
    if (i >= a.M) return;
    float sx = 0.f, sy = 0.f, sz = 0.f;
    for (int p = a.pstart[i]; p < a.pstart[i + 1]; ++p) {
        f32x4 v = *reinterpret_cast<const f32x4*>(a.part + (size_t)p * 4);
        sx += v[0]; sy += v[1]; sz += v[2];
    }
    float m = a.nmask[i];
    f32x4 x = *reinterpret_cast<const f32x4*>(a.xcur + (size_t)i * 4);
    x[0] = (x[0] + sx / a.norm) * m;
    x[1] = (x[1] + sy / a.norm) * m;
    x[2] = (x[2] + sz / a.norm) * m;
    *reinterpret_cast<f32x4*>(a.xcur + (size_t)i * 4) = x;
}

struct AggArgs {
    const float* part;
    const int* pstart;
    float* agg;
    float norm;
    int M, H;
};

__global__ void k_agg(AggArgs a) {
    const int q = a.H >> 2;
    const int idx = blockIdx.x * blockDim.x + threadIdx.x;
    const int i = idx / q, c4 = idx - i * q;
    if (i >= a.M) return;
    f32x4 v = {0.f, 0.f, 0.f, 0.f};
    for (int p = a.pstart[i]; p < a.pstart[i + 1]; ++p) v += *reinterpret_cast<const f32x4*>(a.part + (size_t)p * a.H + 4 * c4);
    *reinterpret_cast<f32x4*>(a.agg + (size_t)i * a.H + 4 * c4) = v / a.norm;
}


struct Post1Args {
    const float* h;
    const float* outW;
    const float* out_b;
    const float* x0;
    const float* xcur;
    const int* node_of;
    const float* nmask;
    float* out;
    int* nanflag;
    int M, N, D, F, H, mol_shape;
};

__global__ void k_post1(Post1Args a) {
    const int lane = threadIdx.x & 63;
    const int i = blockIdx.x * (blockDim.x >> 6) + (threadIdx.x >> 6);
    if (i >= a.M) return;
    const int flat = a.node_of[i];
    const float m = a.nmask[i];
    float* orow = a.out + (size_t)flat * a.D;
    const int q = a.H >> 2;
    for (int f0 = 0; f0 < a.F; f0 += 8) {
        float p[8];
#pragma unroll
        for (int k = 0; k < 8; ++k) p[k] = 0.f;
        for (int c4 = lane; c4 < q; c4 += 64) {
            const f32x4 hv = *reinterpret_cast<const f32x4*>(a.h + (size_t)i * a.H + 4 * c4);
#pragma unroll
            for (int k = 0; k < 8; ++k) {
                if (f0 + k < a.F) {
                    const f32x4 w = *reinterpret_cast<const f32x4*>(a.outW + (size_t)(f0 + k) * a.H + 4 * c4);
#pragma unroll
                    for (int j = 0; j < 4; ++j) p[k] = __builtin_fmaf(hv[j], w[j], p[k]);
                }
            }
        }
        const bool b5 = lane & 32, b4 = lane & 16, b3 = lane & 8;
        float v4[4], v2[2], v1;
#pragma unroll
        for (int k = 0; k < 4; ++k) v4[k] = (b5 ? p[k + 4] : p[k]) + __shfl_xor(b5 ? p[k] : p[k + 4], 32);
#pragma unroll
        for (int k = 0; k < 2; ++k) v2[k] = (b4 ? v4[k + 2] : v4[k]) + __shfl_xor(b4 ? v4[k] : v4[k + 2], 16);
        v1 = (b3 ? v2[1] : v2[0]) + __shfl_xor(b3 ? v2[0] : v2[1], 8);
        v1 += __shfl_xor(v1, 4); v1 += __shfl_xor(v1, 2); v1 += __shfl_xor(v1, 1);
        const int f = f0 + (b5 ? 4 : 0) + (b4 ? 2 : 0) + (b3 ? 1 : 0);
        if ((lane & 7) == 0 && f < a.F) orow[3 + f] = (v1 + a.out_b[f]) * m;
    }
    if (lane < 3) {
        const int nloc = flat % a.N;
        float v = 0.f;
        if (a.mol_shape < 0 || nloc < a.mol_shape) v = (a.xcur[(size_t)i * 4 + lane] - a.x0[(size_t)i * 4 + lane]) * m;
        orow[lane] = v;
        if (v != v) atomicOr(a.nanflag, 1);
    }
}


struct Post2Args {
    const int* slot_of;
    const float* nmask;
    const int* nvalid;
    float* out;
    const int* nanflag;
    long long* nan_events;
    int B, N, D;
};

__global__ void k_post2(Post2Args a) {
    const int lane = threadIdx.x & 63;
    const int b = blockIdx.x * (blockDim.x >> 6) + (threadIdx.x >> 6);
    if (b >= a.B) return;
    const bool nan = (*a.nanflag) != 0;
    if (nan && b == 0 && lane == 0) atomicAdd(reinterpret_cast<unsigned long long*>(a.nan_events), 1ULL);
    float sx = 0.f, sy = 0.f, sz = 0.f;
    for (int nn = lane; nn < a.N; nn += 64) {
        const int flat = b * a.N + nn;
        float* orow = a.out + (size_t)flat * a.D;
        if (a.slot_of[flat] < 0) {
            for (int d = 0; d < a.D; ++d) orow[d] = 0.f;
        } else if (nan) {
            orow[0] = 0.f; orow[1] = 0.f; orow[2] = 0.f;
        } else {
            sx += orow[0]; sy += orow[1]; sz += orow[2];
        }
    }
#pragma unroll
    for (int o = 32; o > 0; o >>= 1) { sx += __shfl_xor(sx, o); sy += __shfl_xor(sy, o); sz += __shfl_xor(sz, o); }
    const int cnt = a.nvalid[b];
    if (cnt == 0) return;
    const float mx = sx / (float)cnt, my = sy / (float)cnt, mz = sz / (float)cnt;
    for (int nn = lane; nn < a.N; nn += 64) {
        const int flat = b * a.N + nn;
        const int s = a.slot_of[flat];
        if (s < 0) continue;
        const float m = a.nmask[s];
        float* orow = a.out + (size_t)flat * a.D;
        orow[0] -= mx * m; orow[1] -= my * m; orow[2] -= mz * m;
    }
}


struct NoiseSrc {
    const float* raw_x;
    const float* raw_h;
    int rows;
    uint64_t seed, sample_base;
    uint32_t draw;
    int share;
};

HD_DEVINL float raw_noise(const NoiseSrc& s, int b, int nn, int c, int mol, int F) {
    if (s.raw_x) {
        const int rb = (s.rows == 1) ? 0 : b;
        return (c < 3) ? s.raw_x[((size_t)rb * mol + nn) * 3 + c] : s.raw_h[((size_t)rb * mol + nn) * F + (c - 3)];
    }
    const uint64_t sid = s.sample_base + (s.share ? 0 : (uint64_t)b);
    return philox_normal(s.seed, sid, s.draw, (uint32_t)(nn * (3 + F) + c));
}

struct StepArgs {
    const float* zt;
    const float* eps;
    const float* coef;
    const uint8_t* nm;
    float* zs;
    NoiseSrc noise;
    const uint32_t* draw_ptr;
    const int* step_ptr;
    const unsigned long long* base_ptr;
    uint32_t draw0;
    int coef_rows, B, N, D, F, mol, out_stride;
};

HD_DEVINL float block_sum4(float v, float* red, int tid) {
#pragma unroll
    for (int o = 32; o > 0; o >>= 1) v += __shfl_xor(v, o);
    __syncthreads();
    if ((tid & 63) == 0) red[tid >> 6] = v;
    __syncthreads();
    return (red[0] + red[1]) + (red[2] + red[3]);
}

__global__ __launch_bounds__(256) void k_post_step(StepArgs a) {
    extern __shared__ float nz_s[];
    __shared__ float red[4];
    const int tid = threadIdx.x;
    const int b = blockIdx.x;
    NoiseSrc ns = a.noise;
    if (a.base_ptr) ns.sample_base = *a.base_ptr;
    if (a.draw_ptr) {
        ns.draw = *a.draw_ptr;
        if (ns.raw_x) {
            const size_t k = (size_t)(ns.draw - a.draw0) * ns.rows * a.mol;
            ns.raw_x += k * 3;
            ns.raw_h += k * a.F;
        }
    }
    const float* cf = a.coef + (a.step_ptr ? (size_t)(*a.step_ptr) * 4 : (size_t)((a.coef_rows == 1) ? 0 : b) * 4);
    const float alpha_ts = cf[0], sigma2_ts = cf[1], sigma_t = cf[2], sigma = cf[3];
    const float ceps = (sigma2_ts / alpha_ts) / sigma_t;
    const int mol = a.mol, D = a.D, total = mol * D;
    float se[3] = {0.f, 0.f, 0.f}, sn[3] = {0.f, 0.f, 0.f}, cnt = 0.f;
    for (int e = tid; e < total; e += 256) {
        const int nn = e / D, c = e - nn * D;
        const float m = a.nm[b * a.N + nn] ? 1.f : 0.f;
        const float z = raw_noise(ns, b, nn, c, mol, a.F) * m;
        nz_s[e] = z;
        if (c < 3) {
            const float ev = a.eps[((size_t)b * a.N + nn) * D + c];
#pragma unroll
            for (int k = 0; k < 3; ++k) { if (c == k) { se[k] += ev; sn[k] += z; } }
            if (c == 0) cnt += m;
        }
    }
    float em[3], nmn[3];
#pragma unroll
    for (int k = 0; k < 3; ++k) { em[k] = block_sum4(se[k], red, tid); nmn[k] = block_sum4(sn[k], red, tid); }
    cnt = block_sum4(cnt, red, tid);
#pragma unroll
    for (int k = 0; k < 3; ++k) { em[k] /= cnt; nmn[k] /= cnt; }
    float sv[3] = {0.f, 0.f, 0.f};
    for (int e = tid; e < total; e += 256) {
        const int nn = e / D, c = e - nn * D;
        const float m = a.nm[b * a.N + nn] ? 1.f : 0.f;
        const float zt = a.zt[((size_t)b * a.N + nn) * D + c];
        float ev = a.eps[((size_t)b * a.N + nn) * D + c];
        float z = nz_s[e];
        if (c < 3) {
#pragma unroll
            for (int k = 0; k < 3; ++k) { if (c == k) { ev -= em[k] * m; z -= nmn[k] * m; } }
        }
        const float v = (zt / alpha_ts - ceps * ev) + sigma * z;
        nz_s[e] = v;
        if (c < 3) {
#pragma unroll
            for (int k = 0; k < 3; ++k) { if (c == k) sv[k] += v; }
        }
    }
    float mean[3];
#pragma unroll
    for (int k = 0; k < 3; ++k) mean[k] = block_sum4(sv[k], red, tid) / cnt;
    for (int e = tid; e < total; e += 256) {
        const int nn = e / D, c = e - nn * D;
        float v = nz_s[e];
        if (c < 3) {
            const float m = a.nm[b * a.N + nn] ? 1.f : 0.f;
#pragma unroll
            for (int k = 0; k < 3; ++k) { if (c == k) v -= mean[k] * m; }
        }
        a.zs[((size_t)b * a.out_stride + nn) * D + c] = v;
    }
}

struct DecodeArgs {
    const float* z0;
    const float* eps;
    const uint8_t* nm;
    float* x;
    float* hfeat;
    NoiseSrc noise;
    float sigma_0, alpha_0, sigma_x;
    int B, N, D, F;
};

__global__ void k_final_decode(DecodeArgs a) {
    const int lane = threadIdx.x & 63;
    const int b = blockIdx.x * (blockDim.x >> 6) + (threadIdx.x >> 6);
    if (b >= a.B) return;
    float nx = 0.f, ny = 0.f, nz = 0.f, cnt = 0.f;
    for (int nn = lane; nn < a.N; nn += 64) {
        const float m = a.nm[b * a.N + nn] ? 1.f : 0.f;
        nx += raw_noise(a.noise, b, nn, 0, a.N, a.F) * m;
        ny += raw_noise(a.noise, b, nn, 1, a.N, a.F) * m;
        nz += raw_noise(a.noise, b, nn, 2, a.N, a.F) * m;
        cnt += m;
    }
#pragma unroll
    for (int o = 32; o > 0; o >>= 1) {
        nx += __shfl_xor(nx, o); ny += __shfl_xor(ny, o); nz += __shfl_xor(nz, o); cnt += __shfl_xor(cnt, o);
    }
    const float nmn[3] = {nx / cnt, ny / cnt, nz / cnt};
    const float inv_a = 1.0f / a.alpha_0;
    for (int nn = lane; nn < a.N; nn += 64) {
        const float m = a.nm[b * a.N + nn] ? 1.f : 0.f;
        const size_t r = (size_t)b * a.N + nn;
        const float* zr = a.z0 + r * a.D;
        const float* er = a.eps + r * a.D;
#pragma unroll
        for (int c = 0; c < 3; ++c) {
            float nz_ = raw_noise(a.noise, b, nn, c, a.N, a.F) * m - nmn[c] * m;
            a.x[r * 3 + c] = inv_a * (zr[c] - a.sigma_0 * er[c]) + a.sigma_x * nz_;
        }
        for (int f = 0; f < a.F; ++f) a.hfeat[r * a.F + f] = zr[3 + f] * m;
    }
}

struct NoiseArgs {
    const uint8_t* nm;
    float* z;
    NoiseSrc noise;
    int B, N, D, F;
};

__global__ void k_noise(NoiseArgs a) {
    const int lane = threadIdx.x & 63;
    const int b = blockIdx.x * (blockDim.x >> 6) + (threadIdx.x >> 6);
    if (b >= a.B) return;
    float nx = 0.f, ny = 0.f, nz = 0.f, cnt = 0.f;
    for (int nn = lane; nn < a.N; nn += 64) {
        const float m = a.nm[b * a.N + nn] ? 1.f : 0.f;
        nx += raw_noise(a.noise, b, nn, 0, a.N, a.F) * m;
        ny += raw_noise(a.noise, b, nn, 1, a.N, a.F) * m;
        nz += raw_noise(a.noise, b, nn, 2, a.N, a.F) * m;
        cnt += m;
    }
#pragma unroll
    for (int o = 32; o > 0; o >>= 1) {
        nx += __shfl_xor(nx, o); ny += __shfl_xor(ny, o); nz += __shfl_xor(nz, o); cnt += __shfl_xor(cnt, o);
    }
    const float nmn[3] = {nx / cnt, ny / cnt, nz / cnt};
    for (int nn = lane; nn < a.N; nn += 64) {
        const float m = a.nm[b * a.N + nn] ? 1.f : 0.f;
        float* o = a.z + ((size_t)b * a.N + nn) * a.D;
#pragma unroll
        for (int c = 0; c < 3; ++c) o[c] = raw_noise(a.noise, b, nn, c, a.N, a.F) * m - nmn[c] * m;
        for (int c = 3; c < a.D; ++c) o[c] = raw_noise(a.noise, b, nn, c, a.N, a.F) * m;
    }
}

__global__ void k_loop_state(int* step, uint32_t* draw, float* t_cur, unsigned long long* base, const float* tau,
                             int s0, uint32_t d0, unsigned long long b0) {
    *step = s0; *draw = d0; *t_cur = tau[s0 + 1]; *base = b0;
}

__global__ void k_advance(int* step, uint32_t* draw, float* t_cur, const float* tau) {
    int s = *step - 1;
    *step = s;
    *draw = *draw + 1;
    *t_cur = tau[s + 1 >= 0 ? s + 1 : 0];
}


template <int KIND>
__global__ __launch_bounds__(256, 2) void k_mfma_probe(const float* in, float* out, int iters) {
    const int lane = threadIdx.x & 63;
    f32x16 acc[8];
#pragma unroll
    for (int c = 0; c < 8; ++c)
#pragma unroll
        for (int r = 0; r < 16; ++r) acc[c][r] = 0.f;
    f16x8 ah, bh;
    bf16x8 ab, bb;
#pragma unroll
    for (int i = 0; i < 8; ++i) {
        ah[i] = (_Float16)in[(lane * 8 + i) & 1023]; bh[i] = (_Float16)in[(lane * 8 + i + 512) & 1023];
        ab[i] = (__bf16)in[(lane * 8 + i) & 1023]; bb[i] = (__bf16)in[(lane * 8 + i + 512) & 1023];
    }
    const float af = in[lane & 1023], bfv = in[(lane + 64) & 1023];
    for (int it = 0; it < iters; ++it) {
#pragma unroll
        for (int c = 0; c < 8; ++c) {
            if constexpr (KIND == 0) asm volatile("v_mfma_f32_32x32x2_f32 %0, %1, %2, %0" : "+v"(acc[c]) : "v"(af), "v"(bfv));
            if constexpr (KIND == 1) asm volatile("v_mfma_f32_32x32x16_f16 %0, %1, %2, %0" : "+v"(acc[c]) : "v"(ah), "v"(bh));
            if constexpr (KIND == 2) asm volatile("v_mfma_f32_32x32x16_bf16 %0, %1, %2, %0" : "+v"(acc[c]) : "v"(ab), "v"(bb));
        }
    }
    float s = 0.f;
#pragma unroll
    for (int c = 0; c < 8; ++c)
#pragma unroll
        for (int r = 0; r < 16; ++r) s += acc[c][r];
    out[blockIdx.x * 256 + threadIdx.x] = s;
}
```

Before: 47.31.

## Fold coordinate update into next edge kernel and post2 into step kernel

Removes the standalone k_xupd launch by having the next non-coordinate edge kernel (or post1) recompute the updated coordinates on the fly from the partial sums, while grid-striding to write them into a ping-pong buffer. It also merges the per-molecule centering (post2) into the diffusion step kernel, saving another launch per step. The cost is redundant partial-sum reduction per edge endpoint and extra complexity. An env/profile bit can restore the unfused path.

```diff
diff --git a/hierdiff_amd/csrc/common.hpp b/hierdiff_amd/csrc/common.hpp
--- a/hierdiff_amd/csrc/common.hpp
+++ b/hierdiff_amd/csrc/common.hpp
@@ -103,6 +103,36 @@
     }
 }
 
+struct XFuse {
+    const float* part;
+    const int* pstart;
+    const float* nmask;
+    float* xnew;
+    float norm;
+    int M;
+};
+
+HD_DEVINL f32x4 xupd_row(const float* xold, const float* part, const int* pstart, const float* nmask, float norm, int i) {
+#pragma clang fp contract(off)
+    float sx = 0.f, sy = 0.f, sz = 0.f;
+    for (int p = pstart[i]; p < pstart[i + 1]; ++p) {
+        f32x4 v = *reinterpret_cast<const f32x4*>(part + (size_t)p * 4);
+        sx += v[0]; sy += v[1]; sz += v[2];
+    }
+    const float m = nmask[i];
+    f32x4 x = *reinterpret_cast<const f32x4*>(xold + (size_t)i * 4);
+    x[0] = (x[0] + sx / norm) * m;
+    x[1] = (x[1] + sy / norm) * m;
+    x[2] = (x[2] + sz / norm) * m;
+    return x;
+}
+
+HD_DEVINL void xfuse_store(const XFuse& f, const float* xold) {
+    if (!f.part) return;
+    for (int i = blockIdx.x * blockDim.x + threadIdx.x; i < f.M; i += gridDim.x * blockDim.x)
+        *reinterpret_cast<f32x4*>(f.xnew + (size_t)i * 4) = xupd_row(xold, f.part, f.pstart, f.nmask, f.norm, i);
+}
+
 
 HD_DEVINL void philox_round(uint32_t& c0, uint32_t& c1, uint32_t& c2, uint32_t& c3, uint32_t k0, uint32_t k1) {
     const uint32_t M0 = 0xD2511F53u, M1 = 0xCD9E8D57u;
diff --git a/hierdiff_amd/csrc/hierdiff_hip.hip b/hierdiff_amd/csrc/hierdiff_hip.hip
--- a/hierdiff_amd/csrc/hierdiff_hip.hip
+++ b/hierdiff_amd/csrc/hierdiff_hip.hip
@@ -86,6 +86,7 @@
     int f32_split;
     int mix_max_tiles;
     int mix_rounds;
+    int glue_unfused;
     int n_cu;
 #ifdef HD_DEBUG_KERNELS
     long long* d_trace;
@@ -104,22 +105,23 @@
 struct GraphKey {
     const float *raw_x, *raw_h;
     int has_ctx, mol_shape, noise_rows, T, s_hi;
+    int glue_unfused;
     uint64_t seed;
     unsigned long long weights_gen, sched_gen;
     bool operator==(const GraphKey& o) const {
         return raw_x == o.raw_x && raw_h == o.raw_h && has_ctx == o.has_ctx && mol_shape == o.mol_shape &&
                noise_rows == o.noise_rows && T == o.T && s_hi == o.s_hi && seed == o.seed && weights_gen == o.weights_gen &&
-               sched_gen == o.sched_gen;
+               sched_gen == o.sched_gen && glue_unfused == o.glue_unfused;
     }
 };
 
 struct InpaintKey {
-    int has_ctx, T, resamplings;
+    int has_ctx, T, resamplings, glue_unfused;
     uint64_t seed;
     unsigned long long weights_gen, sched_gen, ip_gen;
     bool operator==(const InpaintKey& o) const {
         return has_ctx == o.has_ctx && T == o.T && resamplings == o.resamplings && seed == o.seed && weights_gen == o.weights_gen &&
-               sched_gen == o.sched_gen && ip_gen == o.ip_gen;
+               sched_gen == o.sched_gen && ip_gen == o.ip_gen && glue_unfused == o.glue_unfused;
     }
 };
 
@@ -134,7 +136,7 @@
     float *w2img, *w2timg;
     uint8_t *eseg, *nm_bytes;
     float* nmask;
-    float *hbuf, *AB, *AB2, *Tb, *agg, *x0, *xcur, *part, *xpart, *eps;
+    float *hbuf, *AB, *AB2, *Tb, *agg, *x0, *xcur, *xcur2, *part, *xpart, *eps;
     float *abmax, *abmax2;
     float *rowinfo;
     float *zbuf, *ctxbuf;
@@ -254,6 +256,7 @@
     h->node_split_max_rows = HD_NODE_SPLIT_MAX_ROWS;
     h->f32_split = 1;
     h->mix_rounds = -1;
+    h->glue_unfused = 0;
     {
         hipDeviceProp_t prop;
         h->n_cu = (hipGetDeviceProperties(&prop, device) == hipSuccess && prop.multiProcessorCount > 0) ? prop.multiProcessorCount : 256;
@@ -834,6 +837,7 @@
     const size_t f_part = carve((size_t)std::max(1, n_parts) * H), f_xpart = carve((size_t)std::max(1, n_parts) * 4);
     const size_t f_abmax = carve((size_t)M_pad * 2), f_abmax2 = carve((size_t)M_pad * 2), f_rowinfo = carve((size_t)M_pad * 2);
     const size_t f_eps = carve(BN * h->D), f_z = carve(BN * h->D), f_ctx = carve(BN * (size_t)std::max(1, h->cfg.context_node_nf));
+    const size_t f_xcur2 = carve((size_t)M_pad * 4);
     const size_t f_w2 = carve((size_t)H * H * 3 / 2), f_w2t = carve((size_t)H * H * 3 / 2);
     auto build = [&]() -> int {
         ArenaSlot sl;
@@ -854,7 +858,7 @@
         t->rptr = I(o_rptr); t->rrows = I(o_rrows); t->sptr = I(o_sptr); t->srows = I(o_srows);
         float* ws = reinterpret_cast<float*>(base + table_bytes);
         t->hbuf = ws + f_h; t->AB = ws + f_AB; t->AB2 = ws + f_AB2; t->Tb = ws + f_Tb; t->agg = ws + f_agg; t->x0 = ws + f_x0;
-        t->xcur = ws + f_xcur; t->part = ws + f_part; t->xpart = ws + f_xpart; t->eps = ws + f_eps; t->zbuf = ws + f_z;
+        t->xcur = ws + f_xcur; t->xcur2 = ws + f_xcur2; t->part = ws + f_part; t->xpart = ws + f_xpart; t->eps = ws + f_eps; t->zbuf = ws + f_z;
         t->abmax = ws + f_abmax; t->abmax2 = ws + f_abmax2; t->rowinfo = ws + f_rowinfo;
         t->ctxbuf = ws + f_ctx; t->w2img = ws + f_w2; t->w2timg = ws + f_w2t;
         t->node_of_host = new std::vector<int>(node_of);
@@ -900,6 +904,7 @@
 extern "C" int hd_profile_enable(hd_handle* h, int on) {
     if (!h) return fail(HD_E_INVALID, "hd_profile_enable: null handle");
     h->prof = on & 7;
+    h->glue_unfused = (on >> 3) & 1;
     h->prof_stride = std::max(1, on >> 8);
     h->prof_fwd = 0;
     h->prof_now = false;
@@ -1266,14 +1271,22 @@
     }
 }
 
+static Post2Args post2_args(hd_handle* h, hd_topology* t, float* out) {
+    Post2Args p;
+    p.slot_of = t->slot_of; p.nmask = t->nmask; p.nvalid = t->nvalid; p.out = out; p.nanflag = h->d_nanflag;
+    p.nan_events = h->d_nan_events; p.B = t->B; p.N = t->N; p.D = h->D;
+    return p;
+}
+
 static int forward_impl(hd_handle* h, hd_topology* t, const float* xh, const float* tt, int t_numel,
-                        const float* context, int mol_shape, float* out, hipStream_t s) {
+                        const float* context, int mol_shape, float* out, hipStream_t s, bool defer_post2 = false) {
     const hd_config& c = h->cfg;
     const int H = h->H, M = t->M;
     const float* W = h->dw;
     h->prof_now = h->prof != 0 && (h->prof_fwd++ % h->prof_stride) == 0;
     if (M == 0) HIP_TRY(hipMemsetAsync(h->d_nanflag, 0, sizeof(int), s));
     if (M > 0) {
+        const bool fold = !h->glue_unfused;
         {
             ProfScope ps(h, s, 2);
             InitArgs a;
@@ -1327,6 +1340,11 @@
             a.Wimg[q] = W + nw.ab_img; a.bias[q] = W + nw.ab_bias; a.winv[q] = 1.0f / nw.abs_; a.ABout[q] = dst;
             a.ABmax[q] = h->edge_mode == 3 ? (dst == t->AB ? t->abmax : t->abmax2) : nullptr;
         };
+        float* xc = t->xcur;
+        bool xparts = false;
+        auto set_xfuse = [&](XFuse& f, float* xnew) {
+            f.part = t->xpart; f.pstart = t->pstart; f.nmask = t->nmask; f.xnew = xnew; f.norm = agg_norm(c, t); f.M = M;
+        };
         {
             const LayerW* first[2] = {&h->gcl[0], nullptr};
             float* dst[2] = {t->AB, nullptr};
@@ -1363,7 +1381,12 @@
                     hipLaunchKernelGGL(k_ab_rowmax, dim3((M + 3) / 4), dim3(256), 0, s, am);
                 }
                 e.ei = t->ei; e.ej = t->ej; e.eseg = t->eseg; e.seg_part = t->seg_part; e.tile_nseg = t->tile_nseg;
-                e.xcur = t->xcur; e.x0 = t->x0; e.part = coord ? t->xpart : t->part; e.ba = w.ba;
+                e.xcur = xc; e.x0 = t->x0; e.part = coord ? t->xpart : t->part; e.ba = w.ba;
+                if (xparts) {
+                    float* xn = (xc == t->xcur) ? t->xcur2 : t->xcur;
+                    set_xfuse(e.xf, xn);
+                    xc = xn; xparts = false;
+                }
                 e.norm_constant = c.norm_constant; e.coords_range = range; e.attention = c.attention;
                 e.use_tanh = c.tanh; e.n_tiles = t->n_tiles; e.n_wg = t->n_wg;
                 HD_TRY(edge(h, coord, e, s));
@@ -1417,11 +1440,15 @@
                     }
                     ab_cur = t->AB;
                 } else {
-                    ProfScope ps(h, s, 2);
-                    XupdArgs x;
-                    x.part = t->xpart; x.pstart = t->pstart; x.nmask = t->nmask; x.xcur = t->xcur;
-                    x.norm = agg_norm(c, t); x.M = M;
-                    hipLaunchKernelGGL(k_xupd, dim3((M + 255) / 256), dim3(256), 0, s, x);
+                    if (fold && t->n_wg > 0) {
+                        xparts = true;
+                    } else {
+                        ProfScope ps(h, s, 2);
+                        XupdArgs x;
+                        x.part = t->xpart; x.pstart = t->pstart; x.nmask = t->nmask; x.xcur = t->xcur;
+                        x.norm = agg_norm(c, t); x.M = M;
+                        hipLaunchKernelGGL(k_xupd, dim3((M + 255) / 256), dim3(256), 0, s, x);
+                    }
                     ab_cur = t->AB2;
                 }
             }
@@ -1429,17 +1456,17 @@
         {
             ProfScope ps(h, s, 2);
             Post1Args p;
-            p.h = t->hbuf; p.outW = W + h->outW; p.out_b = W + h->out_b; p.x0 = t->x0; p.xcur = t->xcur;
+            p.h = t->hbuf; p.outW = W + h->outW; p.out_b = W + h->out_b; p.x0 = t->x0; p.xcur = xc;
+            std::memset(&p.xf, 0, sizeof(p.xf));
+            if (xparts) set_xfuse(p.xf, nullptr);
             p.node_of = t->node_of; p.nmask = t->nmask; p.out = out; p.nanflag = h->d_nanflag;
             p.M = M; p.N = t->N; p.D = h->D; p.F = h->F; p.H = H; p.mol_shape = mol_shape;
             hipLaunchKernelGGL(k_post1, dim3((M + 3) / 4), dim3(256), 0, s, p);
         }
     }
-    {
+    if (!defer_post2) {
         ProfScope ps(h, s, 2);
-        Post2Args p;
-        p.slot_of = t->slot_of; p.nmask = t->nmask; p.nvalid = t->nvalid; p.out = out; p.nanflag = h->d_nanflag;
-        p.nan_events = h->d_nan_events; p.B = t->B; p.N = t->N; p.D = h->D;
+        const Post2Args p = post2_args(h, t, out);
         hipLaunchKernelGGL(k_post2, dim3((t->B + 3) / 4), dim3(256), 0, s, p);
     }
     HIP_TRY(hipGetLastError());
@@ -2318,13 +2345,19 @@
 
 static int step_impl(hd_handle* h, hd_topology* t, const float* zt, const float* eps, const float* coef, int coef_rows,
                      const NoiseSrc& ns, int mol, float* zs, int out_stride, const int* step_ptr,
-                     const uint32_t* draw_ptr, uint32_t draw0, hipStream_t s, const unsigned long long* base_ptr = nullptr) {
+                     const uint32_t* draw_ptr, uint32_t draw0, hipStream_t s, const unsigned long long* base_ptr = nullptr,
+                     bool with_post2 = false) {
     ProfScope ps(h, s, 2);
     StepArgs a;
     a.zt = zt; a.eps = eps; a.coef = coef; a.nm = t->nm_bytes; a.zs = zs; a.noise = ns; a.draw_ptr = draw_ptr;
     a.step_ptr = step_ptr; a.base_ptr = base_ptr; a.draw0 = draw0; a.coef_rows = coef_rows; a.B = t->B; a.N = t->N; a.D = h->D; a.F = h->F;
     a.mol = mol; a.out_stride = out_stride;
-    hipLaunchKernelGGL(k_post_step, dim3(t->B), dim3(256), (size_t)a.mol * a.D * sizeof(float), s, a);
+    if (with_post2) {
+        const Post2Args p = post2_args(h, t, const_cast<float*>(eps));
+        hipLaunchKernelGGL(k_post_step_with_post2, dim3(t->B), dim3(256), (size_t)a.mol * a.D * sizeof(float), s, p, a);
+    } else {
+        hipLaunchKernelGGL(k_post_step, dim3(t->B), dim3(256), (size_t)a.mol * a.D * sizeof(float), s, a);
+    }
     HIP_TRY(hipGetLastError());
     return HD_OK;
 }
@@ -2418,14 +2451,15 @@
     const int T = h->T;
     const uint32_t draw0 = (uint32_t)(T - (s_hi - 1));
     const int share = (noise_rows == 1) ? 1 : 0;
+    const bool fold = !h->glue_unfused;
     if (!use_graph) {
         for (int k = 0; k < nsteps; ++k) {
             const int sidx = s_hi - 1 - k;
-            HD_TRY(forward_impl(h, topo, z, h->d_tau + sidx + 1, 1, context, mol_shape < 0 ? -1 : mol, topo->eps, s));
+            HD_TRY(forward_impl(h, topo, z, h->d_tau + sidx + 1, 1, context, mol_shape < 0 ? -1 : mol, topo->eps, s, fold));
             NoiseSrc ns = make_noise(raw_x ? raw_x + (size_t)k * noise_rows * mol * 3 : nullptr,
                                      raw_h ? raw_h + (size_t)k * noise_rows * mol * h->F : nullptr, noise_rows, seed,
                                      sample_id_base, draw0 + (uint32_t)k, share);
-            HD_TRY(step_impl(h, topo, z, topo->eps, h->d_coef + (size_t)sidx * 4, 1, ns, mol, z, topo->N, nullptr, nullptr, 0, s));
+            HD_TRY(step_impl(h, topo, z, topo->eps, h->d_coef + (size_t)sidx * 4, 1, ns, mol, z, topo->N, nullptr, nullptr, 0, s, nullptr, fold));
         }
         return HD_OK;
     }
@@ -2440,6 +2474,7 @@
     }
     GraphKey key;
     key.raw_x = raw_x; key.raw_h = raw_h; key.has_ctx = context ? 1 : 0; key.mol_shape = mol_shape < 0 ? -1 : mol;
+    key.glue_unfused = h->glue_unfused;
     key.noise_rows = noise_rows; key.T = T; key.s_hi = raw_x ? s_hi : 0; key.seed = seed; key.weights_gen = h->weights_gen; key.sched_gen = h->sched_gen;
     if (h->ev_last_set) HIP_TRY(hipStreamWaitEvent(rs, h->ev_last, 0));
     if (topo->gexec && !(topo->gkey == key)) {
@@ -2454,11 +2489,11 @@
         hipGraph_t graph = nullptr;
         HIP_TRY(hipStreamBeginCapture(rs, hipStreamCaptureModeThreadLocal));
         int rc = forward_impl(h, topo, topo->zbuf, h->d_tcur, 1, context ? topo->ctxbuf : nullptr, mol_shape < 0 ? -1 : mol,
-                              topo->eps, rs);
+                              topo->eps, rs, fold);
         if (rc == HD_OK) {
             NoiseSrc ns = make_noise(raw_x, raw_h, noise_rows, seed, 0, draw0, share);
             rc = step_impl(h, topo, topo->zbuf, topo->eps, h->d_coef, 1, ns, mol, topo->zbuf, topo->N, h->d_step, h->d_draw,
-                           draw0, rs, h->d_base);
+                           draw0, rs, h->d_base, fold);
         }
         if (rc == HD_OK) hipLaunchKernelGGL(k_advance, dim3(1), dim3(1), 0, rs, h->d_step, h->d_draw, h->d_tcur, h->d_tau);
         const hipError_t ce = hipStreamEndCapture(rs, &graph);
@@ -2548,14 +2583,15 @@
     if (nsteps == 0) return HD_OK;
     const int N = topo->N;
     const uint32_t draw0 = (uint32_t)(T - (s_hi - 1));
+    const bool fold = !h->glue_unfused;
     if (!use_graph) {
         for (int k = 0; k < nsteps; ++k) {
             const int sidx = s_hi - 1 - k;
             const uint32_t d = draw0 + (uint32_t)k;
             for (int j = 0; j < R; ++j) {
-                HD_TRY(forward_impl(h, topo, z, h->d_tau + sidx + 1, 1, context, -1, topo->eps, s));
+                HD_TRY(forward_impl(h, topo, z, h->d_tau + sidx + 1, 1, context, -1, topo->eps, s, fold));
                 NoiseSrc ns = make_noise(nullptr, nullptr, noise_rows, seed, sample_id_base, stride * (uint32_t)(3 * j) + d, 0);
-                HD_TRY(step_impl(h, topo, z, topo->eps, h->d_coef + (size_t)sidx * 4, 1, ns, N, z, N, nullptr, nullptr, 0, s));
+                HD_TRY(step_impl(h, topo, z, topo->eps, h->d_coef + (size_t)sidx * 4, 1, ns, N, z, N, nullptr, nullptr, 0, s, nullptr, fold));
                 HD_TRY(inpaint_launch(h, topo, false, z, fixed_mask, xh_known, seed, sample_id_base, stride * (uint32_t)(3 * j + 1) + d,
                                       sidx, nullptr, nullptr, nullptr, s));
                 if (j < R - 1)
@@ -2589,6 +2625,7 @@
     if (!topo->ip_known) HIP_TRY(hipMalloc(reinterpret_cast<void**>(&topo->ip_known), zbytes));
     InpaintKey key;
     key.has_ctx = context ? 1 : 0; key.T = T; key.resamplings = R; key.seed = seed; key.weights_gen = h->weights_gen;
+    key.glue_unfused = h->glue_unfused;
     key.sched_gen = h->sched_gen; key.ip_gen = h->ip_gen;
     if (topo->gexec_ip && !(topo->ikey == key)) {
         if (h->ev_last_set) HIP_TRY(hipEventSynchronize(h->ev_last));
@@ -2603,11 +2640,11 @@
         HIP_TRY(hipStreamBeginCapture(rs, hipStreamCaptureModeThreadLocal));
         int rc = HD_OK;
         for (int j = 0; j < R && rc == HD_OK; ++j) {
-            rc = forward_impl(h, topo, topo->zbuf, h->d_tcur, 1, context ? topo->ctxbuf : nullptr, -1, topo->eps, rs);
+            rc = forward_impl(h, topo, topo->zbuf, h->d_tcur, 1, context ? topo->ctxbuf : nullptr, -1, topo->eps, rs, fold);
             if (rc == HD_OK) {
                 NoiseSrc ns = make_noise(nullptr, nullptr, noise_rows, seed, 0, 0, 0);
                 rc = step_impl(h, topo, topo->zbuf, topo->eps, h->d_coef, 1, ns, N, topo->zbuf, N, h->d_step, h->d_ipdraw + 3 * j,
-                               0, rs, h->d_base);
+                               0, rs, h->d_base, fold);
             }
             if (rc == HD_OK)
                 rc = inpaint_launch(h, topo, false, topo->zbuf, topo->ip_fixed, topo->ip_known, seed, 0, 0, 0, h->d_ipdraw + 3 * j + 1,
diff --git a/hierdiff_amd/csrc/k_edge.hpp b/hierdiff_amd/csrc/k_edge.hpp
--- a/hierdiff_amd/csrc/k_edge.hpp
+++ b/hierdiff_amd/csrc/k_edge.hpp
@@ -35,7 +35,14 @@
     const float* abmax;
     const float* dscal;
     float* pre2;
+    XFuse xf;
 };
+
+template <bool FOLD>
+HD_DEVINL f32x4 edge_row_x(const EdgeArgs& a, int i) {
+    if (FOLD && a.xf.part) return xupd_row(a.xcur, a.xf.part, a.xf.pstart, a.xf.nmask, a.xf.norm, i);
+    return *reinterpret_cast<const f32x4*>(a.xcur + (size_t)i * 4);
+}
 
 constexpr int HD_EDGE_SAVE = 256;
 constexpr int HD_EDGE_UNSCALED = 512;
@@ -189,8 +196,8 @@
     }
 
     int gc = 0;
-    f32x4 xi = *reinterpret_cast<const f32x4*>(a.xcur + (size_t)ni * 4);
-    f32x4 xj = *reinterpret_cast<const f32x4*>(a.xcur + (size_t)nj * 4);
+    f32x4 xi = edge_row_x<!COORD>(a, ni);
+    f32x4 xj = edge_row_x<!COORD>(a, nj);
     f32x4 yi = *reinterpret_cast<const f32x4*>(a.x0 + (size_t)ni * 4);
     f32x4 yj = *reinterpret_cast<const f32x4*>(a.x0 + (size_t)nj * 4);
     const float dx = xi[0] - xj[0], dy = xi[1] - xj[1], dz = xi[2] - xj[2];
@@ -733,5 +740,6 @@
 __global__ __launch_bounds__(256, 2) void k_edge(EdgeArgs a) {
     extern __shared__ __attribute__((aligned(16))) float smem[];
     __shared__ __attribute__((aligned(16))) float wrd_s[4 * H];
+    if constexpr (!COORD) xfuse_store(a.xf, a.xcur);
     edge_tile_body<H, COORD, PREC, ABL>(a, smem, wrd_s, blockIdx.x, a.n_wg);
 }
diff --git a/hierdiff_amd/csrc/k_edge_split.hpp b/hierdiff_amd/csrc/k_edge_split.hpp
--- a/hierdiff_amd/csrc/k_edge_split.hpp
+++ b/hierdiff_amd/csrc/k_edge_split.hpp
@@ -31,8 +31,8 @@
     const int e = tile * 32 + n;
     const int ni = a.ei[e], nj = a.ej[e];
     const uint32_t segb = a.eseg[e];
-    const f32x4 xi = *reinterpret_cast<const f32x4*>(a.xcur + (size_t)ni * 4);
-    const f32x4 xj = *reinterpret_cast<const f32x4*>(a.xcur + (size_t)nj * 4);
+    const f32x4 xi = edge_row_x<!COORD>(a, ni);
+    const f32x4 xj = edge_row_x<!COORD>(a, nj);
     const f32x4 yi = *reinterpret_cast<const f32x4*>(a.x0 + (size_t)ni * 4);
     const f32x4 yj = *reinterpret_cast<const f32x4*>(a.x0 + (size_t)nj * 4);
     const float dx = xi[0] - xj[0], dy = xi[1] - xj[1], dz = xi[2] - xj[2];
@@ -374,6 +374,7 @@
 __global__ __launch_bounds__(256) void k_edge_split(EdgeArgs a) {
     __shared__ __attribute__((aligned(16))) float wrd_s[4 * H];
     __shared__ __attribute__((aligned(16))) char lds[edge_split_lds_bytes<H, PREC>()];
+    if constexpr (!COORD) xfuse_store(a.xf, a.xcur);
     edge_split_body<H, COORD, PREC, true>(a, lds, wrd_s, blockIdx.x);
 }
 
@@ -382,6 +383,7 @@
     extern __shared__ __attribute__((aligned(16))) float smem[];
     __shared__ __attribute__((aligned(16))) float wrd_s[4 * H];
     const int bid = blockIdx.x;
+    if constexpr (!COORD) xfuse_store(a.xf, a.xcur);
     if (bid < a.n_wg) edge_tile_body<H, COORD, PREC, 0>(a, smem, wrd_s, bid, a.n_wg);
     else edge_split_body<H, COORD, PREC, false>(a, reinterpret_cast<char*>(smem), wrd_s, 4 * a.n_wg + (bid - a.n_wg));
 }
diff --git a/hierdiff_amd/csrc/k_sampling.hpp b/hierdiff_amd/csrc/k_sampling.hpp
--- a/hierdiff_amd/csrc/k_sampling.hpp
+++ b/hierdiff_amd/csrc/k_sampling.hpp
@@ -14,17 +14,7 @@
 __global__ void k_xupd(XupdArgs a) {
     int i = blockIdx.x * blockDim.x + threadIdx.x;
     if (i >= a.M) return;
-    float sx = 0.f, sy = 0.f, sz = 0.f;
-    for (int p = a.pstart[i]; p < a.pstart[i + 1]; ++p) {
-        f32x4 v = *reinterpret_cast<const f32x4*>(a.part + (size_t)p * 4);
-        sx += v[0]; sy += v[1]; sz += v[2];
-    }
-    float m = a.nmask[i];
-    f32x4 x = *reinterpret_cast<const f32x4*>(a.xcur + (size_t)i * 4);
-    x[0] = (x[0] + sx / a.norm) * m;
-    x[1] = (x[1] + sy / a.norm) * m;
-    x[2] = (x[2] + sz / a.norm) * m;
-    *reinterpret_cast<f32x4*>(a.xcur + (size_t)i * 4) = x;
+    *reinterpret_cast<f32x4*>(a.xcur + (size_t)i * 4) = xupd_row(a.xcur, a.part, a.pstart, a.nmask, a.norm, i);
 }
 
 struct AggArgs {
@@ -57,6 +47,7 @@
     float* out;
     int* nanflag;
     int M, N, D, F, H, mol_shape;
+    XFuse xf;
 };
 
 __global__ void k_post1(Post1Args a) {
@@ -96,7 +87,10 @@
     if (lane < 3) {
         const int nloc = flat % a.N;
         float v = 0.f;
-        if (a.mol_shape < 0 || nloc < a.mol_shape) v = (a.xcur[(size_t)i * 4 + lane] - a.x0[(size_t)i * 4 + lane]) * m;
+        if (a.mol_shape < 0 || nloc < a.mol_shape) {
+            const float xc = a.xf.part ? xupd_row(a.xcur, a.xf.part, a.xf.pstart, a.nmask, a.xf.norm, i)[lane] : a.xcur[(size_t)i * 4 + lane];
+            v = (xc - a.x0[(size_t)i * 4 + lane]) * m;
+        }
         orow[lane] = v;
         if (v != v) atomicOr(a.nanflag, 1);
     }
@@ -113,10 +107,7 @@
     int B, N, D;
 };
 
-__global__ void k_post2(Post2Args a) {
-    const int lane = threadIdx.x & 63;
-    const int b = blockIdx.x * (blockDim.x >> 6) + (threadIdx.x >> 6);
-    if (b >= a.B) return;
+HD_DEVINL void post2_mol(const Post2Args& a, const int b, const int lane) {
     const bool nan = (*a.nanflag) != 0;
     if (nan && b == 0 && lane == 0) atomicAdd(reinterpret_cast<unsigned long long*>(a.nan_events), 1ULL);
     float sx = 0.f, sy = 0.f, sz = 0.f;
@@ -144,6 +135,13 @@
         float* orow = a.out + (size_t)flat * a.D;
         orow[0] -= mx * m; orow[1] -= my * m; orow[2] -= mz * m;
     }
+}
+
+__global__ void k_post2(Post2Args a) {
+    const int lane = threadIdx.x & 63;
+    const int b = blockIdx.x * (blockDim.x >> 6) + (threadIdx.x >> 6);
+    if (b >= a.B) return;
+    post2_mol(a, b, lane);
 }
 
 
@@ -188,11 +186,7 @@
     return (red[0] + red[1]) + (red[2] + red[3]);
 }
 
-__global__ __launch_bounds__(256) void k_post_step(StepArgs a) {
-    extern __shared__ float nz_s[];
-    __shared__ float red[4];
-    const int tid = threadIdx.x;
-    const int b = blockIdx.x;
+HD_DEVINL void post_step_mol(const StepArgs& a, float* nz_s, float* red, const int tid, const int b) {
     NoiseSrc ns = a.noise;
     if (a.base_ptr) ns.sample_base = *a.base_ptr;
     if (a.draw_ptr) {
@@ -257,6 +251,21 @@
         }
         a.zs[((size_t)b * a.out_stride + nn) * D + c] = v;
     }
+}
+
+__global__ __launch_bounds__(256) void k_post_step(StepArgs a) {
+    extern __shared__ float nz_s[];
+    __shared__ float red[4];
+    post_step_mol(a, nz_s, red, threadIdx.x, blockIdx.x);
+}
+
+__global__ __launch_bounds__(256) void k_post_step_with_post2(Post2Args p, StepArgs a) {
+    extern __shared__ float nz_s[];
+    __shared__ float red[4];
+    if (threadIdx.x < 64) post2_mol(p, blockIdx.x, threadIdx.x);
+    __threadfence_block();
+    __syncthreads();
+    post_step_mol(a, nz_s, red, threadIdx.x, blockIdx.x);
 }
 
 struct DecodeArgs {
```

Result: no change. 47.31 (-0.0%).
